# andrewjong/SwapNet

Hardware: NVIDIA H100
Metric: images/sec (G+D fwd+bwd) warp-stage 512x512 (higher is better)
Workload: dtype fp16/bf16-split x3 tensor-core products, fp32 accumulate (fp32-faithful)

## Files before the change

### include/swapnet_b200.h

```cpp
#ifndef SWAPNET_B200_H
#define SWAPNET_B200_H

#include <stdint.h>

#ifdef __cplusplus
extern "C" {
#endif

#define SN_MAX_TAPS 32
#define SN_MAX_SRC 3

enum { SN_ACT_NONE = 0, SN_ACT_TANH = 1, SN_ACT_LRELU = 2, SN_ACT_RELU = 3 };
enum { SN_LAYOUT_NCHW = 0, SN_LAYOUT_NHWC = 1, SN_LAYOUT_LABEL_U8 = 2, SN_LAYOUT_MASK_I32 = 3 };
#define SN_FMT_BF16 0
#define SN_FMT_F16 1

const char* sn_version(void);
const char* sn_last_error(void);
long long sn_launch_count(void);
void sn_count_replayed(long long n);

typedef struct sn_tap {
  int c_off;
  int kb_off;
  int dw, dh;
  int hp;
} sn_tap;

typedef struct sn_tap_gemm_desc {
  const void* a_hi; const void* a_lo;
  int a_n, a_h, a_w, a_c, a_pitch;
  int a_parity;
  int a_fmt;
  int a_chunk;
  const void* b_hi; const void* b_lo;
  int b_rows; long long b_k;
  int b_fmt;
  const float* b_scale;
  int m_n, m_h, m_w;
  int ntaps; int k_per_tap;
  sn_tap taps[SN_MAX_TAPS];
  float* out;
  long long out_sn, out_sh, out_sw;
  int out_mul_h, out_off_h, out_mul_w, out_off_w;
  int n_valid;
  int block_n;
  const float* bias;
  int act;
  int nsplit;
  int nphase;
  int stack_slot, stack_c;
  double* stats;
} sn_tap_gemm_desc;

typedef struct sn_wgrad_desc {
  const void* x_hi; const void* x_lo; int x_n, x_h, x_w, x_c, x_pitch, x_parity, x_fmt;
  const void* y_hi; const void* y_lo; int y_n, y_h, y_w, y_c, y_pitch, y_parity, y_fmt;
  int m_n, m_h, m_w;
  int ntaps;
  sn_tap xtaps[SN_MAX_TAPS];
  sn_tap ytaps[SN_MAX_TAPS];
  long long tap_off[SN_MAX_TAPS];
  float* out; long long s_row, s_col;
  int rows_valid, cols_valid;
  int block_n;
  int y_chunk;
  int ngroups; int group_start[SN_MAX_TAPS]; int group_size[SN_MAX_TAPS];
  int ksplit;
  int nsplit;
  int deterministic;
} sn_wgrad_desc;

typedef struct sn_plan sn_plan;

int sn_tap_gemm_plan_create(const sn_tap_gemm_desc* desc, sn_plan** out);
int sn_wgrad_plan_create(const sn_wgrad_desc* desc, sn_plan** out);
int sn_plan_run(const sn_plan* plan, void* stream);
void sn_plan_destroy(sn_plan* plan);
int sn_plan_has_stats(const sn_plan* plan);
int sn_plan_geometry(const sn_plan* plan, int* out);
long long sn_plan_workspace_bytes(const sn_plan* plan);
int sn_wgrad_ksplit(const sn_wgrad_desc* desc, int sm_count);

int sn_pack_planes(const float* src, int src_layout, int src_pitch, int n, int c, int h, int w,
                   void* dst_hi, void* dst_lo, int dst_pitch, int dst_coff, int fmt, void* stream);

int sn_pack_concat(int lead, const float* src0, int layout0, int pitch0, int c0, const float* src1, int layout1,
                   int pitch1, int c1, int n, int h, int w, int c_fill, void* dst_hi, void* dst_lo, void* dst2_hi,
                   void* dst2_lo, int dst_pitch, int dst_coff, int fmt, int fmt2, void* stream);

typedef struct sn_scale_item { const float* w; long long count; float* scale2; } sn_scale_item;
typedef struct sn_pack_item {
  const float* src; long long s_row, s_k;
  int rows, taps, taps_pitch, k_real, k_pad, fmt;
  void* hi; void* lo; const float* scale2;
  int slot[16];
  int block_begin;
} sn_pack_item;
int sn_weight_scale_multi(const sn_scale_item* items_dev, int nitems, unsigned int* scratch_dev, void* stream);
int sn_pack_weights_multi(const sn_pack_item* items_dev, int nitems, int total_blocks, int max_taps, void* stream);
int sn_pack_rows_per_block(void);
int sn_pack_k_per_block(void);

int sn_pack_head_weights(const float* src, int cout, int cin, int rows_pad, int k_pad, int dgrad, int taps_pitch,
                         void* dst_hi, void* dst_lo, int fmt, const float* scale2, void* stream);
int sn_pack_head_stacked(const float* src, int cout, int cin, int slot, int k_pad, void* dst_hi, void* dst_lo, int fmt,
                         const float* scale2, void* stream);
int sn_fold_head_wgrad(const float* geff, int cout, int cin, float* dw, void* stream);

int sn_plane_stats(const float* y, int pitch, int n, int hw, int c, float eps, double* stats,
                   void* stream);
int sn_stats_finalize(double* stats, int count, int hw, float eps, void* stream);
int sn_plane_sums(const float* y, int pitch, int n, int hw, int c, double* stats, void* stream);

long long sn_det_slots(int n, int c);
int sn_plane_sums_det(const float* y, int pitch, int n, int hw, int c, double* stats, double* slots,
                      long long slots_cap, void* stream);
int sn_plane_stats_det(const float* y, int pitch, int n, int hw, int c, float eps, double* stats, double* slots,
                       long long slots_cap, void* stream);

int sn_bn_finalize(double* stats, int n, int c, int groups, int hw, float eps, float momentum, float* running_mean,
                   float* running_var, long long* num_batches_tracked, void* stream);
int sn_bn_eval_stats(double* stats, int n, int c, const float* running_mean, const float* running_var, float eps,
                     void* stream);
int sn_bn_group_sums(const double* stats, int n, int c, int groups, int hw, double* part, void* stream);
int sn_bn_finalize_gathered(double* stats, int n, int c, int groups, const double* gathered, int world, float eps,
                            float momentum, float* running_mean, float* running_var, long long* num_batches_tracked,
                            void* stream);

typedef struct sn_norm_act_desc {
  const float* y; int y_pitch;
  int n, h, w, c;
  const double* stats;
  int act; float slope;
  float drop_p; unsigned long long drop_seed;
  unsigned long long drop_offset;
  const float* drop_step_seed_dev; unsigned int drop_stage_id;
  const float* residual; int res_pitch;
  void* out_hi; void* out_lo; int out_pitch, out_coff;
  int out_fmt;
  void* out2_hi; void* out2_lo; int out2_fmt;
  int out_reflect_pad;
  float* out_f32; int f32_pitch;
  const float* gamma; const float* beta;
} sn_norm_act_desc;
int sn_norm_act_fwd(const sn_norm_act_desc* d, void* stream);

typedef struct sn_grad_src {
  const float* ptr; int pitch; int c_off;
  int reflect_padded;
  int up;
  int act;
} sn_grad_src;

typedef struct sn_norm_act_bwd_desc {
  sn_grad_src src[SN_MAX_SRC]; int nsrc;
  const float* y; int y_pitch;
  int n, h, w, c;
  const double* stats;
  int act; float slope;
  float drop_p; unsigned long long drop_seed;
  unsigned long long drop_offset; const float* drop_step_seed_dev; unsigned int drop_stage_id;
  double* gstats;
  void* dy_hi; void* dy_lo; int dy_pitch, dy_coff;
  int dy_fmt;
  float* bias_grad;
  const float* gamma; const float* beta;
  int bn_groups;
  int bn_train;
  float* gamma_grad; float* beta_grad;
  double* det_slots; long long det_slots_cap;
  int bn_phase;
  const double* bn_gathered; int bn_world; int bn_rank;
} sn_norm_act_bwd_desc;
int sn_norm_act_bwd(const sn_norm_act_bwd_desc* d, void* stream);

int sn_bias_grad(const void* dy_hi, const void* dy_lo, int pitch, int coff, int fmt, long long npix, int c,
                 double* scratch, float* db, void* stream);
int sn_bias_grad_det(const void* dy_hi, const void* dy_lo, int pitch, int coff, int fmt, long long npix, int c,
                     double* scratch, float* db, double* slots, long long slots_cap, void* stream);

int sn_sum_grads(const sn_grad_src* src, int nsrc, int n, int h, int w, int c, float* dst,
                 int dst_pitch, void* stream);

int sn_tanh_bwd(const sn_grad_src* src, int nsrc, const float* out, int out_pitch, int n, int h,
                int w, int c, void* dy_hi, void* dy_lo, int dy_pitch, int dy_coff, int dy_fmt, void* stream);

int sn_upsample_planes(const void* src_hi, const void* src_lo, int src_pitch, int src_coff, int n, int h, int w,
                       int c, int factor, void* dst_hi, void* dst_lo, int dst_pitch, int dst_coff, void* stream);

int sn_adamw_step(float* p, const float* g, float* m, float* v, long long n, double lr, double beta1, double beta2,
                  double eps, double weight_decay, int step, void* stream);
int sn_adamw_step_dev(float* p, const float* g, float* m, float* v, long long n, const float* hyper_dev, void* stream);
void sn_adamw_hyper(double lr, double beta1, double beta2, double eps, double weight_decay, int step, double gscale,
                    float hyper_out[8]);

int sn_adabound_step(float* p, const float* g, float* m, float* v, long long n, double lr, double base_lr, double beta1,
                     double beta2, double eps, double weight_decay, double final_lr, double gamma, int step,
                     void* stream);
int sn_adabound_step_dev(float* p, const float* g, float* m, float* v, long long n, const float* hyper_dev,
                         void* stream);
void sn_adabound_hyper(double lr, double base_lr, double beta1, double beta2, double eps, double weight_decay,
                       double final_lr, double gamma, int step, double gscale, float hyper_out[8]);

int sn_set_step_params(float* dst, const float* vals, int n, void* stream);

int sn_dropout_mask(unsigned long long seed, float p, long long count, uint8_t* out, void* stream);

int sn_ce_loss_fwd_bwd(const float* logits, int pitch, const void* target, int target_layout, int n, int h, int w,
                       int c, float weight, double* loss_acc, float* grad, int grad_pitch, void* stream);
int sn_ce_tanh_bwd(const float* logits, int pitch, const void* target, int target_layout, const sn_grad_src* src,
                   int nsrc, int n, int h, int w, int c, float weight, double* loss_acc, void* dy_hi, void* dy_lo,
                   int dy_pitch, int dy_coff, int dy_fmt, void* stream);
int sn_ce_tanh_bwd_det(const float* logits, int pitch, const void* target, int target_layout, const sn_grad_src* src,
                       int nsrc, int n, int h, int w, int c, float weight, double* loss_acc, void* dy_hi, void* dy_lo,
                       int dy_pitch, int dy_coff, int dy_fmt, double* slots, long long slots_cap, void* stream);
int sn_bce_logits_fwd_bwd(const float* pred, long long count_per_half, int halves, float t0, float t1,
                          float gscale, double* loss_acc, float* dpred, void* stream);
int sn_bce_logits_fwd_bwd_dev(const float* pred, long long count_per_half, int halves, const float* t_dev,
                              float gscale, double* loss_acc, float* dpred, void* stream);
enum { SN_GAN_BCE = 0, SN_GAN_MSE = 1, SN_GAN_WGAN = 2 };
int sn_gan_loss_fwd_bwd_dev(int objective, const float* pred, long long count_per_half, int halves, float t0, float t1,
                            const float* t_dev, float gscale, double* loss_acc, float* dpred, void* stream);
int sn_gan_loss_fwd_bwd_det(int objective, const float* pred, long long count_per_half, int halves, float t0, float t1,
                            const float* t_dev, float gscale, double* loss_acc, float* dpred, double* slots,
                            long long slots_cap, void* stream);
int sn_l1_loss_fwd_bwd(const float* a, int pitch, const float* b_nchw, int n, int h, int w, int c,
                       float weight, double* loss_acc, float* grad, int grad_pitch, void* stream);
int sn_l1_loss_fwd_bwd_det(const float* a, int pitch, const float* b_nchw, int n, int h, int w, int c, float weight,
                           double* loss_acc, float* grad, int grad_pitch, double* slots, long long slots_cap,
                           void* stream);

int sn_tap_sum_fwd(const float* p, int p_pitch, int n, int h, int w, int k, int pad, const float* bias, float* y,
                   int y_pitch, void* stream);

int sn_to_one_fwd(const void* x_hi, const void* x_lo, int x_pitch, int x_fmt, long long npix, int c, const float* weight,
                  int k, float* p, int p_pitch, void* stream);
int sn_to_one_wgrad(const void* x_hi, const void* x_lo, int x_pitch, int x_fmt, int n, int h, int w, int c,
                    const void* dy_hi, const void* dy_lo, int dy_pitch, int dy_fmt, int k, int pad, float* dw,
                    void* stream);
int sn_to_one_wgrad_det(const void* x_hi, const void* x_lo, int x_pitch, int x_fmt, int n, int h, int w, int c,
                        const void* dy_hi, const void* dy_lo, int dy_pitch, int dy_fmt, int k, int pad, float* dw,
                        float* slots, long long slots_cap, void* stream);
long long sn_to_one_wgrad_det_slots(int c);
int sn_to_one_dgrad(const void* dy_hi, const void* dy_lo, int dy_pitch, int dy_fmt, int n, int h, int w, int c,
                    const float* weight, int k, int pad, float* dx, int dx_pitch, void* stream);

int sn_affine_pack(const float* src, int src_layout, int src_pitch, int n, int c, int h, int w, float mul, float add,
                   void* dst_hi, void* dst_lo, int dst_pitch, int dst_coff, int fmt, void* stream);
int sn_relu_pool_fwd(const float* y, int y_pitch, int n, int h, int w, int c, void* out_hi, void* out_lo,
                     int out_pitch, int out_coff, int fmt, void* stream);
int sn_relu_pool_bwd(const float* y, int y_pitch, const float* g_pool, int gp_pitch, const float* g_direct,
                     int gd_pitch, int n, int h, int w, int c, void* dy_hi, void* dy_lo, int dy_pitch, int dy_coff,
                     int dy_fmt, void* stream);
int sn_feat_loss_fwd_bwd(const float* y_out, int po, const float* y_tgt, int pt, long long npix, int c, double weight,
                         double gscale, double* loss_acc, float* dx, int pdx, void* stream);
int sn_feat_loss_fwd_bwd_det(const float* y_out, int po, const float* y_tgt, int pt, long long npix, int c,
                             double weight, double gscale, double* loss_acc, float* dx, int pdx, double* slots,
                             long long slots_cap, void* stream);

typedef struct sn_pixel_desc {
  const void* x_hi; const void* x_lo;
  const void* xb_hi; const void* xb_lo;
  int x_pitch, x_c;
  int n, hw, cin;
  const float* w1; const float* b1; const float* w2; const float* b2; const float* w3; const float* b3;
  const float* scale1; const float* scale2;
  int norm;
  int nsplit;
  float slope, eps;
  double* stats;
  double* gstats;
  float* pred;
  const float* dpred;
  float* dw1; float* db1; float* dw2; float* db2; float* dw3; float* db3;
  float* dx; int dx_pitch;
  float* debug;
  double* slots; long long slots_cap;
} sn_pixel_desc;
int sn_pixel_fwd_stats(const sn_pixel_desc* d, void* stream);
int sn_pixel_fwd(const sn_pixel_desc* d, void* stream);
int sn_pixel_bwd_reduce(const sn_pixel_desc* d, void* stream);
int sn_pixel_bwd_apply(const sn_pixel_desc* d, void* stream);
long long sn_pixel_det_slots(int n, int cin);
int sn_gram_rows(const float* a, long long a_n, long long a_c, long long a_p, int n_a, const float* b, long long b_n,
                 long long b_c, long long b_p, int n_b, int c, long long npix, double* out, void* stream);
int sn_gram_rows_det(const float* a, long long a_n, long long a_c, long long a_p, int n_a, const float* b,
                     long long b_n, long long b_c, long long b_p, int n_b, int c, long long npix, double* out,
                     double* slots, long long slots_cap, void* stream);
long long sn_gram_rows_det_slots(int rows_l, int rows);
int sn_gram_rows_mse(const double* gram_out, const double* gram_tgt, int rows_l, int rows, double weight,
                     double gscale, double* loss_acc, float* m, void* stream);
int sn_gram_rows_bwd(const float* m, int rows_l, const float* src, long long s_n, long long s_c, long long s_p, int n,
                     int c, long long npix, float* dx, int dx_pitch, int accumulate, void* stream);

int sn_roi_align_pack_fwd(const float* tex_nchw, int b, int ch, int h, int w, const float* rois,
                          int nroi, int pool, float* out_f32, int out_pitch, void* out_hi,
                          void* out_lo, int plane_pitch, int plane_coff, int plane_fmt, void* stream);

#define SN_AUG_NONE 0
#define SN_AUG_HFLIP 1
#define SN_AUG_VFLIP 2
#define SN_AUG_AFFINE_NEAREST 3
#define SN_AUG_PERSPECTIVE_BILINEAR 4
#define SN_AUG_MAX_OPS 8
typedef struct sn_aug_op {
  int kind;
  int nops;
  double p[8];
} sn_aug_op;
int sn_augment_channels(const void* labels_u8, const float* dense_nchw, int n, int c, int h, int w,
                        const sn_aug_op* ops_dev, int op_stride, int max_ops, float* out_nchw, float* tmp_nchw,
                        void* stream);

int sn_tap_gemm_simt(const sn_tap_gemm_desc* desc, void* stream);

#ifdef __cplusplus
}
#endif
#endif
```

### swapnet_b200/_lib.py

```python
from __future__ import annotations

import ctypes as C
import os

_HERE = os.path.dirname(os.path.abspath(__file__))
LIB_PATH = os.path.join(_HERE, "libswapnet_b200.so")

SN_MAX_TAPS = 32
SN_MAX_SRC = 3
ACT_NONE, ACT_TANH, ACT_LRELU, ACT_RELU = 0, 1, 2, 3
LAYOUT_NCHW, LAYOUT_NHWC, LAYOUT_LABEL_U8, LAYOUT_MASK_I32 = 0, 1, 2, 3
FMT_BF16, FMT_F16 = 0, 1
AUG_NONE, AUG_HFLIP, AUG_VFLIP, AUG_AFFINE_NEAREST, AUG_PERSPECTIVE_BILINEAR = 0, 1, 2, 3, 4
AUG_MAX_OPS = 8


class SnTap(C.Structure):
    _fields_ = [("c_off", C.c_int), ("kb_off", C.c_int), ("dw", C.c_int), ("dh", C.c_int), ("hp", C.c_int)]


class SnTapGemmDesc(C.Structure):
    _fields_ = [
        ("a_hi", C.c_void_p), ("a_lo", C.c_void_p),
        ("a_n", C.c_int), ("a_h", C.c_int), ("a_w", C.c_int), ("a_c", C.c_int), ("a_pitch", C.c_int),
        ("a_parity", C.c_int), ("a_fmt", C.c_int), ("a_chunk", C.c_int),
        ("b_hi", C.c_void_p), ("b_lo", C.c_void_p),
        ("b_rows", C.c_int), ("b_k", C.c_longlong), ("b_fmt", C.c_int), ("b_scale", C.c_void_p),
        ("m_n", C.c_int), ("m_h", C.c_int), ("m_w", C.c_int),
        ("ntaps", C.c_int), ("k_per_tap", C.c_int),
        ("taps", SnTap * SN_MAX_TAPS),
        ("out", C.c_void_p),
        ("out_sn", C.c_longlong), ("out_sh", C.c_longlong), ("out_sw", C.c_longlong),
        ("out_mul_h", C.c_int), ("out_off_h", C.c_int), ("out_mul_w", C.c_int), ("out_off_w", C.c_int),
        ("n_valid", C.c_int), ("block_n", C.c_int),
        ("bias", C.c_void_p), ("act", C.c_int), ("nsplit", C.c_int), ("nphase", C.c_int),
        ("stack_slot", C.c_int), ("stack_c", C.c_int), ("stats", C.c_void_p),
    ]


class SnWgradDesc(C.Structure):
    _fields_ = [
        ("x_hi", C.c_void_p), ("x_lo", C.c_void_p),
        ("x_n", C.c_int), ("x_h", C.c_int), ("x_w", C.c_int), ("x_c", C.c_int), ("x_pitch", C.c_int),
        ("x_parity", C.c_int), ("x_fmt", C.c_int),
        ("y_hi", C.c_void_p), ("y_lo", C.c_void_p),
        ("y_n", C.c_int), ("y_h", C.c_int), ("y_w", C.c_int), ("y_c", C.c_int), ("y_pitch", C.c_int),
        ("y_parity", C.c_int), ("y_fmt", C.c_int),
        ("m_n", C.c_int), ("m_h", C.c_int), ("m_w", C.c_int),
        ("ntaps", C.c_int),
        ("xtaps", SnTap * SN_MAX_TAPS), ("ytaps", SnTap * SN_MAX_TAPS),
        ("tap_off", C.c_longlong * SN_MAX_TAPS),
        ("out", C.c_void_p), ("s_row", C.c_longlong), ("s_col", C.c_longlong),
        ("rows_valid", C.c_int), ("cols_valid", C.c_int),
        ("block_n", C.c_int), ("y_chunk", C.c_int),
        ("ngroups", C.c_int), ("group_start", C.c_int * SN_MAX_TAPS), ("group_size", C.c_int * SN_MAX_TAPS),
        ("ksplit", C.c_int), ("nsplit", C.c_int), ("deterministic", C.c_int),
    ]


class SnScaleItem(C.Structure):
    _fields_ = [("w", C.c_void_p), ("count", C.c_longlong), ("scale2", C.c_void_p)]


class SnPackItem(C.Structure):
    _fields_ = [("src", C.c_void_p), ("s_row", C.c_longlong), ("s_k", C.c_longlong),
                ("rows", C.c_int), ("taps", C.c_int), ("taps_pitch", C.c_int), ("k_real", C.c_int), ("k_pad", C.c_int),
                ("fmt", C.c_int), ("hi", C.c_void_p), ("lo", C.c_void_p), ("scale2", C.c_void_p),
                ("slot", C.c_int * 16), ("block_begin", C.c_int)]


class SnNormActDesc(C.Structure):
    _fields_ = [
        ("y", C.c_void_p), ("y_pitch", C.c_int),
        ("n", C.c_int), ("h", C.c_int), ("w", C.c_int), ("c", C.c_int),
        ("stats", C.c_void_p),
        ("act", C.c_int), ("slope", C.c_float),
        ("drop_p", C.c_float), ("drop_seed", C.c_ulonglong),
        ("drop_offset", C.c_ulonglong), ("drop_step_seed_dev", C.c_void_p), ("drop_stage_id", C.c_uint),
        ("residual", C.c_void_p), ("res_pitch", C.c_int),
        ("out_hi", C.c_void_p), ("out_lo", C.c_void_p), ("out_pitch", C.c_int), ("out_coff", C.c_int),
        ("out_fmt", C.c_int), ("out2_hi", C.c_void_p), ("out2_lo", C.c_void_p), ("out2_fmt", C.c_int),
        ("out_reflect_pad", C.c_int),
        ("out_f32", C.c_void_p), ("f32_pitch", C.c_int),
        ("gamma", C.c_void_p), ("beta", C.c_void_p),
    ]


class SnGradSrc(C.Structure):
    _fields_ = [("ptr", C.c_void_p), ("pitch", C.c_int), ("c_off", C.c_int), ("reflect_padded", C.c_int),
                ("up", C.c_int), ("act", C.c_int)]


class SnNormActBwdDesc(C.Structure):
    _fields_ = [
        ("src", SnGradSrc * SN_MAX_SRC), ("nsrc", C.c_int),
        ("y", C.c_void_p), ("y_pitch", C.c_int),
        ("n", C.c_int), ("h", C.c_int), ("w", C.c_int), ("c", C.c_int),
        ("stats", C.c_void_p),
        ("act", C.c_int), ("slope", C.c_float),
        ("drop_p", C.c_float), ("drop_seed", C.c_ulonglong),
        ("drop_offset", C.c_ulonglong), ("drop_step_seed_dev", C.c_void_p), ("drop_stage_id", C.c_uint),
        ("gstats", C.c_void_p),
        ("dy_hi", C.c_void_p), ("dy_lo", C.c_void_p), ("dy_pitch", C.c_int), ("dy_coff", C.c_int),
        ("dy_fmt", C.c_int), ("bias_grad", C.c_void_p),
        ("gamma", C.c_void_p), ("beta", C.c_void_p), ("bn_groups", C.c_int), ("bn_train", C.c_int),
        ("gamma_grad", C.c_void_p), ("beta_grad", C.c_void_p),
        ("det_slots", C.c_void_p), ("det_slots_cap", C.c_longlong),
        ("bn_phase", C.c_int), ("bn_gathered", C.c_void_p), ("bn_world", C.c_int), ("bn_rank", C.c_int),
    ]


class SnPixelDesc(C.Structure):
    _fields_ = [
        ("x_hi", C.c_void_p), ("x_lo", C.c_void_p), ("xb_hi", C.c_void_p), ("xb_lo", C.c_void_p),
        ("x_pitch", C.c_int), ("x_c", C.c_int), ("n", C.c_int), ("hw", C.c_int), ("cin", C.c_int),
        ("w1", C.c_void_p), ("b1", C.c_void_p), ("w2", C.c_void_p), ("b2", C.c_void_p), ("w3", C.c_void_p),
        ("b3", C.c_void_p), ("scale1", C.c_void_p), ("scale2", C.c_void_p),
        ("norm", C.c_int), ("nsplit", C.c_int), ("slope", C.c_float), ("eps", C.c_float),
        ("stats", C.c_void_p), ("gstats", C.c_void_p), ("pred", C.c_void_p), ("dpred", C.c_void_p),
        ("dw1", C.c_void_p), ("db1", C.c_void_p), ("dw2", C.c_void_p), ("db2", C.c_void_p), ("dw3", C.c_void_p),
        ("db3", C.c_void_p), ("dx", C.c_void_p), ("dx_pitch", C.c_int), ("debug", C.c_void_p),
        ("slots", C.c_void_p), ("slots_cap", C.c_longlong),
    ]


_VP, _I, _LL, _F, _ULL = C.c_void_p, C.c_int, C.c_longlong, C.c_float, C.c_ulonglong
SIGNATURES = {
    "sn_version": (C.c_char_p, []),
    "sn_last_error": (C.c_char_p, []),
    "sn_launch_count": (_LL, []),
    "sn_count_replayed": (None, [_LL]),
    "sn_tap_gemm_plan_create": (_I, [C.POINTER(SnTapGemmDesc), C.POINTER(_VP)]),
    "sn_wgrad_plan_create": (_I, [C.POINTER(SnWgradDesc), C.POINTER(_VP)]),
    "sn_plan_run": (_I, [_VP, _VP]),
    "sn_plan_destroy": (None, [_VP]),
    "sn_plan_has_stats": (_I, [_VP]),
    "sn_plan_geometry": (_I, [_VP, C.POINTER(C.c_int)]),
    "sn_plan_workspace_bytes": (_LL, [_VP]),
    "sn_wgrad_ksplit": (_I, [C.POINTER(SnWgradDesc), _I]),
    "sn_det_slots": (_LL, [_I, _I]),
    "sn_plane_sums_det": (_I, [_VP, _I, _I, _I, _I, _VP, _VP, _LL, _VP]),
    "sn_plane_stats_det": (_I, [_VP, _I, _I, _I, _I, _F, _VP, _VP, _LL, _VP]),
    "sn_bias_grad_det": (_I, [_VP, _VP, _I, _I, _I, _LL, _I, _VP, _VP, _VP, _LL, _VP]),
    "sn_ce_tanh_bwd_det": (_I, [_VP, _I, _VP, _I, C.POINTER(SnGradSrc), _I, _I, _I, _I, _I, _F, _VP, _VP, _VP, _I, _I,
                                _I, _VP, _LL, _VP]),
    "sn_gan_loss_fwd_bwd_det": (_I, [_I, _VP, _LL, _I, _F, _F, _VP, _F, _VP, _VP, _VP, _LL, _VP]),
    "sn_l1_loss_fwd_bwd_det": (_I, [_VP, _I, _VP, _I, _I, _I, _I, _F, _VP, _VP, _I, _VP, _LL, _VP]),
    "sn_to_one_wgrad_det": (_I, [_VP, _VP, _I, _I, _I, _I, _I, _I, _VP, _VP, _I, _I, _I, _I, _VP, _VP, _LL, _VP]),
    "sn_to_one_wgrad_det_slots": (_LL, [_I]),
    "sn_stats_finalize": (_I, [_VP, _I, _I, _F, _VP]),
    "sn_plane_sums": (_I, [_VP, _I, _I, _I, _I, _VP, _VP]),
    "sn_bn_finalize": (_I, [_VP, _I, _I, _I, _I, _F, _F, _VP, _VP, _VP, _VP]),
    "sn_bn_eval_stats": (_I, [_VP, _I, _I, _VP, _VP, _F, _VP]),
    "sn_bn_group_sums": (_I, [_VP, _I, _I, _I, _I, _VP, _VP]),
    "sn_bn_finalize_gathered": (_I, [_VP, _I, _I, _I, _VP, _I, _F, _F, _VP, _VP, _VP, _VP]),
    "sn_pack_planes": (_I, [_VP, _I, _I, _I, _I, _I, _I, _VP, _VP, _I, _I, _I, _VP]),
    "sn_pack_concat": (_I, [_I, _VP, _I, _I, _I, _VP, _I, _I, _I, _I, _I, _I, _I, _VP, _VP, _VP, _VP, _I, _I, _I, _I, _VP]),
    "sn_pack_head_weights": (_I, [_VP, _I, _I, _I, _I, _I, _I, _VP, _VP, _I, _VP, _VP]),
    "sn_weight_scale_multi": (_I, [_VP, _I, _VP, _VP]),
    "sn_pack_weights_multi": (_I, [_VP, _I, _I, _I, _VP]),
    "sn_pack_rows_per_block": (_I, []),
    "sn_pack_k_per_block": (_I, []),
    "sn_pack_head_stacked": (_I, [_VP, _I, _I, _I, _I, _VP, _VP, _I, _VP, _VP]),
    "sn_fold_head_wgrad": (_I, [_VP, _I, _I, _VP, _VP]),
    "sn_plane_stats": (_I, [_VP, _I, _I, _I, _I, _F, _VP, _VP]),
    "sn_norm_act_fwd": (_I, [C.POINTER(SnNormActDesc), _VP]),
    "sn_norm_act_bwd": (_I, [C.POINTER(SnNormActBwdDesc), _VP]),
    "sn_bias_grad": (_I, [_VP, _VP, _I, _I, _I, _LL, _I, _VP, _VP, _VP]),
    "sn_sum_grads": (_I, [C.POINTER(SnGradSrc), _I, _I, _I, _I, _I, _VP, _I, _VP]),
    "sn_tanh_bwd": (_I, [C.POINTER(SnGradSrc), _I, _VP, _I, _I, _I, _I, _I, _VP, _VP, _I, _I, _I, _VP]),
    "sn_upsample_planes": (_I, [_VP, _VP, _I, _I, _I, _I, _I, _I, _I, _VP, _VP, _I, _I, _VP]),
    "sn_adamw_step": (_I, [_VP, _VP, _VP, _VP, _LL, C.c_double, C.c_double, C.c_double, C.c_double, C.c_double, _I, _VP]),
    "sn_adamw_step_dev": (_I, [_VP, _VP, _VP, _VP, _LL, _VP, _VP]),
    "sn_adamw_hyper": (None, [C.c_double, C.c_double, C.c_double, C.c_double, C.c_double, _I, C.c_double,
                              C.POINTER(C.c_float)]),
    "sn_adabound_step": (_I, [_VP, _VP, _VP, _VP, _LL] + [C.c_double] * 8 + [_I, _VP]),
    "sn_adabound_step_dev": (_I, [_VP, _VP, _VP, _VP, _LL, _VP, _VP]),
    "sn_adabound_hyper": (None, [C.c_double] * 8 + [_I, C.c_double, C.POINTER(C.c_float)]),
    "sn_set_step_params": (_I, [_VP, C.POINTER(C.c_float), _I, _VP]),
    "sn_bce_logits_fwd_bwd_dev": (_I, [_VP, _LL, _I, _VP, _F, _VP, _VP, _VP]),
    "sn_dropout_mask": (_I, [_ULL, _F, _LL, _VP, _VP]),
    "sn_ce_loss_fwd_bwd": (_I, [_VP, _I, _VP, _I, _I, _I, _I, _I, _F, _VP, _VP, _I, _VP]),
    "sn_ce_tanh_bwd": (_I, [_VP, _I, _VP, _I, C.POINTER(SnGradSrc), _I, _I, _I, _I, _I, _F, _VP, _VP, _VP, _I, _I, _I, _VP]),
    "sn_bce_logits_fwd_bwd": (_I, [_VP, _LL, _I, _F, _F, _F, _VP, _VP, _VP]),
    "sn_gan_loss_fwd_bwd_dev": (_I, [_I, _VP, _LL, _I, _F, _F, _VP, _F, _VP, _VP, _VP]),
    "sn_l1_loss_fwd_bwd": (_I, [_VP, _I, _VP, _I, _I, _I, _I, _F, _VP, _VP, _I, _VP]),
    "sn_tap_sum_fwd": (_I, [_VP, _I, _I, _I, _I, _I, _I, _VP, _VP, _I, _VP]),
    "sn_to_one_fwd": (_I, [_VP, _VP, _I, _I, _LL, _I, _VP, _I, _VP, _I, _VP]),
    "sn_to_one_wgrad": (_I, [_VP, _VP, _I, _I, _I, _I, _I, _I, _VP, _VP, _I, _I, _I, _I, _VP, _VP]),
    "sn_to_one_dgrad": (_I, [_VP, _VP, _I, _I, _I, _I, _I, _I, _VP, _I, _I, _VP, _I, _VP]),
    "sn_affine_pack": (_I, [_VP, _I, _I, _I, _I, _I, _I, _F, _F, _VP, _VP, _I, _I, _I, _VP]),
    "sn_relu_pool_fwd": (_I, [_VP, _I, _I, _I, _I, _I, _VP, _VP, _I, _I, _I, _VP]),
    "sn_relu_pool_bwd": (_I, [_VP, _I, _VP, _I, _VP, _I, _I, _I, _I, _I, _VP, _VP, _I, _I, _I, _VP]),
    "sn_feat_loss_fwd_bwd": (_I, [_VP, _I, _VP, _I, _LL, _I, C.c_double, C.c_double, _VP, _VP, _I, _VP]),
    "sn_feat_loss_fwd_bwd_det": (_I, [_VP, _I, _VP, _I, _LL, _I, C.c_double, C.c_double, _VP, _VP, _I, _VP, _LL, _VP]),
    "sn_gram_rows": (_I, [_VP, _LL, _LL, _LL, _I, _VP, _LL, _LL, _LL, _I, _I, _LL, _VP, _VP]),
    "sn_gram_rows_det": (_I, [_VP, _LL, _LL, _LL, _I, _VP, _LL, _LL, _LL, _I, _I, _LL, _VP, _VP, _LL, _VP]),
    "sn_gram_rows_det_slots": (_LL, [_I, _I]),
    "sn_gram_rows_mse": (_I, [_VP, _VP, _I, _I, C.c_double, C.c_double, _VP, _VP, _VP]),
    "sn_gram_rows_bwd": (_I, [_VP, _I, _VP, _LL, _LL, _LL, _I, _I, _LL, _VP, _I, _I, _VP]),
    "sn_roi_align_pack_fwd": (_I, [_VP, _I, _I, _I, _I, _VP, _I, _I, _VP, _I, _VP, _VP, _I, _I, _I, _VP]),
    "sn_tap_gemm_simt": (_I, [C.POINTER(SnTapGemmDesc), _VP]),
    "sn_pixel_fwd_stats": (_I, [C.POINTER(SnPixelDesc), _VP]),
    "sn_pixel_fwd": (_I, [C.POINTER(SnPixelDesc), _VP]),
    "sn_pixel_bwd_reduce": (_I, [C.POINTER(SnPixelDesc), _VP]),
    "sn_pixel_bwd_apply": (_I, [C.POINTER(SnPixelDesc), _VP]),
    "sn_pixel_det_slots": (_LL, [_I, _I]),
    "sn_augment_channels": (_I, [_VP, _VP, _I, _I, _I, _I, _VP, _I, _I, _VP, _VP, _VP]),
}

_lib = None


class SwapnetB200Error(RuntimeError):
    pass


def load(build_if_missing: bool = False) -> C.CDLL:
    global _lib
    if _lib is not None:
        return _lib
    if not os.path.exists(LIB_PATH):
        if build_if_missing:
            from . import build as _build

            _build.build(verbose=False)
        else:
            raise SwapnetB200Error(
                f"{LIB_PATH} is missing: build it with `python -m swapnet_b200.build` "
                "(there is no CPU / eager fallback for the hot path)"
            )
    lib = C.CDLL(LIB_PATH)
    for name, (res, args) in SIGNATURES.items():
        fn = getattr(lib, name)
        fn.restype = res
        fn.argtypes = args
    _lib = lib
    return lib


def check(rc: int) -> None:
    if rc != 0:
        msg = load().sn_last_error().decode("utf-8", "replace")
        raise SwapnetB200Error(f"libswapnet_b200 call failed ({rc}): {msg}")
```

### swapnet_b200/csrc/api.cu

```cuda
#include <stdarg.h>
#include <atomic>
#include "common.cuh"
#include "plan.h"

static thread_local char g_err[1024] = "";
std::atomic<long long> g_launches{0};

void sn_set_error(const char* fmt, ...) {
  va_list ap;
  va_start(ap, fmt);
  vsnprintf(g_err, sizeof(g_err), fmt, ap);
  va_end(ap);
}
void sn_count_launch(int n) { g_launches.fetch_add(n, std::memory_order_relaxed); }

struct sn_plan {
  int kind;
  TapGemmPlan tg;
  WgradPlan wg;
};

static int g_sm_count = 0;
static int sm_count() {
  if (!g_sm_count) {
    int dev = 0;
    cudaGetDevice(&dev);
    cudaDeviceGetAttribute(&g_sm_count, cudaDevAttrMultiProcessorCount, dev);
    if (g_sm_count <= 0) g_sm_count = SN_NUM_SMS;
  }
  return g_sm_count;
}

extern "C" {

const char* sn_version(void) { return "swapnet_b200 0.1.0 (sm_90a, wgmma split-bf16)"; }
const char* sn_last_error(void) { return g_err; }
long long sn_launch_count(void) { return g_launches.load(std::memory_order_relaxed); }
void sn_count_replayed(long long n) { g_launches.fetch_add(n, std::memory_order_relaxed); }

int sn_tap_gemm_plan_create(const sn_tap_gemm_desc* desc, sn_plan** out) {
  SN_REQUIRE(desc && out, "null argument");
  sn_plan* p = new sn_plan();
  p->kind = 0;
  int rc = sn_tap_gemm_plan_init(&p->tg, desc);
  if (rc) {
    delete p;
    return rc;
  }
  *out = p;
  return SN_OK;
}

int sn_wgrad_plan_create(const sn_wgrad_desc* desc, sn_plan** out) {
  SN_REQUIRE(desc && out, "null argument");
  sn_plan* p = new sn_plan();
  p->kind = 1;
  int rc = sn_wgrad_plan_init(&p->wg, desc, sm_count());
  if (rc) {
    delete p;
    return rc;
  }
  *out = p;
  return SN_OK;
}

int sn_plan_run(const sn_plan* plan, void* stream) {
  SN_REQUIRE(plan, "null plan");
  sn_count_launch(1);
  if (plan->kind == 0) return sn_tap_gemm_plan_launch(&plan->tg, (cudaStream_t)stream);
  return sn_wgrad_plan_launch(&plan->wg, (cudaStream_t)stream);
}

int sn_plan_has_stats(const sn_plan* plan) { return plan && plan->kind == 0 && plan->tg.p.stats != nullptr; }

int sn_plan_geometry(const sn_plan* plan, int* out) {
  SN_REQUIRE(plan && out, "null argument");
  const dim3 g = plan->kind == 0 ? plan->tg.grid : plan->wg.grid;
  out[0] = plan->kind;
  out[1] = (int)g.x;
  out[2] = (int)g.y;
  out[3] = (int)g.z;
  out[4] = plan->kind == 0 ? plan->tg.p.block_n : plan->wg.p.block_n;
  out[5] = plan->kind == 0 ? plan->tg.p.a_chunk : plan->wg.p.y_chunk;
  return SN_OK;
}

long long sn_plan_workspace_bytes(const sn_plan* plan) {
  return plan && plan->kind == 1 ? (long long)plan->wg.ws_bytes : 0;
}

int sn_wgrad_ksplit(const sn_wgrad_desc* desc, int sm_count) { return sn_wgrad_plan_ksplit(desc, sm_count); }

void sn_plan_destroy(sn_plan* plan) {
  if (plan && plan->kind == 0 && plan->tg.p.tile_counter) cudaFree(plan->tg.p.tile_counter);
  if (plan && plan->kind == 1 && plan->wg.p.det_ws) cudaFree(plan->wg.p.det_ws);
  delete plan;
}

}
```

### swapnet_b200/csrc/common.cuh

```cuda
#pragma once
#include <cuda_runtime.h>
#include <cuda.h>
#include <cuda_bf16.h>
#include <cuda_fp16.h>
#include <stdint.h>
#include <stdio.h>
#include <string.h>

void sn_set_error(const char* fmt, ...);
#define SN_OK 0
#define SN_ERR_INVALID (-1)
#define SN_ERR_CUDA (-2)
#define SN_ERR_UNSUPPORTED (-3)
#define SN_NUM_SMS 132
#ifndef SN_FMT_BF16
#define SN_FMT_BF16 0
#define SN_FMT_F16 1
#endif

#define SN_CHECK_CUDA(expr)                                                        \
  do {                                                                             \
    cudaError_t _e = (expr);                                                       \
    if (_e != cudaSuccess) {                                                       \
      sn_set_error("%s:%d CUDA error %s: %s", __FILE__, __LINE__, #expr,           \
                   cudaGetErrorString(_e));                                        \
      return SN_ERR_CUDA;                                                          \
    }                                                                              \
  } while (0)

#define SN_REQUIRE(cond, ...)                                                      \
  do {                                                                             \
    if (!(cond)) {                                                                 \
      sn_set_error(__VA_ARGS__);                                                   \
      return SN_ERR_INVALID;                                                       \
    }                                                                              \
  } while (0)

#ifdef __CUDACC__

__device__ __forceinline__ uint32_t smem_u32(const void* p) {
  return static_cast<uint32_t>(__cvta_generic_to_shared(p));
}

__device__ __forceinline__ bool elect_one_sync() {
  uint32_t pred = 0;
  asm volatile(
      "{\n\t"
      ".reg .pred P;\n\t"
      "elect.sync _|P, 0xffffffff;\n\t"
      "selp.b32 %0, 1, 0, P;\n\t"
      "}\n"
      : "=r"(pred));
  return pred != 0;
}

__device__ __forceinline__ void mbar_init(uint64_t* bar, uint32_t count) {
  asm volatile("mbarrier.init.shared::cta.b64 [%0], %1;" ::"r"(smem_u32(bar)), "r"(count));
}
__device__ __forceinline__ void mbar_fence_init() {
  asm volatile("fence.mbarrier_init.release.cluster;" ::: "memory");
}
__device__ __forceinline__ void mbar_expect_tx(uint64_t* bar, uint32_t bytes) {
  asm volatile("mbarrier.arrive.expect_tx.shared::cta.b64 _, [%0], %1;" ::"r"(smem_u32(bar)),
               "r"(bytes)
               : "memory");
}
__device__ __forceinline__ void mbar_arrive(uint64_t* bar) {
  asm volatile("mbarrier.arrive.shared::cta.b64 _, [%0];" ::"r"(smem_u32(bar)) : "memory");
}
__device__ __forceinline__ bool mbar_try_wait(uint64_t* bar, uint32_t parity) {
  uint32_t ok;
  asm volatile(
      "{\n\t"
      ".reg .pred P;\n\t"
      "mbarrier.try_wait.parity.shared::cta.b64 P, [%1], %2;\n\t"
      "selp.b32 %0, 1, 0, P;\n\t"
      "}\n"
      : "=r"(ok)
      : "r"(smem_u32(bar)), "r"(parity)
      : "memory");
  return ok != 0;
}
__device__ __forceinline__ void mbar_wait(uint64_t* bar, uint32_t parity) {
  uint32_t spins = 0;
  while (!mbar_try_wait(bar, parity)) {
    if (++spins > (1u << 28)) __trap();
  }
}

__device__ __forceinline__ void tma_prefetch_desc(const void* desc) {
  asm volatile("prefetch.tensormap [%0];" ::"l"(reinterpret_cast<uint64_t>(desc)) : "memory");
}
__device__ __forceinline__ void tma_load_2d(const void* desc, uint64_t* bar, void* dst, int c0,
                                            int c1) {
  asm volatile(
      "cp.async.bulk.tensor.2d.shared::cluster.global.mbarrier::complete_tx::bytes"
      " [%0], [%1, {%3, %4}], [%2];"
      :
      : "r"(smem_u32(dst)), "l"(reinterpret_cast<uint64_t>(desc)), "r"(smem_u32(bar)), "r"(c0),
        "r"(c1)
      : "memory");
}
__device__ __forceinline__ void tma_load_3d(const void* desc, uint64_t* bar, void* dst, int c0, int c1, int c2) {
  asm volatile(
      "cp.async.bulk.tensor.3d.shared::cluster.global.mbarrier::complete_tx::bytes"
      " [%0], [%1, {%3, %4, %5}], [%2];"
      :
      : "r"(smem_u32(dst)), "l"(reinterpret_cast<uint64_t>(desc)), "r"(smem_u32(bar)), "r"(c0), "r"(c1), "r"(c2)
      : "memory");
}
__device__ __forceinline__ void tma_load_5d(const void* desc, uint64_t* bar, void* dst, int c0,
                                            int c1, int c2, int c3, int c4) {
  asm volatile(
      "cp.async.bulk.tensor.5d.shared::cluster.global.mbarrier::complete_tx::bytes"
      " [%0], [%1, {%3, %4, %5, %6, %7}], [%2];"
      :
      : "r"(smem_u32(dst)), "l"(reinterpret_cast<uint64_t>(desc)), "r"(smem_u32(bar)), "r"(c0),
        "r"(c1), "r"(c2), "r"(c3), "r"(c4)
      : "memory");
}

__device__ __forceinline__ void wgmma_fence() { asm volatile("wgmma.fence.sync.aligned;" ::: "memory"); }
__device__ __forceinline__ void wgmma_commit() { asm volatile("wgmma.commit_group.sync.aligned;" ::: "memory"); }
template <int N>
__device__ __forceinline__ void wgmma_wait() {
  asm volatile("wgmma.wait_group.sync.aligned %0;" ::"n"(N) : "memory");
}
template <int R>
__device__ __forceinline__ void wgmma_fence_acc(float (&d)[R]) {
#pragma unroll
  for (int i = 0; i < R; ++i) asm volatile("" : "+f"(d[i])::"memory");
}

template <int N, bool F16>
struct Wgmma;
template <> struct Wgmma<16, false> {
  template <int TA, int TB>
  static __device__ __forceinline__ void mma(float (&d)[8], uint64_t a, uint64_t b, int scale_d) {
    asm volatile(
        "{\n.reg .pred p;\nsetp.ne.b32 p, %10, 0;\n"
        "wgmma.mma_async.sync.aligned.m64n16k16.f32.bf16.bf16 "
        "{%0, %1, %2, %3, %4, %5, %6, %7}, %8, %9, p, 1, 1, %11, %12;\n}\n"
        : "+f"(d[0]), "+f"(d[1]), "+f"(d[2]), "+f"(d[3]), "+f"(d[4]), "+f"(d[5]), "+f"(d[6]), "+f"(d[7])
        : "l"(a), "l"(b), "r"(scale_d), "n"(TA), "n"(TB));
  }
};
template <> struct Wgmma<16, true> {
  template <int TA, int TB>
  static __device__ __forceinline__ void mma(float (&d)[8], uint64_t a, uint64_t b, int scale_d) {
    asm volatile(
        "{\n.reg .pred p;\nsetp.ne.b32 p, %10, 0;\n"
        "wgmma.mma_async.sync.aligned.m64n16k16.f32.f16.f16 "
        "{%0, %1, %2, %3, %4, %5, %6, %7}, %8, %9, p, 1, 1, %11, %12;\n}\n"
        : "+f"(d[0]), "+f"(d[1]), "+f"(d[2]), "+f"(d[3]), "+f"(d[4]), "+f"(d[5]), "+f"(d[6]), "+f"(d[7])
        : "l"(a), "l"(b), "r"(scale_d), "n"(TA), "n"(TB));
  }
};
template <> struct Wgmma<32, false> {
  template <int TA, int TB>
  static __device__ __forceinline__ void mma(float (&d)[16], uint64_t a, uint64_t b, int scale_d) {
    asm volatile(
        "{\n.reg .pred p;\nsetp.ne.b32 p, %18, 0;\n"
        "wgmma.mma_async.sync.aligned.m64n32k16.f32.bf16.bf16 "
        "{%0, %1, %2, %3, %4, %5, %6, %7, %8, %9, %10, %11, %12, %13, %14, %15}, %16, %17, p, 1, 1, %19, %20;\n}\n"
        : "+f"(d[0]), "+f"(d[1]), "+f"(d[2]), "+f"(d[3]), "+f"(d[4]), "+f"(d[5]), "+f"(d[6]), "+f"(d[7]), "+f"(d[8]), "+f"(d[9]), "+f"(d[10]), "+f"(d[11]), "+f"(d[12]), "+f"(d[13]), "+f"(d[14]), "+f"(d[15])
        : "l"(a), "l"(b), "r"(scale_d), "n"(TA), "n"(TB));
  }
};
template <> struct Wgmma<32, true> {
  template <int TA, int TB>
  static __device__ __forceinline__ void mma(float (&d)[16], uint64_t a, uint64_t b, int scale_d) {
    asm volatile(
        "{\n.reg .pred p;\nsetp.ne.b32 p, %18, 0;\n"
        "wgmma.mma_async.sync.aligned.m64n32k16.f32.f16.f16 "
        "{%0, %1, %2, %3, %4, %5, %6, %7, %8, %9, %10, %11, %12, %13, %14, %15}, %16, %17, p, 1, 1, %19, %20;\n}\n"
        : "+f"(d[0]), "+f"(d[1]), "+f"(d[2]), "+f"(d[3]), "+f"(d[4]), "+f"(d[5]), "+f"(d[6]), "+f"(d[7]), "+f"(d[8]), "+f"(d[9]), "+f"(d[10]), "+f"(d[11]), "+f"(d[12]), "+f"(d[13]), "+f"(d[14]), "+f"(d[15])
        : "l"(a), "l"(b), "r"(scale_d), "n"(TA), "n"(TB));
  }
};
template <> struct Wgmma<64, false> {
  template <int TA, int TB>
  static __device__ __forceinline__ void mma(float (&d)[32], uint64_t a, uint64_t b, int scale_d) {
    asm volatile(
        "{\n.reg .pred p;\nsetp.ne.b32 p, %34, 0;\n"
        "wgmma.mma_async.sync.aligned.m64n64k16.f32.bf16.bf16 "
        "{%0, %1, %2, %3, %4, %5, %6, %7, %8, %9, %10, %11, %12, %13, %14, %15, %16, %17, %18, %19, %20, %21, %22, %23, %24, %25, %26, %27, %28, %29, %30, %31}, %32, %33, p, 1, 1, %35, %36;\n}\n"
        : "+f"(d[0]), "+f"(d[1]), "+f"(d[2]), "+f"(d[3]), "+f"(d[4]), "+f"(d[5]), "+f"(d[6]), "+f"(d[7]), "+f"(d[8]), "+f"(d[9]), "+f"(d[10]), "+f"(d[11]), "+f"(d[12]), "+f"(d[13]), "+f"(d[14]), "+f"(d[15]), "+f"(d[16]), "+f"(d[17]), "+f"(d[18]), "+f"(d[19]), "+f"(d[20]), "+f"(d[21]), "+f"(d[22]), "+f"(d[23]), "+f"(d[24]), "+f"(d[25]), "+f"(d[26]), "+f"(d[27]), "+f"(d[28]), "+f"(d[29]), "+f"(d[30]), "+f"(d[31])
        : "l"(a), "l"(b), "r"(scale_d), "n"(TA), "n"(TB));
  }
};
template <> struct Wgmma<64, true> {
  template <int TA, int TB>
  static __device__ __forceinline__ void mma(float (&d)[32], uint64_t a, uint64_t b, int scale_d) {
    asm volatile(
        "{\n.reg .pred p;\nsetp.ne.b32 p, %34, 0;\n"
        "wgmma.mma_async.sync.aligned.m64n64k16.f32.f16.f16 "
        "{%0, %1, %2, %3, %4, %5, %6, %7, %8, %9, %10, %11, %12, %13, %14, %15, %16, %17, %18, %19, %20, %21, %22, %23, %24, %25, %26, %27, %28, %29, %30, %31}, %32, %33, p, 1, 1, %35, %36;\n}\n"
        : "+f"(d[0]), "+f"(d[1]), "+f"(d[2]), "+f"(d[3]), "+f"(d[4]), "+f"(d[5]), "+f"(d[6]), "+f"(d[7]), "+f"(d[8]), "+f"(d[9]), "+f"(d[10]), "+f"(d[11]), "+f"(d[12]), "+f"(d[13]), "+f"(d[14]), "+f"(d[15]), "+f"(d[16]), "+f"(d[17]), "+f"(d[18]), "+f"(d[19]), "+f"(d[20]), "+f"(d[21]), "+f"(d[22]), "+f"(d[23]), "+f"(d[24]), "+f"(d[25]), "+f"(d[26]), "+f"(d[27]), "+f"(d[28]), "+f"(d[29]), "+f"(d[30]), "+f"(d[31])
        : "l"(a), "l"(b), "r"(scale_d), "n"(TA), "n"(TB));
  }
};
template <> struct Wgmma<96, false> {
  template <int TA, int TB>
  static __device__ __forceinline__ void mma(float (&d)[48], uint64_t a, uint64_t b, int scale_d) {
    asm volatile(
        "{\n.reg .pred p;\nsetp.ne.b32 p, %50, 0;\n"
        "wgmma.mma_async.sync.aligned.m64n96k16.f32.bf16.bf16 "
        "{%0, %1, %2, %3, %4, %5, %6, %7, %8, %9, %10, %11, %12, %13, %14, %15, %16, %17, %18, %19, %20, %21, %22, %23, %24, %25, %26, %27, %28, %29, %30, %31, %32, %33, %34, %35, %36, %37, %38, %39, %40, %41, %42, %43, %44, %45, %46, %47}, %48, %49, p, 1, 1, %51, %52;\n}\n"
        : "+f"(d[0]), "+f"(d[1]), "+f"(d[2]), "+f"(d[3]), "+f"(d[4]), "+f"(d[5]), "+f"(d[6]), "+f"(d[7]), "+f"(d[8]), "+f"(d[9]), "+f"(d[10]), "+f"(d[11]), "+f"(d[12]), "+f"(d[13]), "+f"(d[14]), "+f"(d[15]), "+f"(d[16]), "+f"(d[17]), "+f"(d[18]), "+f"(d[19]), "+f"(d[20]), "+f"(d[21]), "+f"(d[22]), "+f"(d[23]), "+f"(d[24]), "+f"(d[25]), "+f"(d[26]), "+f"(d[27]), "+f"(d[28]), "+f"(d[29]), "+f"(d[30]), "+f"(d[31]), "+f"(d[32]), "+f"(d[33]), "+f"(d[34]), "+f"(d[35]), "+f"(d[36]), "+f"(d[37]), "+f"(d[38]), "+f"(d[39]), "+f"(d[40]), "+f"(d[41]), "+f"(d[42]), "+f"(d[43]), "+f"(d[44]), "+f"(d[45]), "+f"(d[46]), "+f"(d[47])
        : "l"(a), "l"(b), "r"(scale_d), "n"(TA), "n"(TB));
  }
};
template <> struct Wgmma<96, true> {
  template <int TA, int TB>
  static __device__ __forceinline__ void mma(float (&d)[48], uint64_t a, uint64_t b, int scale_d) {
    asm volatile(
        "{\n.reg .pred p;\nsetp.ne.b32 p, %50, 0;\n"
        "wgmma.mma_async.sync.aligned.m64n96k16.f32.f16.f16 "
        "{%0, %1, %2, %3, %4, %5, %6, %7, %8, %9, %10, %11, %12, %13, %14, %15, %16, %17, %18, %19, %20, %21, %22, %23, %24, %25, %26, %27, %28, %29, %30, %31, %32, %33, %34, %35, %36, %37, %38, %39, %40, %41, %42, %43, %44, %45, %46, %47}, %48, %49, p, 1, 1, %51, %52;\n}\n"
        : "+f"(d[0]), "+f"(d[1]), "+f"(d[2]), "+f"(d[3]), "+f"(d[4]), "+f"(d[5]), "+f"(d[6]), "+f"(d[7]), "+f"(d[8]), "+f"(d[9]), "+f"(d[10]), "+f"(d[11]), "+f"(d[12]), "+f"(d[13]), "+f"(d[14]), "+f"(d[15]), "+f"(d[16]), "+f"(d[17]), "+f"(d[18]), "+f"(d[19]), "+f"(d[20]), "+f"(d[21]), "+f"(d[22]), "+f"(d[23]), "+f"(d[24]), "+f"(d[25]), "+f"(d[26]), "+f"(d[27]), "+f"(d[28]), "+f"(d[29]), "+f"(d[30]), "+f"(d[31]), "+f"(d[32]), "+f"(d[33]), "+f"(d[34]), "+f"(d[35]), "+f"(d[36]), "+f"(d[37]), "+f"(d[38]), "+f"(d[39]), "+f"(d[40]), "+f"(d[41]), "+f"(d[42]), "+f"(d[43]), "+f"(d[44]), "+f"(d[45]), "+f"(d[46]), "+f"(d[47])
        : "l"(a), "l"(b), "r"(scale_d), "n"(TA), "n"(TB));
  }
};
template <> struct Wgmma<128, false> {
  template <int TA, int TB>
  static __device__ __forceinline__ void mma(float (&d)[64], uint64_t a, uint64_t b, int scale_d) {
    asm volatile(
        "{\n.reg .pred p;\nsetp.ne.b32 p, %66, 0;\n"
        "wgmma.mma_async.sync.aligned.m64n128k16.f32.bf16.bf16 "
        "{%0, %1, %2, %3, %4, %5, %6, %7, %8, %9, %10, %11, %12, %13, %14, %15, %16, %17, %18, %19, %20, %21, %22, %23, %24, %25, %26, %27, %28, %29, %30, %31, %32, %33, %34, %35, %36, %37, %38, %39, %40, %41, %42, %43, %44, %45, %46, %47, %48, %49, %50, %51, %52, %53, %54, %55, %56, %57, %58, %59, %60, %61, %62, %63}, %64, %65, p, 1, 1, %67, %68;\n}\n"
        : "+f"(d[0]), "+f"(d[1]), "+f"(d[2]), "+f"(d[3]), "+f"(d[4]), "+f"(d[5]), "+f"(d[6]), "+f"(d[7]), "+f"(d[8]), "+f"(d[9]), "+f"(d[10]), "+f"(d[11]), "+f"(d[12]), "+f"(d[13]), "+f"(d[14]), "+f"(d[15]), "+f"(d[16]), "+f"(d[17]), "+f"(d[18]), "+f"(d[19]), "+f"(d[20]), "+f"(d[21]), "+f"(d[22]), "+f"(d[23]), "+f"(d[24]), "+f"(d[25]), "+f"(d[26]), "+f"(d[27]), "+f"(d[28]), "+f"(d[29]), "+f"(d[30]), "+f"(d[31]), "+f"(d[32]), "+f"(d[33]), "+f"(d[34]), "+f"(d[35]), "+f"(d[36]), "+f"(d[37]), "+f"(d[38]), "+f"(d[39]), "+f"(d[40]), "+f"(d[41]), "+f"(d[42]), "+f"(d[43]), "+f"(d[44]), "+f"(d[45]), "+f"(d[46]), "+f"(d[47]), "+f"(d[48]), "+f"(d[49]), "+f"(d[50]), "+f"(d[51]), "+f"(d[52]), "+f"(d[53]), "+f"(d[54]), "+f"(d[55]), "+f"(d[56]), "+f"(d[57]), "+f"(d[58]), "+f"(d[59]), "+f"(d[60]), "+f"(d[61]), "+f"(d[62]), "+f"(d[63])
        : "l"(a), "l"(b), "r"(scale_d), "n"(TA), "n"(TB));
  }
};
template <> struct Wgmma<128, true> {
  template <int TA, int TB>
  static __device__ __forceinline__ void mma(float (&d)[64], uint64_t a, uint64_t b, int scale_d) {
    asm volatile(
        "{\n.reg .pred p;\nsetp.ne.b32 p, %66, 0;\n"
        "wgmma.mma_async.sync.aligned.m64n128k16.f32.f16.f16 "
        "{%0, %1, %2, %3, %4, %5, %6, %7, %8, %9, %10, %11, %12, %13, %14, %15, %16, %17, %18, %19, %20, %21, %22, %23, %24, %25, %26, %27, %28, %29, %30, %31, %32, %33, %34, %35, %36, %37, %38, %39, %40, %41, %42, %43, %44, %45, %46, %47, %48, %49, %50, %51, %52, %53, %54, %55, %56, %57, %58, %59, %60, %61, %62, %63}, %64, %65, p, 1, 1, %67, %68;\n}\n"
        : "+f"(d[0]), "+f"(d[1]), "+f"(d[2]), "+f"(d[3]), "+f"(d[4]), "+f"(d[5]), "+f"(d[6]), "+f"(d[7]), "+f"(d[8]), "+f"(d[9]), "+f"(d[10]), "+f"(d[11]), "+f"(d[12]), "+f"(d[13]), "+f"(d[14]), "+f"(d[15]), "+f"(d[16]), "+f"(d[17]), "+f"(d[18]), "+f"(d[19]), "+f"(d[20]), "+f"(d[21]), "+f"(d[22]), "+f"(d[23]), "+f"(d[24]), "+f"(d[25]), "+f"(d[26]), "+f"(d[27]), "+f"(d[28]), "+f"(d[29]), "+f"(d[30]), "+f"(d[31]), "+f"(d[32]), "+f"(d[33]), "+f"(d[34]), "+f"(d[35]), "+f"(d[36]), "+f"(d[37]), "+f"(d[38]), "+f"(d[39]), "+f"(d[40]), "+f"(d[41]), "+f"(d[42]), "+f"(d[43]), "+f"(d[44]), "+f"(d[45]), "+f"(d[46]), "+f"(d[47]), "+f"(d[48]), "+f"(d[49]), "+f"(d[50]), "+f"(d[51]), "+f"(d[52]), "+f"(d[53]), "+f"(d[54]), "+f"(d[55]), "+f"(d[56]), "+f"(d[57]), "+f"(d[58]), "+f"(d[59]), "+f"(d[60]), "+f"(d[61]), "+f"(d[62]), "+f"(d[63])
        : "l"(a), "l"(b), "r"(scale_d), "n"(TA), "n"(TB));
  }
};


__device__ __forceinline__ uint64_t gmma_smem_desc(uint32_t smem_addr, uint32_t lbo_bytes, uint32_t sbo_bytes,
                                                   uint32_t layout = 1) {
  uint64_t d = 0;
  d |= (uint64_t)((smem_addr >> 4) & 0x3FFF);
  d |= (uint64_t)((lbo_bytes >> 4) & 0x3FFF) << 16;
  d |= (uint64_t)((sbo_bytes >> 4) & 0x3FFF) << 32;
  d |= (uint64_t)(layout & 3u) << 62;
  return d;
}
__host__ __device__ __forceinline__ uint32_t gmma_layout_of_chunk(int chunk) {
  return chunk >= 64 ? 1u : (chunk == 32 ? 2u : 3u);
}

__device__ __forceinline__ void split16(float v, int fmt, uint16_t& hi, uint16_t& lo) {
  if (fmt == SN_FMT_F16) {
    if (fabsf(v) <= 3.402823466e38f) v = fminf(fmaxf(v, -65504.f), 65504.f);
    const __half h = __float2half_rn(v);
    const __half l = __float2half_rn(v - __half2float(h));
    hi = __half_as_ushort(h);
    lo = __half_as_ushort(l);
  } else {
    const __nv_bfloat16 h = __float2bfloat16_rn(v);
    const __nv_bfloat16 l = __float2bfloat16_rn(v - __bfloat162float(h));
    hi = __bfloat16_as_ushort(h);
    lo = __bfloat16_as_ushort(l);
  }
}
__device__ __forceinline__ float decode16(uint16_t x, int fmt) {
  return fmt == SN_FMT_F16 ? __half2float(__ushort_as_half(x)) : __bfloat162float(__ushort_as_bfloat16(x));
}

__device__ __forceinline__ float warp_sum(float v) {
#pragma unroll
  for (int o = 16; o > 0; o >>= 1) v += __shfl_xor_sync(0xffffffffu, v, o);
  return v;
}

template <typename T>
__global__ void det_sum_slots_kernel(const T* __restrict__ slots, int nslots, long long count, T* __restrict__ dst) {
  for (long long i = blockIdx.x * (long long)blockDim.x + threadIdx.x; i < count;
       i += (long long)gridDim.x * blockDim.x) {
    T s = slots[i];
    for (int k = 1; k < nslots; ++k) s += slots[(long long)k * count + i];
    dst[i] += s;
  }
}
template <typename T>
inline cudaError_t det_sum_slots(const T* slots, int nslots, long long count, T* dst, cudaStream_t st) {
  long long g = (count + 255) / 256;
  if (g > SN_NUM_SMS * 8) g = SN_NUM_SMS * 8;
  det_sum_slots_kernel<T><<<(int)(g < 1 ? 1 : g), 256, 0, st>>>(slots, nslots, count, dst);
  return cudaGetLastError();
}

#endif
```

### swapnet_b200/csrc/gemm_tc.cu

```cuda
#include "common.cuh"
#include "plan.h"

namespace {

constexpr int kBlockM = 128;
constexpr int kTileRing = 4;
constexpr int kTileBytes = 16384;
constexpr int kConsumerWarps = 8;
constexpr int kProducerWarp = kConsumerWarps;
constexpr int kThreads = (kConsumerWarps + 1) * 32;

template <int NSPLIT>
struct Cfg {
  static constexpr int kPlanes = NSPLIT == 3 ? 2 : 1;
  static constexpr int kStages = NSPLIT == 3 ? 3 : 6;
  static constexpr int kStageBytes = kPlanes * 2 * kTileBytes;
  static constexpr int kSmemBytes = kStages * kStageBytes + 1024;
};

__device__ __forceinline__ float apply_act(float v, int act) {
  if (act == SN_ACT_TANH) return tanhf(v);
  return v;
}

__device__ __forceinline__ float quad_col_sum(float v) {
  v += __shfl_xor_sync(0xffffffffu, v, 4);
  v += __shfl_xor_sync(0xffffffffu, v, 8);
  v += __shfl_xor_sync(0xffffffffu, v, 16);
  return v;
}

template <int NSPLIT, int CW, int BN, bool F16>
__global__ void __launch_bounds__(kThreads, 1)
tap_gemm_kernel(const __grid_constant__ TapGemmParams p, const int m_tiles, const int n_tiles, const int total_tiles) {
  const auto tile_coords = [&](int tile, int& mt, int& nt, int& z) {
    nt = tile % n_tiles;
    const int rest = tile / n_tiles;
    mt = rest % m_tiles;
    z = rest / m_tiles;
  };
  using C = Cfg<NSPLIT>;
  extern __shared__ uint8_t smem_raw[];
  __shared__ __align__(8) uint64_t full_bar[C::kStages];
  __shared__ __align__(8) uint64_t empty_bar[C::kStages];
  __shared__ __align__(8) uint64_t tr_full[kTileRing];
  __shared__ __align__(8) uint64_t tr_empty[kTileRing];
  __shared__ int tile_ring[kTileRing];

  const uint32_t smem_base = (smem_u32(smem_raw) + 1023u) & ~1023u;
  uint8_t* smem = smem_raw + (smem_base - smem_u32(smem_raw));
  const int warp = threadIdx.x >> 5;
  const int lane = threadIdx.x & 31;

  constexpr int cw = CW;
  constexpr int tps = 64 / cw;
  const int tpp = p.ntaps / p.nphase;
  const int k_iters = cw == 64 ? tpp * p.chunks : tpp / tps;

  if (threadIdx.x == 0) {
    for (int s = 0; s < C::kStages; ++s) {
      mbar_init(&full_bar[s], 1);
      mbar_init(&empty_bar[s], 2);
    }
    for (int r = 0; r < kTileRing; ++r) {
      mbar_init(&tr_full[r], 1);
      mbar_init(&tr_empty[r], kConsumerWarps);
    }
    mbar_fence_init();
  }
  if (warp == kProducerWarp && lane == 0) {
    for (int pl = 0; pl < C::kPlanes; ++pl) {
      tma_prefetch_desc(&p.tmA[pl]);
      tma_prefetch_desc(&p.tmB[pl]);
    }
  }
  __syncthreads();

  if (warp == kProducerWarp) {
    if (lane == 0) {
      const uint32_t stage_tx = C::kPlanes * (p.a_rows * 128 + p.block_n * 128);
      uint32_t it = 0, tcount = 0;
      for (int tile = blockIdx.x;; ++tcount) {
        const int next = tile < total_tiles ? (int)gridDim.x + atomicAdd(p.tile_counter, 1) : total_tiles;
        const uint32_t slot = tcount % kTileRing, rph = (tcount / kTileRing) & 1;
        mbar_wait(&tr_empty[slot], rph ^ 1);
        tile_ring[slot] = tile < total_tiles ? tile : -1;
        mbar_arrive(&tr_full[slot]);
        if (tile >= total_tiles) break;
        int mt, nt, z;
        tile_coords(tile, mt, nt, z);
        const int ncol0 = nt * p.block_n;
        const int tap0 = z * tpp;
        const int w0 = (mt % p.tiles_w) * p.tw;
        const int h0 = ((mt / p.tiles_w) % p.tiles_h) * p.th;
        const int n0 = (mt / (p.tiles_w * p.tiles_h)) * p.nb;
        for (int k = 0; k < k_iters; ++k, ++it) {
          const uint32_t s = it % C::kStages;
          const uint32_t ph = (it / C::kStages) & 1;
          mbar_wait(&empty_bar[s], ph ^ 1);
          mbar_expect_tx(&full_bar[s], stage_tx);
          uint8_t* st = smem + s * C::kStageBytes;
          if (cw == 64) {
            const int t = k / p.chunks;
            const int ch = k - t * p.chunks;
            const TapDesc tap = p.taps[tap0 + t];
            if (p.a_merged) {
              tma_load_5d(&p.tmA[0], &full_bar[s], st, tap.c_off + ch * 64, w0 + tap.dw, h0 + tap.dh, n0, 0);
            } else {
#pragma unroll
              for (int pl = 0; pl < C::kPlanes; ++pl)
                tma_load_5d(&p.tmA[pl], &full_bar[s], st + pl * kTileBytes, tap.c_off + ch * 64,
                            w0 + tap.dw, tap.hp, h0 + tap.dh, n0);
            }
            if (p.b_merged) {
              tma_load_3d(&p.tmB[0], &full_bar[s], st + C::kPlanes * kTileBytes, tap.kb_off + ch * 64, ncol0, 0);
            } else {
#pragma unroll
              for (int pl = 0; pl < C::kPlanes; ++pl)
                tma_load_2d(&p.tmB[pl], &full_bar[s], st + (C::kPlanes + pl) * kTileBytes,
                            tap.kb_off + ch * 64, ncol0);
            }
          } else {
            constexpr int sub = 128 * cw * 2;
#pragma unroll
            for (int j = 0; j < tps; ++j) {
              const TapDesc tap = p.taps[tap0 + k * tps + j];
#pragma unroll
              for (int pl = 0; pl < C::kPlanes; ++pl)
                tma_load_5d(&p.tmA[pl], &full_bar[s], st + pl * kTileBytes + j * sub, tap.c_off,
                            w0 + tap.dw, tap.hp, h0 + tap.dh, n0);
            }
            const int kb = p.taps[tap0 + k * tps].kb_off;
            if (p.b_merged) {
              tma_load_3d(&p.tmB[0], &full_bar[s], st + C::kPlanes * kTileBytes, kb, ncol0, 0);
            } else {
#pragma unroll
              for (int pl = 0; pl < C::kPlanes; ++pl)
                tma_load_2d(&p.tmB[pl], &full_bar[s], st + (C::kPlanes + pl) * kTileBytes, kb, ncol0);
            }
          }
        }
        tile = next;
      }
    }
  } else {
    const int wg = warp >> 2;
    const int quad = lane & 3;
    const int row0 = wg * 64 + (warp & 3) * 16 + (lane >> 2);
    int w_i[2], h_i[2], n_i[2];
#pragma unroll
    for (int h = 0; h < 2; ++h) {
      const int row = row0 + 8 * h;
      w_i[h] = row % p.tw;
      h_i[h] = (row / p.tw) % p.th;
      n_i[h] = row / (p.tw * p.th);
    }
    const float oscale = p.b_scale ? p.b_scale[1] : 1.f;
    float acc[BN / 2];
    uint32_t it = 0;
    for (uint32_t tcount = 0;; ++tcount) {
      const uint32_t slot = tcount % kTileRing, rph = (tcount / kTileRing) & 1;
      mbar_wait(&tr_full[slot], rph);
      const int tile = tile_ring[slot];
      __syncwarp();
      if (lane == 0) mbar_arrive(&tr_empty[slot]);
      if (tile < 0) break;
      for (int k = 0; k < k_iters; ++k, ++it) {
        const uint32_t s = it % C::kStages;
        const uint32_t ph = (it / C::kStages) & 1;
        mbar_wait(&full_bar[s], ph);
        const uint32_t st = smem_base + s * C::kStageBytes;
        constexpr uint32_t a_layout = cw >= 64 ? 1u : (cw == 32 ? 2u : 3u);
        constexpr uint32_t a_sbo = 8u * cw * 2u;
        const uint32_t a_row0 = (uint32_t)wg * 64u * cw * 2u;
        const uint64_t a_hi = gmma_smem_desc(st + a_row0, 16, a_sbo, a_layout);
        const uint64_t b_hi = gmma_smem_desc(st + C::kPlanes * kTileBytes, 16, 1024);
        const uint64_t a_lo = gmma_smem_desc(st + p.a_lo_off + a_row0, 16, a_sbo, a_layout);
        const uint64_t b_lo = gmma_smem_desc(st + C::kPlanes * kTileBytes + p.b_lo_off, 16, 1024);
        constexpr uint32_t sub16 = (uint32_t)(128 * cw * 2) >> 4;
        wgmma_fence();
#pragma unroll
        for (int kk = 0; kk < 4; ++kk) {
          const uint64_t badv = (uint64_t)(kk * 2);
          const uint64_t aadv = (uint64_t)(((kk * 16) / cw) * sub16 + (((kk * 16) % cw) >> 3));
          Wgmma<BN, F16>::template mma<0, 0>(acc, a_hi + aadv, b_hi + badv, (k | kk) != 0);
          if (NSPLIT == 3) {
            Wgmma<BN, F16>::template mma<0, 0>(acc, a_lo + aadv, b_hi + badv, 1);
            Wgmma<BN, F16>::template mma<0, 0>(acc, a_hi + aadv, b_lo + badv, 1);
          }
        }
        wgmma_commit();
        wgmma_wait<0>();
        wgmma_fence_acc(acc);
        if ((threadIdx.x & 127) == 0) mbar_arrive(&empty_bar[s]);
      }

      int mt, nt, z;
      tile_coords(tile, mt, nt, z);
      const int ncol0 = nt * p.block_n;
      const int ph_h = p.nphase == 4 ? (z >> 1) : 0, ph_w = p.nphase == 4 ? (z & 1) : 0;
      int gw[2], gh[2], gn[2];
      bool valid[2];
      float* optr[2];
#pragma unroll
      for (int h = 0; h < 2; ++h) {
        gw[h] = (mt % p.tiles_w) * p.tw + w_i[h];
        gh[h] = ((mt / p.tiles_w) % p.tiles_h) * p.th + h_i[h];
        gn[h] = (mt / (p.tiles_w * p.tiles_h)) * p.nb + n_i[h];
        valid[h] = (row0 + 8 * h < p.a_rows) && (gw[h] < p.m_w) && (gh[h] < p.m_h) && (gn[h] < p.m_n);
        optr[h] = p.out + (long long)gn[h] * p.out_sn + (long long)(gh[h] * p.omh + p.ooh + ph_h) * p.out_sh +
                  (long long)(gw[h] * p.omw + p.oow + ph_w) * p.out_sw + ncol0;
      }
#pragma unroll
      for (int i = 0; i < BN / 8; ++i) {
        const int c = 8 * i + 2 * quad;
        if (BN > 16 && 8 * i >= p.block_n) break;
        if (p.stack_slot) {
#pragma unroll
          for (int h = 0; h < 2; ++h) {
            if (!valid[h]) continue;
#pragma unroll
            for (int e = 0; e < 2; ++e) {
              const int col = ncol0 + c + e;
              const int ph = col / p.stack_slot, ch = col - ph * p.stack_slot;
              if (ph < 4 && ch < p.stack_c) {
                float v = acc[4 * i + 2 * h + e] * oscale;
                if (p.bias) v += p.bias[ch];
                float* o = p.out + (long long)gn[h] * p.out_sn + (long long)(gh[h] * p.omh + (ph >> 1)) * p.out_sh +
                           (long long)(gw[h] * p.omw + (ph & 1)) * p.out_sw + ch;
                *o = apply_act(v, p.act);
              }
            }
          }
        } else if (p.stats) {
          if (ncol0 + 8 * i >= p.n_valid) continue;
          float v[2][2];
#pragma unroll
          for (int h = 0; h < 2; ++h) {
#pragma unroll
            for (int e = 0; e < 2; ++e) {
              float t = acc[4 * i + 2 * h + e] * oscale;
              if (p.bias) t += p.bias[ncol0 + c + e];
              v[h][e] = valid[h] ? t : 0.f;
            }
            if (valid[h]) *reinterpret_cast<float2*>(optr[h] + c) = make_float2(v[h][0], v[h][1]);
          }
          const float s0 = quad_col_sum(v[0][0] + v[1][0]);
          const float s1 = quad_col_sum(v[0][1] + v[1][1]);
          const float q0 = quad_col_sum(v[0][0] * v[0][0] + v[1][0] * v[1][0]);
          const float q1 = quad_col_sum(v[0][1] * v[0][1] + v[1][1] * v[1][1]);
          if (lane < 4) {
            const int tn = (mt / (p.tiles_w * p.tiles_h)) * p.nb;
            double* sp = p.stats + ((long long)tn * p.n_valid + ncol0 + c) * 2;
            atomicAdd(sp, (double)s0);
            atomicAdd(sp + 1, (double)q0);
            atomicAdd(sp + 2, (double)s1);
            atomicAdd(sp + 3, (double)q1);
          }
        } else {
#pragma unroll
          for (int h = 0; h < 2; ++h) {
            if (!valid[h]) continue;
            float v0 = acc[4 * i + 2 * h] * oscale, v1 = acc[4 * i + 2 * h + 1] * oscale;
            const int col = ncol0 + c;
            if (p.vec4 && col + 1 < p.n_valid) {
              if (p.bias) {
                const float2 bb = *reinterpret_cast<const float2*>(p.bias + col);
                v0 += bb.x; v1 += bb.y;
              }
              *reinterpret_cast<float2*>(optr[h] + c) = make_float2(apply_act(v0, p.act), apply_act(v1, p.act));
            } else {
              if (col < p.n_valid) optr[h][c] = apply_act(p.bias ? v0 + p.bias[col] : v0, p.act);
              if (col + 1 < p.n_valid) optr[h][c + 1] = apply_act(p.bias ? v1 + p.bias[col + 1] : v1, p.act);
            }
          }
        }
      }
    }
  }

  __syncthreads();
  if (threadIdx.x == 0) {
    __threadfence();
    if (atomicAdd(p.tile_counter + 1, 1) == (int)gridDim.x - 1) {
      p.tile_counter[0] = 0;
      p.tile_counter[1] = 0;
      __threadfence();
    }
  }
}

template <int NSPLIT, int BN, bool F16, bool DET>
__global__ void __launch_bounds__(kThreads, 1)
wgrad_gemm_kernel(const __grid_constant__ WgradParams p) {
  using C = Cfg<NSPLIT>;
  extern __shared__ uint8_t smem_raw[];
  __shared__ __align__(8) uint64_t full_bar[C::kStages];
  __shared__ __align__(8) uint64_t empty_bar[C::kStages];

  const uint32_t smem_base = (smem_u32(smem_raw) + 1023u) & ~1023u;
  uint8_t* smem = smem_raw + (smem_base - smem_u32(smem_raw));
  const int warp = threadIdx.x >> 5;
  const int lane = threadIdx.x & 31;

  const int m_tile = blockIdx.x / p.n_tiles;
  const int n_tile = blockIdx.x - m_tile * p.n_tiles;
  const bool grouped = p.ngroups > 0;
  const int tap_i = grouped ? p.gstart[blockIdx.y] : blockIdx.y;
  const int gsize = grouped ? p.gsize[blockIdx.y] : 1;
  const int m0 = m_tile * kBlockM;
  const int ncol0 = n_tile * p.block_n;
  const int total = p.tiles_w * p.tiles_h * p.tiles_n;
  const int kt0 = (int)(((long long)total * blockIdx.z) / gridDim.z);
  const int kt1 = (int)(((long long)total * (blockIdx.z + 1)) / gridDim.z);
  const int k_iters = kt1 - kt0;
  const int ycw = p.y_chunk;
  const int y_blocks = ycw == 64 ? p.block_n / 64 : gsize;
  const int y_block_bytes = 64 * ycw * 2;

  if (threadIdx.x == 0) {
    for (int s = 0; s < C::kStages; ++s) {
      mbar_init(&full_bar[s], 1);
      mbar_init(&empty_bar[s], 2);
    }
    mbar_fence_init();
  }
  if (warp == kProducerWarp && lane == 0) {
    for (int pl = 0; pl < C::kPlanes; ++pl) {
      tma_prefetch_desc(&p.tmX[pl]);
      tma_prefetch_desc(&p.tmY[pl]);
    }
  }
  __syncthreads();

  if (k_iters > 0) {
    if (warp == kProducerWarp) {
      if (lane == 0) {
        const TapDesc xt = p.xtaps[tap_i];
        const uint32_t stage_tx = C::kPlanes * (2 * 8192 + y_blocks * y_block_bytes);
        for (int it = 0; it < k_iters; ++it) {
          const int s = it % C::kStages;
          const uint32_t ph = (it / C::kStages) & 1;
          mbar_wait(&empty_bar[s], ph ^ 1);
          mbar_expect_tx(&full_bar[s], stage_tx);
          const int kt = kt0 + it;
          const int tw_i = kt % p.tiles_w;
          const int th_i = (kt / p.tiles_w) % p.tiles_h;
          const int tn_i = kt / (p.tiles_w * p.tiles_h);
          const int w0 = tw_i * p.tw, h0 = th_i * p.th, n0 = tn_i * p.nb;
          uint8_t* st = smem + s * C::kStageBytes;
          if (p.x_merged) {
            for (int b = 0; b < 2; ++b)
              tma_load_5d(&p.tmX[0], &full_bar[s], st + b * 16384, xt.c_off + m0 + b * 64, w0 + xt.dw, h0 + xt.dh,
                          n0, 0);
          } else {
#pragma unroll
            for (int pl = 0; pl < C::kPlanes; ++pl)
              for (int b = 0; b < 2; ++b)
                tma_load_5d(&p.tmX[pl], &full_bar[s], st + pl * kTileBytes + b * 8192,
                            xt.c_off + m0 + b * 64, w0 + xt.dw, xt.hp, h0 + xt.dh, n0);
          }
          if (p.y_merged) {
            const TapDesc yt = p.ytaps[tap_i];
            for (int b = 0; b < y_blocks; ++b)
              tma_load_5d(&p.tmY[0], &full_bar[s], st + C::kPlanes * kTileBytes + b * 16384,
                          yt.c_off + ncol0 + b * 64, w0 + yt.dw, h0 + yt.dh, n0, 0);
          } else {
#pragma unroll
            for (int pl = 0; pl < C::kPlanes; ++pl)
              for (int b = 0; b < y_blocks; ++b) {
                const TapDesc yt = p.ytaps[grouped ? tap_i + b : tap_i];
                tma_load_5d(&p.tmY[pl], &full_bar[s],
                            st + (C::kPlanes + pl) * kTileBytes + b * y_block_bytes,
                            yt.c_off + (grouped ? 0 : ncol0 + b * 64), w0 + yt.dw, yt.hp, h0 + yt.dh, n0);
              }
          }
        }
      }
    } else if (warp < kProducerWarp) {
      const int wg = warp >> 2;
      float acc[BN / 2], part[BN / 2];
#pragma unroll
      for (int i = 0; i < BN / 2; ++i) acc[i] = 0.f;
      const uint32_t y_layout = gmma_layout_of_chunk(ycw);
      const uint32_t y_sbo = 8u * ycw * 2u;
      const uint32_t x_lbo = p.x_merged ? 16384u : 8192u;
      const uint32_t x_lo_off = p.x_merged ? 8192u : (uint32_t)kTileBytes;
      const uint32_t y_lbo = p.y_merged ? 16384u : (uint32_t)y_block_bytes;
      const uint32_t y_lo_off = p.y_merged ? 8192u : (uint32_t)kTileBytes;
      for (int it = 0; it < k_iters; ++it) {
        const int s = it % C::kStages;
        const uint32_t ph = (it / C::kStages) & 1;
        mbar_wait(&full_bar[s], ph);
        const uint32_t st = smem_base + s * C::kStageBytes;
        const uint64_t x_hi = gmma_smem_desc(st + wg * x_lbo, x_lbo, 1024);
        const uint64_t y_hi = gmma_smem_desc(st + C::kPlanes * kTileBytes, y_lbo, y_sbo, y_layout);
        const uint64_t x_lo = gmma_smem_desc(st + x_lo_off + wg * x_lbo, x_lbo, 1024);
        const uint64_t y_lo = gmma_smem_desc(st + C::kPlanes * kTileBytes + y_lo_off, y_lbo, y_sbo, y_layout);
        wgmma_fence();
#pragma unroll
        for (int k = 0; k < 4; ++k) {
          const uint64_t xadv = (uint64_t)(k * 128);
          const uint64_t yadv = (uint64_t)((k * 16 * ycw * 2) >> 4);
          Wgmma<BN, F16>::template mma<1, 1>(part, x_hi + xadv, y_hi + yadv, k != 0);
          if (NSPLIT == 3) {
            Wgmma<BN, F16>::template mma<1, 1>(part, x_lo + xadv, y_hi + yadv, 1);
            Wgmma<BN, F16>::template mma<1, 1>(part, x_hi + xadv, y_lo + yadv, 1);
          }
        }
        wgmma_commit();
        wgmma_wait<0>();
        wgmma_fence_acc(part);
        if ((threadIdx.x & 127) == 0) mbar_arrive(&empty_bar[s]);
#pragma unroll
        for (int i = 0; i < BN / 2; ++i) acc[i] += part[i];
      }
      const int quad = lane & 3;
      const int row0 = m0 + wg * 64 + (warp & 3) * 16 + (lane >> 2);
#pragma unroll
      for (int h = 0; h < 2; ++h) {
        const int row = row0 + 8 * h;
        if (row >= p.rows_valid) continue;
        float* orow = p.out + (long long)row * p.s_row;
        float* wrow = DET ? p.det_ws + (long long)blockIdx.z * p.det_count + (long long)row * p.cols_valid : nullptr;
#pragma unroll
        for (int i = 0; i < BN / 8; ++i) {
#pragma unroll
          for (int e = 0; e < 2; ++e) {
            const int c = 8 * i + 2 * quad + e;
            const float v = acc[4 * i + 2 * h + e];
            if (!grouped) {
              const int col = ncol0 + c;
              if (c < p.block_n && col < p.cols_valid) {
                if constexpr (DET) wrow[(long long)tap_i * p.rows_valid * p.cols_valid + col] = v;
                else atomicAdd(orow + p.tap_off[tap_i] + (long long)col * p.s_col, v);
              }
            } else {
              const int b = c / ycw;
              const int cbase = c - b * ycw;
              if (b < gsize && cbase < p.cols_valid) {
                if constexpr (DET) wrow[(long long)(tap_i + b) * p.rows_valid * p.cols_valid + cbase] = v;
                else atomicAdd(orow + p.tap_off[tap_i + b] + (long long)cbase * p.s_col, v);
              }
            }
          }
        }
      }
    }
  }
}

__global__ void __launch_bounds__(256) wgrad_det_sum_kernel(const __grid_constant__ WgradParams p, int ksplit) {
  const long long rc = (long long)p.rows_valid * p.cols_valid;
  for (long long e = blockIdx.x * (long long)blockDim.x + threadIdx.x; e < p.det_count;
       e += (long long)gridDim.x * blockDim.x) {
    float s = p.det_ws[e];
    for (int z = 1; z < ksplit; ++z) s += p.det_ws[(long long)z * p.det_count + e];
    const int tap = (int)(e / rc);
    const long long r = e - tap * rc;
    const int row = (int)(r / p.cols_valid), col = (int)(r - (long long)row * p.cols_valid);
    p.out[(long long)row * p.s_row + p.tap_off[tap] + (long long)col * p.s_col] += s;
  }
}

}

void sn_count_launch(int n);
typedef CUresult (*PFN_encodeTiled)(CUtensorMap*, CUtensorMapDataType, cuuint32_t, void*,
                                    const cuuint64_t*, const cuuint64_t*, const cuuint32_t*,
                                    const cuuint32_t*, CUtensorMapInterleave, CUtensorMapSwizzle,
                                    CUtensorMapL2promotion, CUtensorMapFloatOOBfill);

static PFN_encodeTiled get_encode_fn() {
  static PFN_encodeTiled fn = nullptr;
  if (!fn) {
    void* ptr = nullptr;
    cudaDriverEntryPointQueryResult qres;
    cudaError_t e = cudaGetDriverEntryPoint("cuTensorMapEncodeTiled", &ptr, cudaEnableDefault, &qres);
    if (e != cudaSuccess || qres != cudaDriverEntryPointSuccess || !ptr) return nullptr;
    fn = reinterpret_cast<PFN_encodeTiled>(ptr);
  }
  return fn;
}

int sn_make_act_map(CUtensorMap* tm, const void* base, int N, int H, int W, int C, int pitch,
                    int parity, int box_w, int box_h, int box_n, int chunk = 64, long long plane_stride = 0) {
  PFN_encodeTiled enc = get_encode_fn();
  SN_REQUIRE(enc != nullptr, "cuTensorMapEncodeTiled driver entry point unavailable");
  SN_REQUIRE(pitch % 8 == 0 && ((uintptr_t)base % 16) == 0,
             "activation plane needs 16-B aligned base and pitch %% 8 == 0 (pitch=%d)", pitch);
  SN_REQUIRE(box_w >= 1 && box_h >= 1 && box_n >= 1 && box_w <= 256 && box_h <= 256 && box_n <= 256,
             "bad TMA box %d x %d x %d", box_w, box_h, box_n);
  cuuint64_t dims[5];
  cuuint64_t strides[4];
  const cuuint64_t e = 2;
  cuuint32_t box[5] = {(cuuint32_t)chunk, (cuuint32_t)box_w, 1, (cuuint32_t)box_h, (cuuint32_t)box_n};
  if (plane_stride > 0) {
    SN_REQUIRE(plane_stride % 16 == 0, "merged planes: 16-B aligned plane stride");
    if (!parity) {
      dims[0] = C; dims[1] = W; dims[2] = H; dims[3] = N; dims[4] = 2;
      strides[0] = (cuuint64_t)pitch * e;
      strides[1] = (cuuint64_t)W * pitch * e;
    } else {
      SN_REQUIRE(H % 2 == 0 && W % 2 == 0, "parity view needs even H, W (got %d x %d)", H, W);
      dims[0] = (cuuint64_t)(W + 1) * pitch + C; dims[1] = W / 2; dims[2] = H / 2; dims[3] = N; dims[4] = 2;
      strides[0] = (cuuint64_t)2 * pitch * e;
      strides[1] = (cuuint64_t)2 * W * pitch * e;
    }
    strides[2] = (cuuint64_t)H * W * pitch * e;
    strides[3] = (cuuint64_t)plane_stride;
    box[2] = (cuuint32_t)box_h; box[3] = (cuuint32_t)box_n; box[4] = 2;
  } else if (!parity) {
    dims[0] = C; dims[1] = W; dims[2] = 1; dims[3] = H; dims[4] = N;
    strides[0] = (cuuint64_t)pitch * e;
    strides[1] = (cuuint64_t)W * pitch * e;
    strides[2] = (cuuint64_t)W * pitch * e;
    strides[3] = (cuuint64_t)H * W * pitch * e;
  } else {
    SN_REQUIRE(H % 2 == 0 && W % 2 == 0, "parity view needs even H, W (got %d x %d)", H, W);
    dims[0] = (cuuint64_t)pitch + C; dims[1] = W / 2; dims[2] = 2; dims[3] = H / 2; dims[4] = N;
    strides[0] = (cuuint64_t)2 * pitch * e;
    strides[1] = (cuuint64_t)W * pitch * e;
    strides[2] = (cuuint64_t)2 * W * pitch * e;
    strides[3] = (cuuint64_t)H * W * pitch * e;
  }
  SN_REQUIRE(chunk == 64 || chunk == 32 || chunk == 16, "row chunk must be 64, 32 or 16 channels (got %d)", chunk);
  cuuint32_t estr[5] = {1, 1, 1, 1, 1};
  const CUtensorMapSwizzle swz = chunk == 64 ? CU_TENSOR_MAP_SWIZZLE_128B
                                 : chunk == 32 ? CU_TENSOR_MAP_SWIZZLE_64B : CU_TENSOR_MAP_SWIZZLE_32B;
  CUresult r = enc(tm, CU_TENSOR_MAP_DATA_TYPE_BFLOAT16, 5, const_cast<void*>(base), dims, strides,
                   box, estr, CU_TENSOR_MAP_INTERLEAVE_NONE, swz,
                   CU_TENSOR_MAP_L2_PROMOTION_L2_256B, CU_TENSOR_MAP_FLOAT_OOB_FILL_NONE);
  SN_REQUIRE(r == CUDA_SUCCESS,
             "cuTensorMapEncodeTiled(act) failed: %d (N=%d H=%d W=%d C=%d pitch=%d parity=%d box=%dx%dx%d)",
             (int)r, N, H, W, C, pitch, parity, box_w, box_h, box_n);
  return SN_OK;
}

int sn_make_weight_map(CUtensorMap* tm, const void* base, int rows, long long k_total, int box_rows,
                       long long plane_stride = 0) {
  PFN_encodeTiled enc = get_encode_fn();
  SN_REQUIRE(enc != nullptr, "cuTensorMapEncodeTiled driver entry point unavailable");
  SN_REQUIRE(k_total % 64 == 0 && ((uintptr_t)base % 16) == 0, "packed weights need K %% 64 == 0");
  cuuint64_t dims[3] = {(cuuint64_t)k_total, (cuuint64_t)rows, 2};
  cuuint64_t strides[2] = {(cuuint64_t)k_total * 2, (cuuint64_t)plane_stride};
  cuuint32_t box[3] = {64, (cuuint32_t)box_rows, 2};
  cuuint32_t estr[3] = {1, 1, 1};
  CUresult r = enc(tm, CU_TENSOR_MAP_DATA_TYPE_BFLOAT16, plane_stride > 0 ? 3 : 2, const_cast<void*>(base), dims, strides,
                   box, estr, CU_TENSOR_MAP_INTERLEAVE_NONE, CU_TENSOR_MAP_SWIZZLE_128B,
                   CU_TENSOR_MAP_L2_PROMOTION_L2_256B, CU_TENSOR_MAP_FLOAT_OOB_FILL_NONE);
  SN_REQUIRE(r == CUDA_SUCCESS, "cuTensorMapEncodeTiled(weights) failed: %d (rows=%d K=%lld box_rows=%d)",
             (int)r, rows, k_total, box_rows);
  return SN_OK;
}

static void pick_patch(int m_h, int m_w, int rows, int* th, int* tw, int* nb) {
  int w = 16;
  while (w > 1 && w / 2 >= m_w) w /= 2;
  if (w > rows) w = rows;
  int h = rows / w;
  while (h > 1 && h / 2 >= m_h) h /= 2;
  *tw = w;
  *th = h;
  *nb = rows / (w * h);
}

static void pick_patch_conv(int m_n, int m_h, int m_w, int* th, int* tw, int* nb) {
  double best_eff = -1.0;
  int best_perim = 1 << 30, best_rows = 0, best_area = 0;
  const long long useful = (long long)m_n * m_h * m_w;
  for (int w = 1; w <= m_w && w <= 128; ++w) {
    for (int h = 1; h <= m_h && h * w <= 128; ++h) {
      int n = 1;
      if (m_h * m_w < 128) {
        if (w != m_w || h != m_h) continue;
        n = 128 / (w * h);
        if (n > m_n) n = m_n;
        if (n > 256) n = 256;
      }
      const long long tiles = (long long)((m_w + w - 1) / w) * ((m_h + h - 1) / h) * ((m_n + n - 1) / n);
      const double eff = (double)useful / (double)(tiles * 128);
      const int rows = w * h * n, perim = w + h, area = w * h;
      const bool better =
          eff > best_eff + 1e-9 ||
          (eff > best_eff - 1e-9 &&
           (rows > best_rows ||
            (rows == best_rows && (area > best_area || (area == best_area && (perim < best_perim || (perim == best_perim && w > *tw)))))));
      if (better) {
        best_eff = eff; best_rows = rows; best_perim = perim; best_area = area;
        *tw = w; *th = h; *nb = n;
      }
    }
  }
}

int sn_tap_gemm_plan_init(TapGemmPlan* plan, const sn_tap_gemm_desc* d) {
  memset(plan, 0, sizeof(*plan));
  TapGemmParams& p = plan->p;
  SN_REQUIRE(d->nsplit == 1 || d->nsplit == 3, "nsplit must be 1 or 3");
  SN_REQUIRE(d->ntaps >= 1 && d->ntaps <= SN_MAX_TAPS, "ntaps out of range: %d", d->ntaps);
  const int a_chunk = d->a_chunk ? d->a_chunk : 64;
  SN_REQUIRE(a_chunk == 64 || a_chunk == 32 || a_chunk == 16, "a_chunk must be 64, 32 or 16");
  if (a_chunk == 64) {
    SN_REQUIRE(d->k_per_tap > 0 && d->k_per_tap % 64 == 0, "k_per_tap must be a multiple of 64");
  } else {
    SN_REQUIRE(d->k_per_tap == a_chunk && d->ntaps % (64 / a_chunk) == 0,
               "narrow operand: k_per_tap must equal a_chunk (%d) and ntaps (%d) be a multiple of %d", a_chunk,
               d->ntaps, 64 / a_chunk);
  }
  p.a_chunk = a_chunk;
  SN_REQUIRE(d->block_n >= 16 && d->block_n <= 128 && d->block_n % 16 == 0,
             "block_n must be a multiple of 16 in [16,128]");
  SN_REQUIRE(d->a_hi && d->b_hi && d->out, "null operand");
  SN_REQUIRE(d->nsplit == 1 || (d->a_lo && d->b_lo), "nsplit=3 needs lo planes");
  SN_REQUIRE(d->a_fmt == d->b_fmt, "A and B of one wgmma must share a 16-bit format (a=%d b=%d)",
             d->a_fmt, d->b_fmt);
  int th, tw, nb;
  pick_patch_conv(d->m_n, d->m_h, d->m_w, &th, &tw, &nb);
  p.a_rows = th * tw * nb;
  p.tw = tw; p.th = th; p.nb = nb;
  p.tiles_w = (d->m_w + tw - 1) / tw;
  p.tiles_h = (d->m_h + th - 1) / th;
  p.tiles_n = (d->m_n + nb - 1) / nb;
  p.m_w = d->m_w; p.m_h = d->m_h; p.m_n = d->m_n;
  p.ntaps = d->ntaps;
  p.chunks = a_chunk == 64 ? d->k_per_tap / 64 : 1;
  for (int t = 0; t < d->ntaps; ++t) {
    p.taps[t].c_off = d->taps[t].c_off;
    p.taps[t].kb_off = d->taps[t].kb_off;
    p.taps[t].dw = (short)d->taps[t].dw;
    p.taps[t].dh = (short)d->taps[t].dh;
    p.taps[t].hp = (short)d->taps[t].hp;
  }
  p.block_n = d->block_n;
  p.n_valid = d->n_valid;
  p.out = d->out;
  p.out_sn = d->out_sn; p.out_sh = d->out_sh; p.out_sw = d->out_sw;
  p.omh = d->out_mul_h; p.ooh = d->out_off_h; p.omw = d->out_mul_w; p.oow = d->out_off_w;
  p.nphase = d->nphase == 4 ? 4 : 1;
  SN_REQUIRE(d->nphase == 0 || d->nphase == 1 || d->nphase == 4, "nphase must be 1 or 4");
  if (p.nphase == 4) {
    SN_REQUIRE(d->ntaps % 4 == 0, "4-phase launch: ntaps must split into 4 equal groups");
    const int tpp = d->ntaps / 4;
    SN_REQUIRE(a_chunk == 64 || tpp % (64 / a_chunk) == 0, "4-phase launch: taps per phase must fill whole stages");
  }
  p.bias = d->bias;
  p.stack_slot = d->stack_slot; p.stack_c = d->stack_c;
  p.stats = nullptr;
  if (d->stack_slot > 0)
    SN_REQUIRE(d->nphase <= 1 && d->n_valid == 4 * d->stack_slot && d->stack_c >= 1 && d->stack_c <= d->stack_slot &&
                   d->out_mul_h == 2 && d->out_mul_w == 2,
               "phase-stacked output: n_valid = 4*stack_slot, nphase 1, out_mul 2 (slot=%d c=%d n_valid=%d)",
               d->stack_slot, d->stack_c, d->n_valid);
  p.b_scale = d->b_scale;
  p.a_fmt = d->a_fmt;
  p.b_fmt = d->b_fmt;
  p.act = d->act;
  p.vec4 = ((uintptr_t)d->out % 16 == 0) && (d->out_sn % 4 == 0) && (d->out_sh % 4 == 0) &&
           (d->out_sw % 4 == 0) && (!d->bias || (uintptr_t)d->bias % 16 == 0);
  if (d->stats && nb == 1 && p.vec4 && d->n_valid % 16 == 0 && d->act == 0 && d->stack_slot == 0 && d->m_n * 1 >= 1)
    p.stats = d->stats;
  plan->stats_bytes = p.stats ? sizeof(double) * 2 * (size_t)d->m_n * d->n_valid : 0;
  p.tile_counter = nullptr;
  SN_CHECK_CUDA(cudaMalloc(&p.tile_counter, 2 * sizeof(int)));
  SN_CHECK_CUDA(cudaMemset(p.tile_counter, 0, 2 * sizeof(int)));
  int rc;
  const void* a_pl[2] = {d->a_hi, d->a_lo};
  const void* b_pl[2] = {d->b_hi, d->b_lo};
  const long long a_ps = d->nsplit == 3 ? (const char*)d->a_lo - (const char*)d->a_hi : 0;
  const long long b_ps = d->nsplit == 3 ? (const char*)d->b_lo - (const char*)d->b_hi : 0;
  p.a_merged = a_chunk == 64 && a_ps > 0 && a_ps % 16 == 0 && p.a_rows % 8 == 0;
  if (p.a_merged && d->a_parity)
    for (int t = 0; t < d->ntaps; ++t) p.taps[t].c_off += p.taps[t].hp * d->a_w * d->a_pitch;
  p.b_merged = b_ps > 0 && b_ps % 16 == 0 && d->block_n % 8 == 0;
  p.a_lo_off = p.a_merged ? p.a_rows * 128 : kTileBytes;
  p.b_lo_off = p.b_merged ? d->block_n * 128 : kTileBytes;
  for (int pl = 0; pl < (d->nsplit == 3 ? 2 : 1); ++pl) {
    if (!(p.a_merged && pl == 1)) {
      rc = sn_make_act_map(&p.tmA[pl], a_pl[pl], d->a_n, d->a_h, d->a_w, d->a_c, d->a_pitch,
                           d->a_parity, tw, th, nb, a_chunk, p.a_merged ? a_ps : 0);
      if (rc) return rc;
    }
    if (!(p.b_merged && pl == 1)) {
      rc = sn_make_weight_map(&p.tmB[pl], b_pl[pl], d->b_rows, d->b_k, d->block_n, p.b_merged ? b_ps : 0);
      if (rc) return rc;
    }
  }
  if (p.a_merged) p.tmA[1] = p.tmA[0];
  if (p.b_merged) p.tmB[1] = p.tmB[0];
  plan->nsplit = d->nsplit;
  plan->grid = dim3(p.tiles_w * p.tiles_h * p.tiles_n, (d->n_valid + d->block_n - 1) / d->block_n, p.nphase);
  return SN_OK;
}

static int mma_n(int block_n) {
  return block_n <= 16 ? 16 : block_n <= 32 ? 32 : block_n <= 64 ? 64 : block_n <= 96 ? 96 : 128;
}

template <int NSPLIT, int CW, int BN, bool F16>
static int launch_tap(const TapGemmPlan* plan, cudaStream_t stream) {
  static bool attr_done = false;
  if (!attr_done) {
    SN_CHECK_CUDA(cudaFuncSetAttribute(tap_gemm_kernel<NSPLIT, CW, BN, F16>, cudaFuncAttributeMaxDynamicSharedMemorySize,
                                       Cfg<NSPLIT>::kSmemBytes));
    attr_done = true;
  }
  static int sms = 0;
  if (sms == 0) {
    int dev = 0;
    SN_CHECK_CUDA(cudaGetDevice(&dev));
    SN_CHECK_CUDA(cudaDeviceGetAttribute(&sms, cudaDevAttrMultiProcessorCount, dev));
  }
  const int m_tiles = (int)plan->grid.x, n_tiles = (int)plan->grid.y;
  const int total = m_tiles * n_tiles * (int)plan->grid.z;
  if (plan->p.stats) SN_CHECK_CUDA(cudaMemsetAsync(plan->p.stats, 0, plan->stats_bytes, stream));
  const int ctas = total < sms ? total : sms;
  tap_gemm_kernel<NSPLIT, CW, BN, F16>
      <<<ctas, kThreads, Cfg<NSPLIT>::kSmemBytes, stream>>>(plan->p, m_tiles, n_tiles, total);
  SN_CHECK_CUDA(cudaGetLastError());
  return SN_OK;
}

template <int NSPLIT, int CW, bool F16>
static int launch_tap_n(const TapGemmPlan* plan, cudaStream_t stream) {
  switch (mma_n(plan->p.block_n)) {
    case 16: return launch_tap<NSPLIT, CW, 16, F16>(plan, stream);
    case 32: return launch_tap<NSPLIT, CW, 32, F16>(plan, stream);
    case 64: return launch_tap<NSPLIT, CW, 64, F16>(plan, stream);
    case 96: return launch_tap<NSPLIT, CW, 96, F16>(plan, stream);
    default: return launch_tap<NSPLIT, CW, 128, F16>(plan, stream);
  }
}

template <int NSPLIT, bool F16>
static int launch_tap_cw(const TapGemmPlan* plan, cudaStream_t stream) {
  const int cw = plan->p.a_chunk;
  if (cw == 64) return launch_tap_n<NSPLIT, 64, F16>(plan, stream);
  if (cw == 32) return launch_tap_n<NSPLIT, 32, F16>(plan, stream);
  return launch_tap_n<NSPLIT, 16, F16>(plan, stream);
}

int sn_tap_gemm_plan_launch(const TapGemmPlan* plan, cudaStream_t stream) {
  const bool f16 = plan->p.a_fmt == SN_FMT_F16;
  if (plan->nsplit == 3) return f16 ? launch_tap_cw<3, true>(plan, stream) : launch_tap_cw<3, false>(plan, stream);
  return f16 ? launch_tap_cw<1, true>(plan, stream) : launch_tap_cw<1, false>(plan, stream);
}

static int wgrad_ksplit(const sn_wgrad_desc* d, int base_ctas, int total, int sm_count) {
  if (d->deterministic) sm_count = SN_NUM_SMS;
  int ks = d->ksplit;
  if (ks <= 0) {
    ks = (3 * sm_count + base_ctas - 1) / base_ctas;
    int max_ks = total / 8;
    if (max_ks < 1) max_ks = 1;
    if (ks > max_ks) ks = max_ks;
    if (ks < 1) ks = 1;
  }
  if (ks > total) ks = total;
  return ks;
}

int sn_wgrad_plan_init(WgradPlan* plan, const sn_wgrad_desc* d, int sm_count) {
  memset(plan, 0, sizeof(*plan));
  WgradParams& p = plan->p;
  SN_REQUIRE(d->nsplit == 1 || d->nsplit == 3, "nsplit must be 1 or 3");
  SN_REQUIRE(d->ntaps >= 1 && d->ntaps <= SN_MAX_TAPS, "ntaps out of range: %d", d->ntaps);
  const int y_chunk = d->y_chunk ? d->y_chunk : 64;
  SN_REQUIRE(y_chunk == 64 || y_chunk == 32 || y_chunk == 16, "y_chunk must be 64, 32 or 16");
  p.y_chunk = y_chunk;
  p.ngroups = 0;
  int grid_y = d->ntaps;
  if (y_chunk == 64) {
    SN_REQUIRE(d->block_n == 64 || d->block_n == 128, "wgrad block_n must be 64 or 128 for 64-channel Y rows");
  } else {
    SN_REQUIRE(d->cols_valid <= y_chunk, "narrow Y: cols_valid must fit one %d-channel block", y_chunk);
    if (d->ngroups > 0) {
      int maxg = 0, covered = 0;
      for (int g = 0; g < d->ngroups; ++g) {
        SN_REQUIRE(d->group_size[g] >= 1 && d->group_start[g] >= 0 &&
                       d->group_start[g] + d->group_size[g] <= d->ntaps, "bad tap group %d", g);
        if (d->group_size[g] > maxg) maxg = d->group_size[g];
        covered += d->group_size[g];
        p.gstart[g] = (short)d->group_start[g];
        p.gsize[g] = (short)d->group_size[g];
      }
      SN_REQUIRE(covered == d->ntaps && maxg * y_chunk <= 128 && d->block_n == maxg * y_chunk,
                 "tap groups must cover all taps and block_n == max group * y_chunk <= 128");
      p.ngroups = d->ngroups;
      grid_y = d->ngroups;
    } else {
      SN_REQUIRE(d->block_n == y_chunk, "narrow Y without groups: block_n must equal y_chunk");
    }
  }
  SN_REQUIRE(d->x_hi && d->y_hi && d->out, "null operand");
  SN_REQUIRE(d->nsplit == 1 || (d->x_lo && d->y_lo), "nsplit=3 needs lo planes");
  SN_REQUIRE(d->x_fmt == d->y_fmt, "X and Y of one wgmma must share a 16-bit format (x=%d y=%d)",
             d->x_fmt, d->y_fmt);
  int th, tw, nb;
  pick_patch(d->m_h, d->m_w, 64, &th, &tw, &nb);
  p.tw = tw; p.th = th; p.nb = nb;
  p.tiles_w = (d->m_w + tw - 1) / tw;
  p.tiles_h = (d->m_h + th - 1) / th;
  p.tiles_n = (d->m_n + nb - 1) / nb;
  p.ntaps = d->ntaps;
  for (int t = 0; t < d->ntaps; ++t) {
    p.xtaps[t].c_off = d->xtaps[t].c_off; p.xtaps[t].dw = (short)d->xtaps[t].dw;
    p.xtaps[t].dh = (short)d->xtaps[t].dh; p.xtaps[t].hp = (short)d->xtaps[t].hp;
    p.ytaps[t].c_off = d->ytaps[t].c_off; p.ytaps[t].dw = (short)d->ytaps[t].dw;
    p.ytaps[t].dh = (short)d->ytaps[t].dh; p.ytaps[t].hp = (short)d->ytaps[t].hp;
    p.tap_off[t] = d->tap_off[t];
  }
  p.block_n = d->block_n;
  p.m_tiles = (d->rows_valid + kBlockM - 1) / kBlockM;
  p.n_tiles = y_chunk == 64 ? (d->cols_valid + d->block_n - 1) / d->block_n : 1;
  p.rows_valid = d->rows_valid;
  p.cols_valid = d->cols_valid;
  p.out = d->out;
  p.s_row = d->s_row;
  p.s_col = d->s_col;
  p.x_fmt = d->x_fmt;
  p.y_fmt = d->y_fmt;
  int rc;
  const void* x_pl[2] = {d->x_hi, d->x_lo};
  const void* y_pl[2] = {d->y_hi, d->y_lo};
  {
    const long long x_ps = d->nsplit == 3 ? (const char*)d->x_lo - (const char*)d->x_hi : 0;
    const long long y_ps = d->nsplit == 3 ? (const char*)d->y_lo - (const char*)d->y_hi : 0;
    p.x_merged = x_ps > 0 && x_ps % 16 == 0 && tw * th * nb == 64;
    p.y_merged = y_ps > 0 && y_ps % 16 == 0 && tw * th * nb == 64 && y_chunk == 64 && d->ngroups == 0;
    for (int t = 0; t < d->ntaps; ++t) {
      if (p.x_merged && d->x_parity) p.xtaps[t].c_off += p.xtaps[t].hp * d->x_w * d->x_pitch;
      if (p.y_merged && d->y_parity) p.ytaps[t].c_off += p.ytaps[t].hp * d->y_w * d->y_pitch;
    }
    for (int pl = 0; pl < (d->nsplit == 3 ? 2 : 1); ++pl) {
      if (!(p.x_merged && pl == 1)) {
        rc = sn_make_act_map(&p.tmX[pl], x_pl[pl], d->x_n, d->x_h, d->x_w, d->x_c, d->x_pitch,
                             d->x_parity, tw, th, nb, 64, p.x_merged ? x_ps : 0);
        if (rc) return rc;
      }
      if (!(p.y_merged && pl == 1)) {
        rc = sn_make_act_map(&p.tmY[pl], y_pl[pl], d->y_n, d->y_h, d->y_w, d->y_c, d->y_pitch,
                             d->y_parity, tw, th, nb, y_chunk, p.y_merged ? y_ps : 0);
        if (rc) return rc;
      }
    }
    if (p.x_merged) p.tmX[1] = p.tmX[0];
    if (p.y_merged) p.tmY[1] = p.tmY[0];
  }
  plan->nsplit = d->nsplit;
  const int base_ctas = p.m_tiles * p.n_tiles * grid_y;
  const int total = p.tiles_w * p.tiles_h * p.tiles_n;
  const int ks = wgrad_ksplit(d, base_ctas, total, sm_count);
  plan->grid = dim3(p.m_tiles * p.n_tiles, grid_y, ks);
  p.det_ws = nullptr;
  p.det_count = 0;
  plan->ws_bytes = 0;
  if (d->deterministic) {
    for (int t = 0; t < d->ntaps; ++t)
      for (int u = 0; u < t; ++u)
        SN_REQUIRE(d->tap_off[t] != d->tap_off[u], "deterministic wgrad: taps %d and %d share tap_off", u, t);
    p.det_count = (long long)d->ntaps * d->rows_valid * d->cols_valid;
    plan->ws_bytes = sizeof(float) * (size_t)ks * p.det_count;
    SN_CHECK_CUDA(cudaMalloc(&p.det_ws, plan->ws_bytes));
  }
  return SN_OK;
}

int sn_wgrad_plan_ksplit(const sn_wgrad_desc* d, int sm_count) {
  SN_REQUIRE(d && d->ntaps >= 1 && d->ntaps <= SN_MAX_TAPS, "wgrad_ksplit: bad descriptor");
  int th, tw, nb;
  pick_patch(d->m_h, d->m_w, 64, &th, &tw, &nb);
  const int total = ((d->m_w + tw - 1) / tw) * ((d->m_h + th - 1) / th) * ((d->m_n + nb - 1) / nb);
  const int y_chunk = d->y_chunk ? d->y_chunk : 64;
  const int grid_y = (y_chunk != 64 && d->ngroups > 0) ? d->ngroups : d->ntaps;
  const int m_tiles = (d->rows_valid + kBlockM - 1) / kBlockM;
  const int n_tiles = y_chunk == 64 ? (d->cols_valid + d->block_n - 1) / d->block_n : 1;
  return wgrad_ksplit(d, m_tiles * n_tiles * grid_y, total, sm_count);
}

template <int NSPLIT, int BN, bool F16, bool DET>
static int launch_wgrad_k(const WgradPlan* plan, cudaStream_t stream) {
  static bool attr_done = false;
  if (!attr_done) {
    SN_CHECK_CUDA(cudaFuncSetAttribute(wgrad_gemm_kernel<NSPLIT, BN, F16, DET>,
                                       cudaFuncAttributeMaxDynamicSharedMemorySize, Cfg<NSPLIT>::kSmemBytes));
    attr_done = true;
  }
  wgrad_gemm_kernel<NSPLIT, BN, F16, DET><<<plan->grid, kThreads, Cfg<NSPLIT>::kSmemBytes, stream>>>(plan->p);
  SN_CHECK_CUDA(cudaGetLastError());
  return SN_OK;
}

template <int NSPLIT, int BN, bool F16>
static int launch_wgrad(const WgradPlan* plan, cudaStream_t stream) {
  if (!plan->p.det_ws) return launch_wgrad_k<NSPLIT, BN, F16, false>(plan, stream);
  const int rc = launch_wgrad_k<NSPLIT, BN, F16, true>(plan, stream);
  if (rc) return rc;
  long long g = (plan->p.det_count + 255) / 256;
  if (g > SN_NUM_SMS * 8) g = SN_NUM_SMS * 8;
  wgrad_det_sum_kernel<<<(int)g, 256, 0, stream>>>(plan->p, (int)plan->grid.z);
  SN_CHECK_CUDA(cudaGetLastError());
  sn_count_launch(1);
  return SN_OK;
}

template <int NSPLIT, bool F16>
static int launch_wgrad_n(const WgradPlan* plan, cudaStream_t stream) {
  switch (mma_n(plan->p.block_n)) {
    case 16: return launch_wgrad<NSPLIT, 16, F16>(plan, stream);
    case 32: return launch_wgrad<NSPLIT, 32, F16>(plan, stream);
    case 64: return launch_wgrad<NSPLIT, 64, F16>(plan, stream);
    case 96: return launch_wgrad<NSPLIT, 96, F16>(plan, stream);
    default: return launch_wgrad<NSPLIT, 128, F16>(plan, stream);
  }
}

int sn_wgrad_plan_launch(const WgradPlan* plan, cudaStream_t stream) {
  const bool f16 = plan->p.x_fmt == SN_FMT_F16;
  if (plan->nsplit == 3) return f16 ? launch_wgrad_n<3, true>(plan, stream) : launch_wgrad_n<3, false>(plan, stream);
  return f16 ? launch_wgrad_n<1, true>(plan, stream) : launch_wgrad_n<1, false>(plan, stream);
}
```

### swapnet_b200/csrc/plan.h

```cpp
#pragma once
#include <cuda.h>
#include <cuda_runtime.h>
#include "../../include/swapnet_b200.h"

struct TapDesc {
  int c_off;
  int kb_off;
  short dw, dh, hp, _pad;
};

struct alignas(64) TapGemmParams {
  CUtensorMap tmA[2];
  CUtensorMap tmB[2];
  TapDesc taps[SN_MAX_TAPS];
  int ntaps, chunks;
  int tiles_w, tiles_h, tiles_n;
  int tw, th, nb;
  int a_rows;
  int m_w, m_h, m_n;
  int block_n, n_valid;
  float* out;
  long long out_sn, out_sh, out_sw;
  int omh, ooh, omw, oow;
  const float* bias;
  const float* b_scale;
  int act;
  int vec4;
  int a_fmt, b_fmt;
  int a_chunk;
  int nphase;
  int a_merged, b_merged;
  int a_lo_off, b_lo_off;
  int stack_slot, stack_c;
  double* stats;
  int* tile_counter;
};

struct alignas(64) WgradParams {
  CUtensorMap tmX[2];
  CUtensorMap tmY[2];
  TapDesc xtaps[SN_MAX_TAPS];
  TapDesc ytaps[SN_MAX_TAPS];
  long long tap_off[SN_MAX_TAPS];
  int ntaps;
  int tiles_w, tiles_h, tiles_n;
  int tw, th, nb;
  int m_tiles, n_tiles, block_n;
  int rows_valid, cols_valid;
  float* out;
  long long s_row, s_col;
  int x_fmt, y_fmt;
  int y_chunk;
  int ngroups;
  int x_merged, y_merged;
  short gstart[SN_MAX_TAPS], gsize[SN_MAX_TAPS];
  float* det_ws;
  long long det_count;
};

struct TapGemmPlan {
  TapGemmParams p;
  dim3 grid;
  int nsplit;
  size_t stats_bytes;
};
struct WgradPlan {
  WgradParams p;
  dim3 grid;
  int nsplit;
  size_t ws_bytes;
};

int sn_tap_gemm_plan_init(TapGemmPlan* plan, const sn_tap_gemm_desc* d);
int sn_tap_gemm_plan_launch(const TapGemmPlan* plan, cudaStream_t stream);
int sn_wgrad_plan_init(WgradPlan* plan, const sn_wgrad_desc* d, int sm_count);
int sn_wgrad_plan_launch(const WgradPlan* plan, cudaStream_t stream);
int sn_wgrad_plan_ksplit(const sn_wgrad_desc* d, int sm_count);
```

### swapnet_b200/lowering.py

```python
from __future__ import annotations

from dataclasses import dataclass, field
from typing import List, Tuple

KINDS = ("conv4s2", "convT4s2", "conv3r", "conv4s1", "head", "conv3z")

@dataclass
class Tap:
    pw: int
    kb: int
    dw: int
    dh: int
    hp: int = 0


@dataclass
class GemmSpec:
    parity: bool
    m_h: int
    m_w: int
    taps: List[Tap]
    out_mul: Tuple[int, int] = (1, 1)
    out_off: Tuple[int, int] = (0, 0)
    w_phase: int = 0
    a_hw: Tuple[int, int] = (0, 0)


@dataclass
class WgradSpec:
    m_h: int
    m_w: int
    x_parity: bool
    y_parity: bool
    xtaps: List[Tap]
    ytaps: List[Tap]
    x_is: str = "dy"
    tap_ids: List[int] = field(default_factory=list)


def _phase_taps():
    out = []
    for py in range(2):
        khs = [(1, 0), (3, -1)] if py == 0 else [(0, 1), (2, 0)]
        for px in range(2):
            kws = [(1, 0), (3, -1)] if px == 0 else [(0, 1), (2, 0)]
            out.append(((py, px), [(kh, dh, kw, dw) for kh, dh in khs for kw, dw in kws]))
    return out


def phase_major_slots() -> List[int]:
    slot = [0] * 16
    for p, (_, taps) in enumerate(_phase_taps()):
        for j, (kh, _, kw, _) in enumerate(taps):
            slot[kh * 4 + kw] = p * 4 + j
    return slot


def pack_slots(kind: str, dgrad: bool) -> List[int]:
    if (kind == "convT4s2" and not dgrad) or (kind == "conv4s2" and dgrad):
        return phase_major_slots()
    return list(range(ntaps(kind)))


def _s2_tap(k: int) -> Tuple[int, int]:
    return ((k - 1) >> 1, (k - 1) & 1)


def out_hw(kind: str, h: int, w: int) -> Tuple[int, int]:
    if kind == "conv4s2":
        return h // 2, w // 2
    if kind == "convT4s2":
        return 2 * h, 2 * w
    if kind in ("conv3r", "conv3z"):
        return h, w
    if kind == "conv4s1":
        return h - 1, w - 1
    if kind == "head":
        return 2 * h, 2 * w
    raise ValueError(kind)


def ntaps(kind: str) -> int:
    return {"conv4s2": 16, "convT4s2": 16, "conv3r": 9, "conv4s1": 16, "head": 25, "conv3z": 9}[kind]


HEAD_PHASE_OFF = (0, 4, 10, 16)


def head_neff(par: int) -> int:
    return 3 if par else 2


def forward_specs(kind: str, h: int, w: int) -> List[GemmSpec]:
    if kind == "conv4s2":
        taps = []
        for kh in range(4):
            dh, hp = _s2_tap(kh)
            for kw in range(4):
                dw, pw = _s2_tap(kw)
                taps.append(Tap(pw, kh * 4 + kw, dw, dh, hp))
        return [GemmSpec(True, h // 2, w // 2, taps, a_hw=(h, w))]
    if kind == "convT4s2":
        slot = phase_major_slots()
        return [GemmSpec(False, h, w, [Tap(0, slot[kh * 4 + kw], dw, dh) for kh, dh, kw, dw in taps], (2, 2),
                         (py, px), a_hw=(h, w)) for (py, px), taps in _phase_taps()]
    if kind == "conv3r":
        taps = [Tap(0, kh * 3 + kw, kw, kh) for kh in range(3) for kw in range(3)]
        return [GemmSpec(False, h, w, taps, a_hw=(h + 2, w + 2))]
    if kind == "conv4s1":
        taps = [Tap(0, kh * 4 + kw, kw - 1, kh - 1) for kh in range(4) for kw in range(4)]
        return [GemmSpec(False, h - 1, w - 1, taps, a_hw=(h, w))]
    if kind == "conv3z":
        taps = [Tap(0, kh * 3 + kw, kw - 1, kh - 1) for kh in range(3) for kw in range(3)]
        return [GemmSpec(False, h, w, taps, a_hw=(h, w))]
    if kind == "head":
        specs = []
        for py in range(2):
            for px in range(2):
                taps = []
                for ey in range(head_neff(py)):
                    for ex in range(head_neff(px)):
                        taps.append(Tap(0, ey * head_neff(px) + ex, ex - 1, ey - 1))
                specs.append(GemmSpec(False, h, w, taps, (2, 2), (py, px), w_phase=2 * py + px, a_hw=(h, w)))
        return specs
    raise ValueError(kind)


HEAD_SLOT = 24


def head_stacked_spec(h: int, w: int) -> GemmSpec:
    taps = [Tap(0, (sy + 1) * 3 + (sx + 1), sx, sy) for sy in (-1, 0, 1) for sx in (-1, 0, 1)]
    return GemmSpec(False, h, w, taps, (2, 2), (0, 0), a_hw=(h, w))


def dgrad_specs(kind: str, h: int, w: int) -> List[GemmSpec]:
    oh, ow = out_hw(kind, h, w)
    if kind == "conv4s2":
        slot = phase_major_slots()
        return [GemmSpec(False, oh, ow, [Tap(0, slot[kh * 4 + kw], dw, dh) for kh, dh, kw, dw in taps], (2, 2),
                         (py, px), a_hw=(oh, ow)) for (py, px), taps in _phase_taps()]
    if kind == "convT4s2":
        taps = []
        for kh in range(4):
            dh, hp = _s2_tap(kh)
            for kw in range(4):
                dw, pw = _s2_tap(kw)
                taps.append(Tap(pw, kh * 4 + kw, dw, dh, hp))
        return [GemmSpec(True, h, w, taps, a_hw=(oh, ow))]
    if kind == "conv3r":
        taps = [Tap(0, kh * 3 + kw, -kw, -kh) for kh in range(3) for kw in range(3)]
        return [GemmSpec(False, h + 2, w + 2, taps, a_hw=(oh, ow))]
    if kind == "conv4s1":
        taps = [Tap(0, kh * 4 + kw, 1 - kw, 1 - kh) for kh in range(4) for kw in range(4)]
        return [GemmSpec(False, h, w, taps, a_hw=(oh, ow))]
    if kind == "conv3z":
        taps = [Tap(0, kh * 3 + kw, 1 - kw, 1 - kh) for kh in range(3) for kw in range(3)]
        return [GemmSpec(False, h, w, taps, a_hw=(oh, ow))]
    if kind == "head":
        taps = []
        for py in range(2):
            for px in range(2):
                for ey in range(head_neff(py)):
                    for ex in range(head_neff(px)):
                        te = HEAD_PHASE_OFF[2 * py + px] + ey * head_neff(px) + ex
                        taps.append(Tap(px, te, -(ex - 1), -(ey - 1), py))
        return [GemmSpec(True, h, w, taps, a_hw=(oh, ow))]
    raise ValueError(kind)


def wgrad_specs(kind: str, h: int, w: int) -> List[WgradSpec]:
    oh, ow = out_hw(kind, h, w)
    zero = Tap(0, 0, 0, 0, 0)
    if kind == "conv4s2":
        yt = []
        for kh in range(4):
            dh, hp = _s2_tap(kh)
            for kw in range(4):
                dw, pw = _s2_tap(kw)
                yt.append(Tap(pw, 0, dw, dh, hp))
        return [WgradSpec(oh, ow, False, True, [zero] * 16, yt, "dy", list(range(16)))]
    if kind == "convT4s2":
        yt = []
        for kh in range(4):
            dh, hp = _s2_tap(kh)
            for kw in range(4):
                dw, pw = _s2_tap(kw)
                yt.append(Tap(pw, 0, dw, dh, hp))
        return [WgradSpec(h, w, False, True, [zero] * 16, yt, "in", list(range(16)))]
    if kind == "conv3r":
        yt = [Tap(0, 0, kw, kh) for kh in range(3) for kw in range(3)]
        return [WgradSpec(h, w, False, False, [zero] * 9, yt, "dy", list(range(9)))]
    if kind == "conv4s1":
        yt = [Tap(0, 0, kw - 1, kh - 1) for kh in range(4) for kw in range(4)]
        return [WgradSpec(oh, ow, False, False, [zero] * 16, yt, "dy", list(range(16)))]
    if kind == "conv3z":
        yt = [Tap(0, 0, kw - 1, kh - 1) for kh in range(3) for kw in range(3)]
        return [WgradSpec(oh, ow, False, False, [zero] * 9, yt, "dy", list(range(9)))]
    if kind == "head":
        xt, yt, ids = [], [], []
        for py in range(2):
            for px in range(2):
                for ey in range(head_neff(py)):
                    for ex in range(head_neff(px)):
                        xt.append(Tap(px, 0, 0, 0, py))
                        yt.append(Tap(0, 0, ex - 1, ey - 1))
                        ids.append(HEAD_PHASE_OFF[2 * py + px] + ey * head_neff(px) + ex)
        return [WgradSpec(h, w, True, False, xt, yt, "dy", ids)]
    raise ValueError(kind)


def pack_strides(kind: str, cin: int, cout: int, dgrad: bool) -> Tuple[int, int, int, int]:
    t = ntaps(kind)
    if kind == "convT4s2":
        if not dgrad:
            return t, cout * t, cout, cin
        return cout * t, t, cin, cout
    if not dgrad:
        return cin * t, t, cout, cin
    return t, cin * t, cin, cout


def wgrad_out_strides(kind: str, cin: int, cout: int, x_is_dy: bool) -> Tuple[int, int]:
    t = ntaps(kind)
    if kind == "head":
        co_s, ci_s = 25 * cin, 1
    elif kind == "convT4s2":
        ci_s, co_s = cout * t, t
    else:
        co_s, ci_s = cin * t, t
    return (co_s, ci_s) if x_is_dy else (ci_s, co_s)


def pad64(c: int) -> int:
    return (c + 63) // 64 * 64


def padc(c: int) -> int:
    if c <= 16:
        return 16
    if c <= 32:
        return 32
    return pad64(c)


def pick_block_n(n_valid: int) -> int:
    if n_valid >= 128:
        return 128
    for b in (16, 32, 64, 128):
        if n_valid <= b:
            return b
    return 128
```

### swapnet_b200/ops.py

```python
from __future__ import annotations

import ctypes as C
from dataclasses import dataclass
from typing import Optional, Sequence, Tuple

import torch

from . import _lib
from . import lowering as L

from ._lib import (ACT_LRELU, ACT_NONE, ACT_RELU, ACT_TANH, FMT_BF16, FMT_F16, LAYOUT_LABEL_U8, LAYOUT_MASK_I32,
                   LAYOUT_NCHW, LAYOUT_NHWC, SnGradSrc, SnNormActBwdDesc, SnNormActDesc, SnTap, SnTapGemmDesc,
                   SnWgradDesc, check)

IN_EPS = 1e-5


def _stream() -> int:
    return torch.cuda.current_stream().cuda_stream


def _ptr(t: Optional[torch.Tensor]) -> Optional[int]:
    return None if t is None else t.data_ptr()


class Planes:

    def __init__(self, n: int, h: int, w: int, pitch: int, device, c: Optional[int] = None, c_off: int = 0,
                 hi: Optional[torch.Tensor] = None, lo: Optional[torch.Tensor] = None, fmt: int = FMT_F16,
                 dual: bool = False, twin: Optional["Planes"] = None):
        assert pitch % 8 == 0
        self.fmt = fmt
        self.twin = twin
        if dual and twin is None:
            self.twin = Planes(n, h, w, pitch, device, c, c_off, fmt=FMT_BF16)
        self.n, self.h, self.w, self.pitch = n, h, w, pitch
        self.c = pitch if c is None else c
        self.c_off = c_off
        if hi is None:
            assert lo is None
            buf = torch.zeros(2, n, h, w, pitch, dtype=torch.bfloat16, device=device)
            hi, lo = buf[0], buf[1]
        self.hi, self.lo = hi, lo

    def slice(self, c_off: int, c: int) -> "Planes":
        assert c_off + c <= self.pitch
        return Planes(self.n, self.h, self.w, self.pitch, self.hi.device, c, self.c_off + c_off, self.hi, self.lo,
                      self.fmt, twin=None if self.twin is None else self.twin.slice(c_off, c))

    def batch_slice(self, n0: int, n: int) -> "Planes":
        return Planes(n, self.h, self.w, self.pitch, self.hi.device, self.c, self.c_off, self.hi[n0:n0 + n],
                      self.lo[n0:n0 + n], self.fmt, twin=None if self.twin is None else self.twin.batch_slice(n0, n))

    @property
    def hi_ptr(self) -> int:
        return self.hi.data_ptr() + 2 * self.c_off

    @property
    def lo_ptr(self) -> int:
        return self.lo.data_ptr() + 2 * self.c_off

    def dense(self) -> torch.Tensor:
        s = slice(self.c_off, self.c_off + self.c)
        if self.fmt == FMT_F16:
            return self.hi[..., s].view(torch.float16).float() + self.lo[..., s].view(torch.float16).float()
        return self.hi[..., s].float() + self.lo[..., s].float()


class PackedWeights:

    def __init__(self, rows: int, k_total: int, device, scale: Optional[torch.Tensor] = None, fmt: int = FMT_F16):
        self.rows, self.k_total = rows, k_total
        self.fmt = fmt
        self.scale = scale if (scale is not None and fmt == FMT_F16) else None
        buf = torch.zeros(2, rows, k_total, dtype=torch.bfloat16, device=device)
        self.hi, self.lo = buf[0], buf[1]


class DetWorkspace:

    def __init__(self, device):
        self.device = torch.device(device)
        self._buf: Optional[torch.Tensor] = None

    @property
    def nbytes(self) -> int:
        return 0 if self._buf is None else self._buf.numel() * self._buf.element_size()

    def get(self, elems: int, dtype=torch.float64) -> torch.Tensor:
        nb = elems * torch.tensor([], dtype=dtype).element_size()
        if nb > self.nbytes:
            if self.device.type == "cuda" and torch.cuda.is_current_stream_capturing():
                raise RuntimeError("DetWorkspace: a CUDA-graph capture cannot grow the workspace; run the step eagerly "
                                   "first")
            self._buf = torch.empty((nb + 7) // 8, dtype=torch.float64, device=self.device)
        return self._buf.view(dtype)

    def slots(self, n: int, c: int) -> torch.Tensor:
        return self.get(int(_lib.load().sn_det_slots(n, c)))


class Plan:

    def __init__(self, handle: int, keep: Sequence, tag=None):
        self.handle = handle
        self.tag = tag
        self._keep = list(keep)

    @property
    def workspace_bytes(self) -> int:
        return int(_lib.load().sn_plan_workspace_bytes(self.handle))

    @property
    def has_stats(self) -> bool:
        return bool(_lib.load().sn_plan_has_stats(self.handle))

    trace = None

    def run(self) -> None:
        if Plan.trace is None:
            check(_lib.load().sn_plan_run(self.handle, _stream()))
            return
        e0, e1 = torch.cuda.Event(enable_timing=True), torch.cuda.Event(enable_timing=True)
        e0.record()
        check(_lib.load().sn_plan_run(self.handle, _stream()))
        e1.record()
        Plan.trace.append((self, e0, e1))

    def __del__(self):
        try:
            if self.handle:
                _lib.load().sn_plan_destroy(self.handle)
        except Exception:
            pass


def _fill_tap(dst: SnTap, tap: L.Tap, pitch: int, k_pad: int, c_base: int = 0) -> None:
    dst.c_off = tap.pw * pitch + c_base
    dst.kb_off = tap.kb * k_pad
    dst.dw, dst.dh, dst.hp = tap.dw, tap.dh, tap.hp


def tap_gemm_desc(a: Planes, spec: L.GemmSpec, w: PackedWeights, k_per_tap: int, out: torch.Tensor,
                  n_valid: int, *, w_row_off: int = 0, w_rows: Optional[int] = None,
                  w_k: Optional[int] = None, w_elem_off: int = 0, bias: Optional[torch.Tensor] = None,
                  act: int = ACT_NONE, nsplit: int = 3, block_n: Optional[int] = None,
                  out_c_off: int = 0, nphase: int = 1, stack_slot: int = 0, stack_c: int = 0,
                  stats: Optional[torch.Tensor] = None) -> SnTapGemmDesc:
    assert (a.h, a.w) == tuple(spec.a_hw), f"operand is {a.h}x{a.w}, spec wants {spec.a_hw}"
    assert a.c_off % 8 == 0 and k_per_tap <= a.c
    narrow = k_per_tap < 64
    assert (k_per_tap in (16, 32)) if narrow else (k_per_tap % 64 == 0)
    taps = list(spec.taps)
    if narrow and nphase == 4:
        assert (len(taps) // 4) % (64 // k_per_tap) == 0, "4-phase narrow launch: taps per phase must fill whole stages"
    elif narrow:
        tps = 64 // k_per_tap
        kb_next = max(t.kb for t in taps) + 1
        while len(taps) % tps:
            taps.append(L.Tap(taps[0].pw, kb_next, taps[0].dw, taps[0].dh, taps[0].hp))
            kb_next += 1
    d = SnTapGemmDesc()
    d.a_chunk = k_per_tap if narrow else 64
    d.a_hi, d.a_lo = a.hi_ptr, a.lo_ptr
    d.a_n, d.a_h, d.a_w, d.a_c, d.a_pitch = a.n, a.h, a.w, a.c, a.pitch
    d.a_parity = 1 if spec.parity else 0
    d.a_fmt, d.b_fmt = a.fmt, w.fmt
    d.b_scale = None if w.scale is None else w.scale.data_ptr()
    d.b_hi = w.hi.data_ptr() + 2 * w_elem_off
    d.b_lo = w.lo.data_ptr() + 2 * w_elem_off
    d.b_rows = w.rows if w_rows is None else w_rows
    d.b_k = w.k_total if w_k is None else w_k
    d.m_n, d.m_h, d.m_w = a.n, spec.m_h, spec.m_w
    d.ntaps, d.k_per_tap = len(taps), k_per_tap
    for i, t in enumerate(taps):
        _fill_tap(d.taps[i], t, a.pitch, k_per_tap)
    assert out.dtype == torch.float32 and out.dim() == 4 and (out.shape[3] == 1 or out.stride(3) == 1)
    d.out = out.data_ptr() + 4 * out_c_off
    d.out_sn, d.out_sh, d.out_sw = out.stride(0), out.stride(1), out.stride(2)
    d.out_mul_h, d.out_mul_w = spec.out_mul
    d.out_off_h, d.out_off_w = spec.out_off
    d.n_valid = n_valid
    d.block_n = block_n or L.pick_block_n(n_valid)
    d.bias = _ptr(bias)
    d.act = act
    d.nsplit = nsplit
    d.nphase = nphase
    d.stack_slot, d.stack_c = stack_slot, stack_c
    if stats is not None:
        assert stats.dtype == torch.float64 and stats.numel() >= a.n * n_valid * 2 and out_c_off == 0
        d.stats = stats.data_ptr()
    return d


def merge_phase_specs(specs) -> Optional[L.GemmSpec]:
    if len(specs) != 4:
        return None
    s0 = specs[0]
    n = len(s0.taps)
    for z, s in enumerate(specs):
        if (s.parity, s.m_h, s.m_w, s.out_mul, s.a_hw, len(s.taps)) != (s0.parity, s0.m_h, s0.m_w, s0.out_mul, s0.a_hw, n):
            return None
        if s.out_off != (z >> 1, z & 1) or s.w_phase != 0:
            return None
    return L.GemmSpec(s0.parity, s0.m_h, s0.m_w, [t for s in specs for t in s.taps], s0.out_mul, (0, 0), 0, s0.a_hw)


def tap_gemm_plan(desc: SnTapGemmDesc, keep: Sequence = ()) -> Plan:
    h = C.c_void_p()
    check(_lib.load().sn_tap_gemm_plan_create(C.byref(desc), C.byref(h)))
    return Plan(h.value, keep)


def tap_gemm_simt(desc: SnTapGemmDesc) -> None:
    check(_lib.load().sn_tap_gemm_simt(C.byref(desc), _stream()))


def wgrad_desc(x: Planes, y: Planes, spec: L.WgradSpec, out: torch.Tensor, s_row: int, s_col: int,
               tap_off: Sequence[int], rows_valid: int, cols_valid: int, *, swap: bool = False,
               nsplit: int = 3, block_n: Optional[int] = None, ksplit: int = 0,
               deterministic: bool = False) -> SnWgradDesc:
    xt, yt = spec.xtaps, spec.ytaps
    xp, yp = spec.x_parity, spec.y_parity
    if swap:
        x, y, xt, yt, xp, yp = y, x, yt, xt, yp, xp
        s_row, s_col = s_col, s_row
        rows_valid, cols_valid = cols_valid, rows_valid
    assert x.c_off % 8 == 0 and y.c_off % 8 == 0
    order = list(range(len(xt)))
    groups = []
    if y.c < 64:
        gmax = 128 // y.c
        key = lambda i: (xt[i].pw, xt[i].dw, xt[i].dh, xt[i].hp)
        order = sorted(order, key=key)
        i = 0
        while i < len(order):
            j = i
            while j < len(order) and j - i < gmax and key(order[j]) == key(order[i]):
                j += 1
            groups.append((i, j - i))
            i = j
        xt = [xt[i] for i in order]
        yt = [yt[i] for i in order]
        tap_off = [tap_off[i] for i in order]
    d = SnWgradDesc()
    d.x_hi, d.x_lo = x.hi_ptr, x.lo_ptr
    d.x_n, d.x_h, d.x_w, d.x_c, d.x_pitch, d.x_parity = x.n, x.h, x.w, x.c, x.pitch, int(xp)
    d.x_fmt, d.y_fmt = x.fmt, y.fmt
    d.y_hi, d.y_lo = y.hi_ptr, y.lo_ptr
    d.y_n, d.y_h, d.y_w, d.y_c, d.y_pitch, d.y_parity = y.n, y.h, y.w, y.c, y.pitch, int(yp)
    d.m_n, d.m_h, d.m_w = x.n, spec.m_h, spec.m_w
    d.ntaps = len(xt)
    for i in range(len(xt)):
        _fill_tap(d.xtaps[i], xt[i], x.pitch, 0)
        _fill_tap(d.ytaps[i], yt[i], y.pitch, 0)
        d.tap_off[i] = tap_off[i]
    assert out.dtype == torch.float32
    d.out = out.data_ptr()
    d.s_row, d.s_col = s_row, s_col
    d.rows_valid, d.cols_valid = rows_valid, cols_valid
    assert x.c >= 64, "the 128-row operand of a wgrad GEMM must carry >= 64 channels (swap the roles)"
    if y.c < 64:
        assert y.c in (16, 32) and cols_valid <= y.c
        d.y_chunk = y.c
        d.ngroups = len(groups)
        for g, (st, sz) in enumerate(groups):
            d.group_start[g], d.group_size[g] = st, sz
        d.block_n = max(sz for _, sz in groups) * y.c
    else:
        d.y_chunk = 64
        d.block_n = block_n or (128 if cols_valid > 64 else 64)
    d.ksplit = ksplit
    d.nsplit = nsplit
    d.deterministic = int(deterministic)
    return d


def wgrad_ksplit(desc: SnWgradDesc, sm_count: int) -> int:
    k = _lib.load().sn_wgrad_ksplit(C.byref(desc), sm_count)
    if k <= 0:
        check(k)
    return int(k)


def wgrad_plan(desc: SnWgradDesc, keep: Sequence = ()) -> Plan:
    h = C.c_void_p()
    check(_lib.load().sn_wgrad_plan_create(C.byref(desc), C.byref(h)))
    return Plan(h.value, keep)


class SegMap:

    def __init__(self, data: torch.Tensor, channels: int):
        assert data.dim() == 3 and data.dtype in (torch.uint8, torch.int32), "uint8 label map or int32 bit mask [n,h,w]"
        assert channels <= (32 if data.dtype == torch.int32 else 256)
        self.data, self.channels = data.contiguous(), channels
        self.layout = LAYOUT_LABEL_U8 if data.dtype == torch.uint8 else LAYOUT_MASK_I32

    @property
    def shape(self):
        n, h, w = self.data.shape
        return (n, self.channels, h, w)

    @property
    def is_cuda(self):
        return self.data.is_cuda

    def dense(self) -> torch.Tensor:
        ch = torch.arange(self.channels, device=self.data.device).view(1, -1, 1, 1)
        d = self.data.unsqueeze(1)
        if self.layout == LAYOUT_LABEL_U8:
            return ((d.long() == ch) & (ch > 0)).float()
        return ((d.long() >> ch) & 1).float()

    @staticmethod
    def from_dense(t: torch.Tensor) -> "SegMap":
        assert t.dim() == 4 and t.shape[1] <= 32
        b = t != 0
        if not torch.equal(b.to(t.dtype), t):
            raise ValueError("SegMap.from_dense: tensor is not 0/1-valued")
        c = t.shape[1]
        if int(b.sum(1).max()) <= 1 and not bool(b[:, 0].any()):
            return SegMap(b.to(torch.uint8).mul(torch.arange(c, dtype=torch.uint8, device=t.device).view(1, -1, 1, 1))
                          .sum(1, dtype=torch.uint8), c)
        w = (1 << torch.arange(c, dtype=torch.int64, device=t.device)).view(1, -1, 1, 1)
        return SegMap((b.long() * w).sum(1).to(torch.int32), c)


def _src_args(t, nhwc: bool):
    if isinstance(t, SegMap):
        n, h, w = t.data.shape
        return t.data.data_ptr(), t.layout, 0, t.channels, (n, h, w)
    assert t.dtype == torch.float32
    if nhwc:
        n, h, w, c = t.shape
        return t.data_ptr(), LAYOUT_NHWC, _pitch(t), c, (n, h, w)
    assert t.is_contiguous()
    n, c, h, w = t.shape
    return t.data_ptr(), LAYOUT_NCHW, 0, c, (n, h, w)


def pack_planes(src, dst: Planes, *, nhwc: bool = False) -> None:
    if isinstance(src, SegMap):
        ptr, layout, _, c, (n, h, w) = _src_args(src, False)
        assert c <= dst.c and (n, h, w) == (dst.n, dst.h, dst.w)
        for d_ in ((dst,) if dst.twin is None else (dst, dst.twin)):
            check(_lib.load().sn_pack_planes(ptr, layout, 0, n, c, h, w, d_.hi_ptr, d_.lo_ptr, d_.pitch, 0, d_.fmt,
                                             _stream()))
        return
    assert src.dtype == torch.float32
    if nhwc:
        n, h, w, sp = src.shape
        assert src.stride(3) == 1 and src.stride(2) == sp
        c = dst.c
        for d_ in ((dst,) if dst.twin is None else (dst, dst.twin)):
            check(_lib.load().sn_pack_planes(src.data_ptr(), LAYOUT_NHWC, sp, n, c, h, w, d_.hi_ptr, d_.lo_ptr,
                                             d_.pitch, 0, d_.fmt, _stream()))
    else:
        assert src.is_contiguous()
        n, c, h, w = src.shape
        assert c <= dst.c
        for d_ in ((dst,) if dst.twin is None else (dst, dst.twin)):
            check(_lib.load().sn_pack_planes(src.data_ptr(), LAYOUT_NCHW, 0, n, c, h, w, d_.hi_ptr, d_.lo_ptr,
                                             d_.pitch, 0, d_.fmt, _stream()))
    assert (n, h, w) == (dst.n, dst.h, dst.w)


def pack_concat(srcs, dst: Planes, lead: int = 0) -> None:
    assert 1 <= len(srcs) <= 2 and dst.c % 8 == 0 and dst.c_off % 8 == 0 and lead >= 0
    args = [lead]
    for t, nhwc in srcs:
        ptr, layout, pitch, c, nhw = _src_args(t, nhwc)
        args += [ptr, layout, pitch, c]
        assert nhw == (dst.n, dst.h, dst.w)
    if len(srcs) == 1:
        args += [None, 0, 0, 0]
    tw = dst.twin
    check(_lib.load().sn_pack_concat(*args, dst.n, dst.h, dst.w, dst.c, dst.hi.data_ptr(), dst.lo.data_ptr(),
                                     None if tw is None else tw.hi.data_ptr(), None if tw is None else tw.lo.data_ptr(),
                                     dst.pitch, dst.c_off, dst.fmt, FMT_BF16 if tw is None else tw.fmt, _stream()))


class PackTable:

    def __init__(self, device):
        self.device = device
        self._scales, self._packs, self._keep = [], [], []
        self._dev = None

    def add_scale(self, weight: torch.Tensor, scale: torch.Tensor) -> None:
        assert weight.is_contiguous() and weight.dtype == torch.float32 and self._dev is None
        assert weight.data_ptr() % 16 == 0, "weight_scale_multi reads float4: the weight must be 16-byte aligned"
        it = _lib.SnScaleItem()
        it.w, it.count, it.scale2 = weight.data_ptr(), weight.numel(), scale.data_ptr()
        self._scales.append(it)
        self._keep += [weight, scale]

    def add_pack(self, weight: torch.Tensor, kind: str, dgrad: bool, k_pad: int, dst: PackedWeights) -> None:
        assert weight.is_contiguous() and weight.dtype == torch.float32 and self._dev is None
        if kind == "convT4s2":
            cin, cout = weight.shape[0], weight.shape[1]
        else:
            cout, cin = weight.shape[0], weight.shape[1]
        s_row, s_k, rows, k_real = L.pack_strides(kind, cin, cout, dgrad)
        t = L.ntaps(kind)
        assert dst.rows >= rows and dst.k_total >= t * k_pad and k_pad >= k_real and dst.k_total % k_pad == 0 and t <= 16
        it = _lib.SnPackItem()
        it.src, it.s_row, it.s_k = weight.data_ptr(), s_row, s_k
        it.rows, it.taps, it.taps_pitch, it.k_real, it.k_pad, it.fmt = rows, t, dst.k_total // k_pad, k_real, k_pad, dst.fmt
        it.hi, it.lo = dst.hi.data_ptr(), dst.lo.data_ptr()
        it.scale2 = None if dst.scale is None else dst.scale.data_ptr()
        for i, sl in enumerate(L.pack_slots(kind, dgrad)):
            it.slot[i] = sl
        self._packs.append(it)
        self._keep += [weight, dst]

    def _upload(self, items, ctype):
        arr = (ctype * len(items))(*items)
        return torch.frombuffer(bytearray(bytes(arr)), dtype=torch.uint8).to(self.device)

    def finalize(self) -> None:
        lib = _lib.load()
        rpb, kpb = lib.sn_pack_rows_per_block(), lib.sn_pack_k_per_block()
        begin = 0
        for it in self._packs:
            it.block_begin = begin
            begin += ((it.rows + rpb - 1) // rpb) * ((it.k_pad + kpb - 1) // kpb)
        self._blocks = begin
        self._max_taps = max([it.taps for it in self._packs], default=1)
        self._dev = (self._upload(self._scales, _lib.SnScaleItem) if self._scales else None,
                     self._upload(self._packs, _lib.SnPackItem) if self._packs else None,
                     torch.zeros(2 * max(1, len(self._scales)), dtype=torch.int32, device=self.device))

    def run(self) -> None:
        if self._dev is None:
            self.finalize()
        sc, pk, scratch = self._dev
        lib = _lib.load()
        if sc is not None:
            check(lib.sn_weight_scale_multi(sc.data_ptr(), len(self._scales), scratch.data_ptr(), _stream()))
        if pk is not None:
            check(lib.sn_pack_weights_multi(pk.data_ptr(), len(self._packs), self._blocks, self._max_taps, _stream()))


def pack_head_weights(weight: torch.Tensor, rows_pad: int, k_pad: int, dgrad: bool, dst: PackedWeights) -> None:
    cout, cin = weight.shape[:2]
    assert dst.hi.numel() >= (cin * 25 * k_pad if dgrad else rows_pad * 25 * k_pad)
    taps_pitch = dst.k_total // k_pad if dgrad else 25
    check(_lib.load().sn_pack_head_weights(weight.data_ptr(), cout, cin, rows_pad, k_pad, int(dgrad), taps_pitch,
                                           dst.hi.data_ptr(), dst.lo.data_ptr(), dst.fmt,
                                           None if dst.scale is None else dst.scale.data_ptr(), _stream()))


def pack_head_stacked(weight: torch.Tensor, slot: int, k_pad: int, dst: PackedWeights) -> None:
    cout, cin = weight.shape[:2]
    assert dst.rows == 4 * slot and dst.k_total == 9 * k_pad and slot >= cout and k_pad >= cin
    check(_lib.load().sn_pack_head_stacked(weight.data_ptr(), cout, cin, slot, k_pad, dst.hi.data_ptr(),
                                           dst.lo.data_ptr(), dst.fmt,
                                           None if dst.scale is None else dst.scale.data_ptr(), _stream()))


def fold_head_wgrad(geff: torch.Tensor, cout: int, cin: int, dw: torch.Tensor) -> None:
    check(_lib.load().sn_fold_head_wgrad(geff.data_ptr(), cout, cin, dw.data_ptr(), _stream()))


def _pitch(t: torch.Tensor) -> int:
    assert t.dim() == 4 and (t.shape[3] == 1 or t.stride(3) == 1)
    n, h, w, c = t.shape
    if w > 1:
        p = t.stride(2)
    elif h > 1:
        p = t.stride(1)
    elif n > 1:
        p = t.stride(0)
    else:
        p = c
    assert t.stride(1) == w * p or h == 1, "not an NHWC-contiguous pixel grid"
    assert t.stride(0) == h * w * p or n == 1, "not an NHWC-contiguous pixel grid"
    return p


def plane_stats(y: torch.Tensor, c: int, stats: torch.Tensor, eps: float = IN_EPS,
                ws: Optional[DetWorkspace] = None) -> None:
    n, h, w, _ = y.shape
    pitch = _pitch(y)
    assert stats.dtype == torch.float64 and stats.numel() >= n * c * 2
    if ws is not None:
        sl = ws.slots(n, c)
        check(_lib.load().sn_plane_stats_det(y.data_ptr(), pitch, n, h * w, c, eps, stats.data_ptr(), sl.data_ptr(),
                                             sl.numel(), _stream()))
        return
    check(_lib.load().sn_plane_stats(y.data_ptr(), pitch, n, h * w, c, eps, stats.data_ptr(), _stream()))


def stats_finalize(stats: torch.Tensor, count: int, hw: int, eps: float = IN_EPS) -> None:
    check(_lib.load().sn_stats_finalize(stats.data_ptr(), count, hw, eps, _stream()))


def plane_sums(y: torch.Tensor, c: int, stats: torch.Tensor, ws: Optional[DetWorkspace] = None) -> None:
    n, h, w, _ = y.shape
    assert stats.dtype == torch.float64 and stats.numel() >= n * c * 2
    if ws is not None:
        sl = ws.slots(n, c)
        check(_lib.load().sn_plane_sums_det(y.data_ptr(), _pitch(y), n, h * w, c, stats.data_ptr(), sl.data_ptr(),
                                            sl.numel(), _stream()))
        return
    check(_lib.load().sn_plane_sums(y.data_ptr(), _pitch(y), n, h * w, c, stats.data_ptr(), _stream()))


def bn_finalize(stats: torch.Tensor, n: int, c: int, groups: int, hw: int, bn: "torch.nn.BatchNorm2d") -> None:
    assert stats.dtype == torch.float64 and n % groups == 0
    assert bn.momentum is not None, "BatchNorm2d(momentum=None) (cumulative average) is not provided"
    track = bn.track_running_stats
    check(_lib.load().sn_bn_finalize(stats.data_ptr(), n, c, groups, hw, float(bn.eps), float(bn.momentum),
                                     _ptr(bn.running_mean if track else None), _ptr(bn.running_var if track else None),
                                     _ptr(bn.num_batches_tracked if track else None), _stream()))


def bn_group_sums(stats: torch.Tensor, n: int, c: int, groups: int, hw: int, part: torch.Tensor) -> None:
    assert stats.dtype == part.dtype == torch.float64 and n % groups == 0 and part.numel() >= groups * c * 3
    check(_lib.load().sn_bn_group_sums(stats.data_ptr(), n, c, groups, hw, part.data_ptr(), _stream()))


def bn_finalize_gathered(stats: torch.Tensor, n: int, c: int, groups: int, gathered: torch.Tensor,
                         bn: "torch.nn.BatchNorm2d") -> None:
    assert stats.dtype == gathered.dtype == torch.float64 and n % groups == 0
    assert gathered.dim() == 4 and tuple(gathered.shape[1:]) == (groups, c, 3) and gathered.is_contiguous()
    assert bn.momentum is not None, "BatchNorm2d(momentum=None) (cumulative average) is not provided"
    track = bn.track_running_stats
    check(_lib.load().sn_bn_finalize_gathered(stats.data_ptr(), n, c, groups, gathered.data_ptr(), gathered.shape[0],
                                              float(bn.eps), float(bn.momentum),
                                              _ptr(bn.running_mean if track else None),
                                              _ptr(bn.running_var if track else None),
                                              _ptr(bn.num_batches_tracked if track else None), _stream()))


def bn_eval_stats(stats: torch.Tensor, n: int, c: int, bn: "torch.nn.BatchNorm2d") -> None:
    assert stats.dtype == torch.float64
    check(_lib.load().sn_bn_eval_stats(stats.data_ptr(), n, c, bn.running_mean.data_ptr(), bn.running_var.data_ptr(),
                                       float(bn.eps), _stream()))


def norm_act_fwd(y: torch.Tensor, c: int, stats: Optional[torch.Tensor], act: int, slope: float = 0.2,
                 drop_p: float = 0.0, drop_seed: int = 0, residual: Optional[torch.Tensor] = None,
                 out: Optional[Planes] = None, reflect_pad: bool = False,
                 out_f32: Optional[torch.Tensor] = None, drop_offset: int = 0,
                 seed_dev: Optional[torch.Tensor] = None, stage_id: int = 0,
                 gamma: Optional[torch.Tensor] = None, beta: Optional[torch.Tensor] = None) -> None:
    n, h, w, _ = y.shape
    pitch = _pitch(y)
    d = SnNormActDesc()
    d.y, d.y_pitch = y.data_ptr(), pitch
    d.n, d.h, d.w, d.c = n, h, w, c
    d.stats = _ptr(stats)
    d.act, d.slope = act, slope
    d.drop_p, d.drop_seed = drop_p, drop_seed
    d.drop_offset, d.drop_step_seed_dev, d.drop_stage_id = drop_offset, _ptr(seed_dev), stage_id
    if residual is not None:
        d.residual, d.res_pitch = residual.data_ptr(), _pitch(residual)
    if out is not None:
        if reflect_pad:
            assert (out.h, out.w) == (h + 2, w + 2)
        else:
            assert (out.h, out.w) == (h, w)
        assert out.c >= c and out.n == n
        d.out_hi, d.out_lo, d.out_pitch, d.out_coff = out.hi.data_ptr(), out.lo.data_ptr(), out.pitch, out.c_off
        d.out_reflect_pad = int(reflect_pad)
        d.out_fmt = out.fmt
        if out.twin is not None:
            d.out2_hi, d.out2_lo, d.out2_fmt = out.twin.hi.data_ptr(), out.twin.lo.data_ptr(), out.twin.fmt
    if out_f32 is not None:
        d.out_f32, d.f32_pitch = out_f32.data_ptr(), _pitch(out_f32)
    d.gamma, d.beta = _ptr(gamma), _ptr(beta)
    check(_lib.load().sn_norm_act_fwd(C.byref(d), _stream()))


@dataclass
class GradSrc:
    t: torch.Tensor
    c_off: int = 0
    reflect_padded: bool = False
    up: int = 1
    act: int = -1


def _fill_srcs(arr, srcs: Sequence[GradSrc]) -> None:
    assert 1 <= len(srcs) <= _lib.SN_MAX_SRC
    for i, s in enumerate(srcs):
        assert s.t.dtype == torch.float32 and (s.t.shape[3] == 1 or s.t.stride(3) == 1)
        arr[i].ptr = s.t.data_ptr()
        arr[i].pitch = _pitch(s.t)
        arr[i].c_off = s.c_off
        arr[i].reflect_padded = int(s.reflect_padded)
        arr[i].up = s.up
        arr[i].act = s.act


def norm_act_bwd(srcs: Sequence[GradSrc], y: torch.Tensor, c: int, stats: Optional[torch.Tensor], act: int,
                 dy: Planes, gstats: Optional[torch.Tensor] = None, slope: float = 0.2, drop_p: float = 0.0,
                 drop_seed: int = 0, drop_offset: int = 0, seed_dev: Optional[torch.Tensor] = None,
                 stage_id: int = 0, bias_grad: Optional[torch.Tensor] = None,
                 bn: Optional[Tuple[torch.Tensor, torch.Tensor]] = None, bn_groups: int = 1, bn_train: bool = True,
                 bn_grads: Optional[Tuple[torch.Tensor, torch.Tensor]] = None,
                 ws: Optional[DetWorkspace] = None, bn_phase: int = 0, bn_gathered: Optional[torch.Tensor] = None,
                 bn_rank: int = 0) -> None:
    n, h, w, _ = y.shape
    pitch = _pitch(y)
    d = SnNormActBwdDesc()
    _fill_srcs(d.src, srcs)
    d.nsrc = len(srcs)
    d.y, d.y_pitch = y.data_ptr(), pitch
    d.n, d.h, d.w, d.c = n, h, w, c
    d.stats = _ptr(stats)
    d.act, d.slope = act, slope
    d.drop_p, d.drop_seed = drop_p, drop_seed
    d.drop_offset, d.drop_step_seed_dev, d.drop_stage_id = drop_offset, _ptr(seed_dev), stage_id
    d.gstats = _ptr(gstats)
    assert (dy.n, dy.h, dy.w) == (n, h, w) and dy.c >= c
    d.dy_hi, d.dy_lo, d.dy_pitch, d.dy_coff = dy.hi.data_ptr(), dy.lo.data_ptr(), dy.pitch, dy.c_off
    d.dy_fmt = dy.fmt
    d.bias_grad = _ptr(bias_grad)
    if bn is not None:
        d.gamma, d.beta = bn[0].data_ptr(), bn[1].data_ptr()
        d.bn_groups, d.bn_train = bn_groups, int(bn_train)
        if bn_grads is not None:
            d.gamma_grad, d.beta_grad = bn_grads[0].data_ptr(), bn_grads[1].data_ptr()
    if ws is not None and stats is not None:
        sl = ws.slots(n, c)
        d.det_slots, d.det_slots_cap = sl.data_ptr(), sl.numel()
    d.bn_phase = bn_phase
    if bn_gathered is not None:
        assert bn_gathered.dtype == torch.float64 and bn_gathered.is_contiguous()
        assert bn_gathered.dim() == 4 and tuple(bn_gathered.shape[1:]) == (bn_groups, c, 3)
        d.bn_gathered, d.bn_world, d.bn_rank = bn_gathered.data_ptr(), bn_gathered.shape[0], bn_rank
    check(_lib.load().sn_norm_act_bwd(C.byref(d), _stream()))


def fused_bias_grad_ok(c: int) -> bool:
    return c in (256, 512, 1024)


def bias_grad(dy: Planes, c: int, scratch: torch.Tensor, db: torch.Tensor, ws: Optional[DetWorkspace] = None) -> None:
    assert scratch.dtype == torch.float64 and scratch.numel() >= c and db.dtype == torch.float32
    if ws is not None:
        sl = ws.slots(1, c)
        check(_lib.load().sn_bias_grad_det(dy.hi.data_ptr(), dy.lo.data_ptr(), dy.pitch, dy.c_off, dy.fmt,
                                           dy.n * dy.h * dy.w, c, scratch.data_ptr(), db.data_ptr(), sl.data_ptr(),
                                           sl.numel(), _stream()))
        return
    check(_lib.load().sn_bias_grad(dy.hi.data_ptr(), dy.lo.data_ptr(), dy.pitch, dy.c_off, dy.fmt, dy.n * dy.h * dy.w, c,
                                   scratch.data_ptr(), db.data_ptr(), _stream()))


def sum_grads(srcs: Sequence[GradSrc], n: int, h: int, w: int, c: int, dst: torch.Tensor) -> None:
    arr = (SnGradSrc * _lib.SN_MAX_SRC)()
    _fill_srcs(arr, srcs)
    check(_lib.load().sn_sum_grads(arr, len(srcs), n, h, w, c, dst.data_ptr(), _pitch(dst), _stream()))


def tanh_bwd(srcs: Sequence[GradSrc], out: torch.Tensor, c: int, dy: Planes) -> None:
    n, h, w, _ = out.shape
    pitch = _pitch(out)
    arr = (SnGradSrc * _lib.SN_MAX_SRC)()
    _fill_srcs(arr, srcs)
    check(_lib.load().sn_tanh_bwd(arr, len(srcs), out.data_ptr(), pitch, n, h, w, c, dy.hi.data_ptr(),
                                  dy.lo.data_ptr(), dy.pitch, dy.c_off, dy.fmt, _stream()))


def upsample_planes(src: Planes, dst: Planes, factor: int) -> None:
    assert (dst.h, dst.w) == (src.h * factor, src.w * factor) and dst.c >= src.c and src.fmt == dst.fmt
    pairs = [(src, dst)]
    if src.twin is not None and dst.twin is not None:
        pairs.append((src.twin, dst.twin))
    for s_, d_ in pairs:
        check(_lib.load().sn_upsample_planes(s_.hi.data_ptr(), s_.lo.data_ptr(), s_.pitch, s_.c_off, dst.n, dst.h,
                                             dst.w, src.c, factor, d_.hi.data_ptr(), d_.lo.data_ptr(), d_.pitch,
                                             d_.c_off, _stream()))


def adamw_step(p: torch.Tensor, g: torch.Tensor, m: torch.Tensor, v: torch.Tensor, lr: float, b1: float, b2: float,
               eps: float, wd: float, step: int) -> None:
    assert p.is_contiguous() and g.is_contiguous() and p.numel() == g.numel() == m.numel() == v.numel()
    check(_lib.load().sn_adamw_step(p.data_ptr(), g.data_ptr(), m.data_ptr(), v.data_ptr(), p.numel(), lr, b1, b2, eps,
                                    wd, step, _stream()))


def adamw_hyper(lr: float, b1: float, b2: float, eps: float, wd: float, step: int, gscale: float = 1.0):
    out = (C.c_float * 8)()
    _lib.load().sn_adamw_hyper(lr, b1, b2, eps, wd, step, gscale, out)
    return list(out)


def adamw_step_dev(p: torch.Tensor, g: torch.Tensor, m: torch.Tensor, v: torch.Tensor, hyper_dev: torch.Tensor) -> None:
    assert p.is_contiguous() and g.is_contiguous() and p.numel() == g.numel() == m.numel() == v.numel()
    assert hyper_dev.dtype == torch.float32 and hyper_dev.numel() >= 8
    check(_lib.load().sn_adamw_step_dev(p.data_ptr(), g.data_ptr(), m.data_ptr(), v.data_ptr(), p.numel(),
                                        hyper_dev.data_ptr(), _stream()))


def adabound_step(p: torch.Tensor, g: torch.Tensor, m: torch.Tensor, v: torch.Tensor, lr: float, base_lr: float,
                  b1: float, b2: float, eps: float, wd: float, final_lr: float, gamma: float, step: int) -> None:
    assert p.is_contiguous() and g.is_contiguous() and p.numel() == g.numel() == m.numel() == v.numel()
    check(_lib.load().sn_adabound_step(p.data_ptr(), g.data_ptr(), m.data_ptr(), v.data_ptr(), p.numel(), lr, base_lr,
                                       b1, b2, eps, wd, final_lr, gamma, step, _stream()))


def adabound_hyper(lr: float, base_lr: float, b1: float, b2: float, eps: float, wd: float, final_lr: float,
                   gamma: float, step: int, gscale: float = 1.0):
    out = (C.c_float * 8)()
    _lib.load().sn_adabound_hyper(lr, base_lr, b1, b2, eps, wd, final_lr, gamma, step, gscale, out)
    return list(out)


def adabound_step_dev(p: torch.Tensor, g: torch.Tensor, m: torch.Tensor, v: torch.Tensor,
                      hyper_dev: torch.Tensor) -> None:
    assert p.is_contiguous() and g.is_contiguous() and p.numel() == g.numel() == m.numel() == v.numel()
    assert hyper_dev.dtype == torch.float32 and hyper_dev.numel() >= 8
    check(_lib.load().sn_adabound_step_dev(p.data_ptr(), g.data_ptr(), m.data_ptr(), v.data_ptr(), p.numel(),
                                           hyper_dev.data_ptr(), _stream()))


def set_step_params(dst: torch.Tensor, values) -> None:
    n = len(values)
    assert dst.dtype == torch.float32 and dst.numel() >= n and n <= 64
    arr = (C.c_float * n)(*values)
    check(_lib.load().sn_set_step_params(dst.data_ptr(), arr, n, _stream()))


def dropout_mask(seed: int, p: float, count: int, device) -> torch.Tensor:
    out = torch.empty(count, dtype=torch.uint8, device=device)
    check(_lib.load().sn_dropout_mask(seed, p, count, out.data_ptr(), _stream()))
    return out


def ce_loss_fwd_bwd(logits: torch.Tensor, c: int, target, weight: float,
                    loss_acc: torch.Tensor, grad: torch.Tensor) -> None:
    n, h, w, pitch = logits.shape
    if isinstance(target, SegMap):
        assert target.layout == LAYOUT_LABEL_U8 and target.shape == (n, c, h, w), "CE target: a uint8 label map"
        tptr, layout = target.data.data_ptr(), LAYOUT_LABEL_U8
    else:
        assert target.is_contiguous() and target.shape == (n, c, h, w)
        tptr, layout = target.data_ptr(), LAYOUT_NCHW
    check(_lib.load().sn_ce_loss_fwd_bwd(logits.data_ptr(), pitch, tptr, layout, n, h, w, c, weight,
                                         loss_acc.data_ptr(), grad.data_ptr(), grad.shape[3], _stream()))


def ce_tanh_bwd(out: torch.Tensor, c: int, target, weight: float, loss_acc: torch.Tensor,
                extra: Sequence[GradSrc], dy: Planes, ws: Optional[DetWorkspace] = None) -> None:
    n, h, w, pitch = out.shape
    if isinstance(target, SegMap):
        assert target.layout == LAYOUT_LABEL_U8 and target.shape == (n, c, h, w), "CE target: a uint8 label map"
        tptr, layout = target.data.data_ptr(), LAYOUT_LABEL_U8
    else:
        assert target.is_contiguous() and target.shape == (n, c, h, w)
        tptr, layout = target.data_ptr(), LAYOUT_NCHW
    arr = (SnGradSrc * _lib.SN_MAX_SRC)()
    if extra:
        _fill_srcs(arr, extra)
    assert (dy.n, dy.h, dy.w) == (n, h, w)
    args = (out.data_ptr(), pitch, tptr, layout, arr, len(extra), n, h, w, c, weight, loss_acc.data_ptr(),
            dy.hi.data_ptr(), dy.lo.data_ptr(), dy.pitch, dy.c_off, dy.fmt)
    if ws is not None:
        sl = ws.slots(1, 1)
        check(_lib.load().sn_ce_tanh_bwd_det(*args, sl.data_ptr(), sl.numel(), _stream()))
        return
    check(_lib.load().sn_ce_tanh_bwd(*args, _stream()))


def bce_logits_fwd_bwd(pred: torch.Tensor, halves: int, t0, t1: float, gscale: float,
                       loss_acc: torch.Tensor, dpred: Optional[torch.Tensor]) -> None:
    count = pred.numel() // halves
    if torch.is_tensor(t0):
        assert t0.dtype == torch.float32 and t0.numel() >= halves and t0.is_cuda
        check(_lib.load().sn_bce_logits_fwd_bwd_dev(pred.data_ptr(), count, halves, t0.data_ptr(), gscale,
                                                    loss_acc.data_ptr(), _ptr(dpred), _stream()))
        return
    check(_lib.load().sn_bce_logits_fwd_bwd(pred.data_ptr(), count, halves, t0, t1, gscale, loss_acc.data_ptr(),
                                            _ptr(dpred), _stream()))


GAN_BCE, GAN_MSE, GAN_WGAN = 0, 1, 2
GAN_OBJECTIVES = {"vanilla": GAN_BCE, "lsgan": GAN_MSE, "wgan": GAN_WGAN}


def gan_loss_fwd_bwd(objective: int, pred: torch.Tensor, halves: int, t, gscale: float, loss_acc: torch.Tensor,
                     dpred: Optional[torch.Tensor], ws: Optional[DetWorkspace] = None) -> None:
    count = pred.numel() // halves
    if torch.is_tensor(t):
        assert objective != GAN_WGAN, "the WGAN signs are constants of the call, passed by value"
        assert t.dtype == torch.float32 and t.numel() >= halves and t.is_cuda
        t0 = t1 = 0.0
        tptr = t.data_ptr()
    else:
        assert len(t) == halves
        t0, t1, tptr = float(t[0]), float(t[-1]), None
    args = (objective, pred.data_ptr(), count, halves, t0, t1, tptr, gscale, loss_acc.data_ptr(), _ptr(dpred))
    if ws is not None:
        sl = ws.slots(1, halves)
        check(_lib.load().sn_gan_loss_fwd_bwd_det(*args, sl.data_ptr(), sl.numel(), _stream()))
        return
    check(_lib.load().sn_gan_loss_fwd_bwd_dev(*args, _stream()))


def l1_loss_fwd_bwd(a: torch.Tensor, c: int, b_nchw: torch.Tensor, weight: float, loss_acc: torch.Tensor,
                    grad: torch.Tensor, ws: Optional[DetWorkspace] = None) -> None:
    n, h, w, pitch = a.shape
    if ws is not None:
        sl = ws.slots(1, 1)
        check(_lib.load().sn_l1_loss_fwd_bwd_det(a.data_ptr(), pitch, b_nchw.data_ptr(), n, h, w, c, weight,
                                                 loss_acc.data_ptr(), grad.data_ptr(), grad.shape[3], sl.data_ptr(),
                                                 sl.numel(), _stream()))
        return
    check(_lib.load().sn_l1_loss_fwd_bwd(a.data_ptr(), pitch, b_nchw.data_ptr(), n, h, w, c, weight,
                                         loss_acc.data_ptr(), grad.data_ptr(), grad.shape[3], _stream()))


def roi_align_pack(tex_nchw: torch.Tensor, rois: torch.Tensor, pool: int, out_f32: Optional[torch.Tensor],
                   out_planes: Optional[Planes]) -> None:
    b, ch, h, w = tex_nchw.shape
    nroi = rois.shape[1]
    assert rois.shape == (b, nroi, 4) and rois.is_contiguous() and tex_nchw.is_contiguous()
    check(_lib.load().sn_roi_align_pack_fwd(
        tex_nchw.data_ptr(), b, ch, h, w, rois.data_ptr(), nroi, pool, _ptr(out_f32),
        0 if out_f32 is None else out_f32.shape[3],
        None if out_planes is None else out_planes.hi.data_ptr(),
        None if out_planes is None else out_planes.lo.data_ptr(),
        0 if out_planes is None else out_planes.pitch, 0 if out_planes is None else out_planes.c_off,
        FMT_F16 if out_planes is None else out_planes.fmt, _stream()))


def augment_channels(src, channels: int, ops_dev: torch.Tensor, op_stride: int, max_ops: int, out: torch.Tensor,
                     tmp: Optional[torch.Tensor]) -> None:
    labels = src.dtype == torch.uint8
    assert src.is_cuda and src.is_contiguous() and out.is_contiguous() and out.dtype == torch.float32
    n, h, w = (src.shape[0], src.shape[-2], src.shape[-1])
    assert (src.dim() == 3) if labels else (src.dtype == torch.float32 and tuple(src.shape) == (n, channels, h, w))
    assert tuple(out.shape) == (n, channels, h, w) and (tmp is None or (tmp.shape == out.shape and tmp.dtype == out.dtype))
    assert ops_dev.is_cuda and ops_dev.dtype == torch.uint8 and ops_dev.numel() == n * channels * op_stride * 72
    check(_lib.load().sn_augment_channels(src.data_ptr() if labels else None, None if labels else src.data_ptr(),
                                          n, channels, h, w, ops_dev.data_ptr(), op_stride, max_ops, out.data_ptr(),
                                          _ptr(tmp), _stream()))


def launch_count() -> int:
    return int(_lib.load().sn_launch_count())


def count_replayed(n: int) -> None:
    _lib.load().sn_count_replayed(int(n))


def affine_pack(src: torch.Tensor, nhwc: bool, mul: float, add: float, dst: Planes) -> None:
    assert src.dtype == torch.float32 and dst.c == 16
    if nhwc:
        n, h, w, c = src.shape
        pitch = _pitch(src)
    else:
        assert src.is_contiguous()
        n, c, h, w = src.shape
        pitch = 0
    assert (n, h, w) == (dst.n, dst.h, dst.w)
    check(_lib.load().sn_affine_pack(src.data_ptr(), LAYOUT_NHWC if nhwc else LAYOUT_NCHW, pitch, n, c, h, w, mul, add,
                                     dst.hi.data_ptr(), dst.lo.data_ptr(), dst.pitch, dst.c_off, dst.fmt, _stream()))


def relu_pool_fwd(y: torch.Tensor, c: int, out: Planes) -> None:
    n, h, w, _ = y.shape
    assert (out.n, out.h, out.w) == (n, h // 2, w // 2) and out.c >= c
    check(_lib.load().sn_relu_pool_fwd(y.data_ptr(), _pitch(y), n, h, w, c, out.hi.data_ptr(), out.lo.data_ptr(),
                                       out.pitch, out.c_off, out.fmt, _stream()))


def relu_pool_bwd(y: torch.Tensor, c: int, g_pool: Optional[torch.Tensor], g_direct: Optional[torch.Tensor],
                  dy: Planes) -> None:
    n, h, w, _ = y.shape
    assert (dy.n, dy.h, dy.w) == (n, h, w) and dy.c >= c
    assert g_pool is None or g_pool.shape[:3] == (n, h // 2, w // 2)
    assert g_direct is None or g_direct.shape[:3] == (n, h, w)
    check(_lib.load().sn_relu_pool_bwd(y.data_ptr(), _pitch(y), _ptr(g_pool), 0 if g_pool is None else _pitch(g_pool),
                                       _ptr(g_direct), 0 if g_direct is None else _pitch(g_direct), n, h, w, c,
                                       dy.hi.data_ptr(), dy.lo.data_ptr(), dy.pitch, dy.c_off, dy.fmt, _stream()))


def feat_loss_fwd_bwd(y_out: torch.Tensor, y_tgt: torch.Tensor, c: int, weight: float, gscale: float,
                      loss_acc: torch.Tensor, dx: torch.Tensor, ws: Optional[DetWorkspace] = None) -> None:
    n, h, w, _ = y_out.shape
    assert y_tgt.shape[:3] == (n, h, w) and dx.shape[:3] == (n, h, w) and loss_acc.dtype == torch.float64
    args = (y_out.data_ptr(), _pitch(y_out), y_tgt.data_ptr(), _pitch(y_tgt), n * h * w, c, weight, gscale,
            loss_acc.data_ptr(), dx.data_ptr(), _pitch(dx))
    if ws is not None:
        sl = ws.slots(1, 1)
        check(_lib.load().sn_feat_loss_fwd_bwd_det(*args, sl.data_ptr(), sl.numel(), _stream()))
        return
    check(_lib.load().sn_feat_loss_fwd_bwd(*args, _stream()))


def _gram_strides(x: torch.Tensor, nhwc: bool):
    if nhwc:
        n, h, w, c = x.shape
        assert x.is_contiguous()
        return n, c, h * w, h * w * c, 1, c
    n, c, h, w = x.shape
    assert x.is_contiguous()
    return n, c, h * w, c * h * w, h * w, 1


def gram_rows(a: torch.Tensor, b: torch.Tensor, nhwc: bool, out: torch.Tensor,
              ws: Optional[DetWorkspace] = None) -> None:
    na, c, npix, an, ac, ap = _gram_strides(a, nhwc)
    nb, cb, npix_b, bn, bc, bp = _gram_strides(b, nhwc)
    assert (cb, npix_b) == (c, npix) and out.dtype == torch.float64 and out.shape == (na * c, nb * c)
    assert out.is_contiguous()
    args = (a.data_ptr(), an, ac, ap, na, b.data_ptr(), bn, bc, bp, nb, c, npix, out.data_ptr())
    if ws is not None:
        sl = ws.get(int(_lib.load().sn_gram_rows_det_slots(na * c, nb * c)))
        check(_lib.load().sn_gram_rows_det(*args, sl.data_ptr(), sl.numel(), _stream()))
        return
    check(_lib.load().sn_gram_rows(*args, _stream()))


def gram_rows_mse(g_out: torch.Tensor, g_tgt: torch.Tensor, weight: float, loss_acc: torch.Tensor, m: torch.Tensor,
                  gscale: float = 1.0) -> None:
    rows_l, rows = g_out.shape
    assert g_tgt.shape == g_out.shape and m.dtype == torch.float32 and m.shape == g_out.shape
    assert g_out.is_contiguous() and g_tgt.is_contiguous() and m.is_contiguous() and loss_acc.dtype == torch.float64
    check(_lib.load().sn_gram_rows_mse(g_out.data_ptr(), g_tgt.data_ptr(), rows_l, rows, weight, gscale,
                                       loss_acc.data_ptr(), m.data_ptr(), _stream()))


def gram_rows_bwd(m: torch.Tensor, x: torch.Tensor, nhwc: bool, dx: torch.Tensor, accumulate: bool) -> None:
    n, c, npix, sn, sc, sp = _gram_strides(x, nhwc)
    rows_l = m.shape[0]
    assert m.dtype == torch.float32 and m.is_contiguous() and m.shape[1] == n * c
    assert dx.shape[0] * c == rows_l and dx.shape[1] * dx.shape[2] == npix
    check(_lib.load().sn_gram_rows_bwd(m.data_ptr(), rows_l, x.data_ptr(), sn, sc, sp, n, c, npix, dx.data_ptr(),
                                       _pitch(dx), 1 if accumulate else 0, _stream()))


def tap_sum_fwd(p: torch.Tensor, k: int, pad: int, bias: Optional[torch.Tensor], y: torch.Tensor) -> None:
    n, h, w, _ = p.shape
    assert y.shape[:3] == (n, h + 2 * pad - k + 1, w + 2 * pad - k + 1)
    check(_lib.load().sn_tap_sum_fwd(p.data_ptr(), _pitch(p), n, h, w, k, pad, _ptr(bias), y.data_ptr(), _pitch(y),
                                     _stream()))


def to_one_fwd(x: Planes, weight: torch.Tensor, p: torch.Tensor) -> None:
    assert weight.is_contiguous() and weight.shape[0] == 1 and tuple(weight.shape[2:]) == (4, 4)
    assert p.dtype == torch.float32 and p.shape[:3] == (x.n, x.h, x.w) and x.c_off % 8 == 0
    check(_lib.load().sn_to_one_fwd(x.hi_ptr, x.lo_ptr, x.pitch, x.fmt, x.n * x.h * x.w, weight.shape[1],
                                    weight.data_ptr(), 4, p.data_ptr(), _pitch(p), _stream()))


def to_one_wgrad(x: Planes, dy: Planes, pad: int, dw: torch.Tensor, ws: Optional[DetWorkspace] = None) -> None:
    assert dw.is_contiguous() and dw.dtype == torch.float32 and (dy.h, dy.w) == (x.h + 2 * pad - 3, x.w + 2 * pad - 3)
    if ws is not None:
        sl = ws.get(int(_lib.load().sn_to_one_wgrad_det_slots(dw.shape[1])), torch.float32)
        check(_lib.load().sn_to_one_wgrad_det(x.hi_ptr, x.lo_ptr, x.pitch, x.fmt, x.n, x.h, x.w, dw.shape[1], dy.hi_ptr,
                                              dy.lo_ptr, dy.pitch, dy.fmt, 4, pad, dw.data_ptr(), sl.data_ptr(),
                                              sl.numel(), _stream()))
        return
    check(_lib.load().sn_to_one_wgrad(x.hi_ptr, x.lo_ptr, x.pitch, x.fmt, x.n, x.h, x.w, dw.shape[1], dy.hi_ptr,
                                      dy.lo_ptr, dy.pitch, dy.fmt, 4, pad, dw.data_ptr(), _stream()))


def to_one_dgrad(dy: Planes, weight: torch.Tensor, pad: int, dx: torch.Tensor) -> None:
    n, h, w, _ = dx.shape
    assert (dy.h, dy.w) == (h + 2 * pad - 3, w + 2 * pad - 3)
    check(_lib.load().sn_to_one_dgrad(dy.hi_ptr, dy.lo_ptr, dy.pitch, dy.fmt, n, h, w, weight.shape[1],
                                      weight.data_ptr(), 4, pad, dx.data_ptr(), _pitch(dx), _stream()))


def pixel_desc(x: Planes, net, scales: torch.Tensor, nsplit: int, **kw) -> "_lib.SnPixelDesc":
    d = _lib.SnPixelDesc()
    d.x_hi, d.x_lo = x.hi_ptr, x.lo_ptr
    if x.twin is not None:
        d.xb_hi, d.xb_lo = x.twin.hi_ptr, x.twin.lo_ptr
    d.x_pitch, d.x_c, d.n, d.hw, d.cin = x.pitch, x.c, x.n, x.h * x.w, net.input_nc
    c0, c2, c5 = net.net[0], net.net[2], net.net[5]
    d.w1, d.b1, d.w2, d.b2 = c0.weight.data_ptr(), c0.bias.data_ptr(), c2.weight.data_ptr(), _ptr(c2.bias)
    d.w3, d.b3 = c5.weight.data_ptr(), _ptr(c5.bias)
    d.scale1, d.scale2 = scales[0].data_ptr(), scales[1].data_ptr()
    d.norm, d.nsplit, d.slope, d.eps = int(net.norm == "instance"), nsplit, 0.2, IN_EPS
    for k, v in kw.items():
        setattr(d, k, v.data_ptr() if torch.is_tensor(v) else v)
    return d


def pixel_pass(name: str, d: "_lib.SnPixelDesc", ws: Optional[DetWorkspace] = None) -> None:
    lib = _lib.load()
    if ws is not None:
        sl = ws.get(int(lib.sn_pixel_det_slots(d.n, d.cin)))
        d.slots, d.slots_cap = sl.data_ptr(), sl.numel()
    else:
        d.slots, d.slots_cap = None, 0
    check(getattr(lib, "sn_pixel_" + name)(C.byref(d), _stream()))
```

Baseline: 137.5.

## Specialize wgrad kernel per tile shape with half-row and narrow-N variants

The weight-gradient GEMM kernel is templated on the per-warpgroup N width and a half-row mode. When 64 or fewer output rows remain, the two warpgroups split the columns instead of the rows, and narrow wgmma shapes (n8, n48) are added. The launcher issues one launch per shape present, each with its own k-split, and CTAs exit early if their shape does not match. This cuts padded MMA work on ragged tiles, and pick_block_n now prefers 96 when it pads less. The cost is extra launches, idle early-exit CTAs, and more kernel instantiations. A MAC-count query API is also added.

```diff
diff --git a/include/swapnet_b200.h b/include/swapnet_b200.h
--- a/include/swapnet_b200.h
+++ b/include/swapnet_b200.h
@@ -81,6 +81,8 @@
 int sn_plan_geometry(const sn_plan* plan, int* out);
 long long sn_plan_workspace_bytes(const sn_plan* plan);
 int sn_wgrad_ksplit(const sn_wgrad_desc* desc, int sm_count);
+long long sn_tap_gemm_mma_macs(const sn_tap_gemm_desc* desc);
+long long sn_wgrad_mma_macs(const sn_wgrad_desc* desc);
 
 int sn_pack_planes(const float* src, int src_layout, int src_pitch, int n, int c, int h, int w,
                    void* dst_hi, void* dst_lo, int dst_pitch, int dst_coff, int fmt, void* stream);
diff --git a/swapnet_b200/_lib.py b/swapnet_b200/_lib.py
--- a/swapnet_b200/_lib.py
+++ b/swapnet_b200/_lib.py
@@ -138,6 +138,8 @@
     "sn_plan_geometry": (_I, [_VP, C.POINTER(C.c_int)]),
     "sn_plan_workspace_bytes": (_LL, [_VP]),
     "sn_wgrad_ksplit": (_I, [C.POINTER(SnWgradDesc), _I]),
+    "sn_tap_gemm_mma_macs": (_LL, [C.POINTER(SnTapGemmDesc)]),
+    "sn_wgrad_mma_macs": (_LL, [C.POINTER(SnWgradDesc)]),
     "sn_det_slots": (_LL, [_I, _I]),
     "sn_plane_sums_det": (_I, [_VP, _I, _I, _I, _I, _VP, _VP, _LL, _VP]),
     "sn_plane_stats_det": (_I, [_VP, _I, _I, _I, _I, _F, _VP, _VP, _LL, _VP]),
diff --git a/swapnet_b200/csrc/api.cu b/swapnet_b200/csrc/api.cu
--- a/swapnet_b200/csrc/api.cu
+++ b/swapnet_b200/csrc/api.cu
@@ -91,6 +91,10 @@
 
 int sn_wgrad_ksplit(const sn_wgrad_desc* desc, int sm_count) { return sn_wgrad_plan_ksplit(desc, sm_count); }
 
+long long sn_tap_gemm_mma_macs(const sn_tap_gemm_desc* desc) { return sn_tap_gemm_plan_mma_macs(desc); }
+
+long long sn_wgrad_mma_macs(const sn_wgrad_desc* desc) { return sn_wgrad_plan_mma_macs(desc); }
+
 void sn_plan_destroy(sn_plan* plan) {
   if (plan && plan->kind == 0 && plan->tg.p.tile_counter) cudaFree(plan->tg.p.tile_counter);
   if (plan && plan->kind == 1 && plan->wg.p.det_ws) cudaFree(plan->wg.p.det_ws);
diff --git a/swapnet_b200/csrc/common.cuh b/swapnet_b200/csrc/common.cuh
--- a/swapnet_b200/csrc/common.cuh
+++ b/swapnet_b200/csrc/common.cuh
@@ -134,9 +134,34 @@
 
 template <int N, bool F16>
 struct Wgmma;
+template <> struct Wgmma<8, false> {
+  template <int TA, int TB, int R>
+  static __device__ __forceinline__ void mma(float (&d)[R], uint64_t a, uint64_t b, int scale_d) {
+    static_assert(R >= 4, "accumulator array too small");
+    asm volatile(
+        "{\n.reg .pred p;\nsetp.ne.b32 p, %6, 0;\n"
+        "wgmma.mma_async.sync.aligned.m64n8k16.f32.bf16.bf16 "
+        "{%0, %1, %2, %3}, %4, %5, p, 1, 1, %7, %8;\n}\n"
+        : "+f"(d[0]), "+f"(d[1]), "+f"(d[2]), "+f"(d[3])
+        : "l"(a), "l"(b), "r"(scale_d), "n"(TA), "n"(TB));
+  }
+};
+template <> struct Wgmma<8, true> {
+  template <int TA, int TB, int R>
+  static __device__ __forceinline__ void mma(float (&d)[R], uint64_t a, uint64_t b, int scale_d) {
+    static_assert(R >= 4, "accumulator array too small");
+    asm volatile(
+        "{\n.reg .pred p;\nsetp.ne.b32 p, %6, 0;\n"
+        "wgmma.mma_async.sync.aligned.m64n8k16.f32.f16.f16 "
+        "{%0, %1, %2, %3}, %4, %5, p, 1, 1, %7, %8;\n}\n"
+        : "+f"(d[0]), "+f"(d[1]), "+f"(d[2]), "+f"(d[3])
+        : "l"(a), "l"(b), "r"(scale_d), "n"(TA), "n"(TB));
+  }
+};
 template <> struct Wgmma<16, false> {
-  template <int TA, int TB>
-  static __device__ __forceinline__ void mma(float (&d)[8], uint64_t a, uint64_t b, int scale_d) {
+  template <int TA, int TB, int R>
+  static __device__ __forceinline__ void mma(float (&d)[R], uint64_t a, uint64_t b, int scale_d) {
+    static_assert(R >= 8, "accumulator array too small");
     asm volatile(
         "{\n.reg .pred p;\nsetp.ne.b32 p, %10, 0;\n"
         "wgmma.mma_async.sync.aligned.m64n16k16.f32.bf16.bf16 "
@@ -146,8 +171,9 @@
   }
 };
 template <> struct Wgmma<16, true> {
-  template <int TA, int TB>
-  static __device__ __forceinline__ void mma(float (&d)[8], uint64_t a, uint64_t b, int scale_d) {
+  template <int TA, int TB, int R>
+  static __device__ __forceinline__ void mma(float (&d)[R], uint64_t a, uint64_t b, int scale_d) {
+    static_assert(R >= 8, "accumulator array too small");
     asm volatile(
         "{\n.reg .pred p;\nsetp.ne.b32 p, %10, 0;\n"
         "wgmma.mma_async.sync.aligned.m64n16k16.f32.f16.f16 "
@@ -157,8 +183,9 @@
   }
 };
 template <> struct Wgmma<32, false> {
-  template <int TA, int TB>
-  static __device__ __forceinline__ void mma(float (&d)[16], uint64_t a, uint64_t b, int scale_d) {
+  template <int TA, int TB, int R>
+  static __device__ __forceinline__ void mma(float (&d)[R], uint64_t a, uint64_t b, int scale_d) {
+    static_assert(R >= 16, "accumulator array too small");
     asm volatile(
         "{\n.reg .pred p;\nsetp.ne.b32 p, %18, 0;\n"
         "wgmma.mma_async.sync.aligned.m64n32k16.f32.bf16.bf16 "
@@ -168,8 +195,9 @@
   }
 };
 template <> struct Wgmma<32, true> {
-  template <int TA, int TB>
-  static __device__ __forceinline__ void mma(float (&d)[16], uint64_t a, uint64_t b, int scale_d) {
+  template <int TA, int TB, int R>
+  static __device__ __forceinline__ void mma(float (&d)[R], uint64_t a, uint64_t b, int scale_d) {
+    static_assert(R >= 16, "accumulator array too small");
     asm volatile(
         "{\n.reg .pred p;\nsetp.ne.b32 p, %18, 0;\n"
         "wgmma.mma_async.sync.aligned.m64n32k16.f32.f16.f16 "
@@ -178,9 +206,34 @@
         : "l"(a), "l"(b), "r"(scale_d), "n"(TA), "n"(TB));
   }
 };
+template <> struct Wgmma<48, false> {
+  template <int TA, int TB, int R>
+  static __device__ __forceinline__ void mma(float (&d)[R], uint64_t a, uint64_t b, int scale_d) {
+    static_assert(R >= 24, "accumulator array too small");
+    asm volatile(
+        "{\n.reg .pred p;\nsetp.ne.b32 p, %26, 0;\n"
+        "wgmma.mma_async.sync.aligned.m64n48k16.f32.bf16.bf16 "
+        "{%0, %1, %2, %3, %4, %5, %6, %7, %8, %9, %10, %11, %12, %13, %14, %15, %16, %17, %18, %19, %20, %21, %22, %23}, %24, %25, p, 1, 1, %27, %28;\n}\n"
+        : "+f"(d[0]), "+f"(d[1]), "+f"(d[2]), "+f"(d[3]), "+f"(d[4]), "+f"(d[5]), "+f"(d[6]), "+f"(d[7]), "+f"(d[8]), "+f"(d[9]), "+f"(d[10]), "+f"(d[11]), "+f"(d[12]), "+f"(d[13]), "+f"(d[14]), "+f"(d[15]), "+f"(d[16]), "+f"(d[17]), "+f"(d[18]), "+f"(d[19]), "+f"(d[20]), "+f"(d[21]), "+f"(d[22]), "+f"(d[23])
+        : "l"(a), "l"(b), "r"(scale_d), "n"(TA), "n"(TB));
+  }
+};
+template <> struct Wgmma<48, true> {
+  template <int TA, int TB, int R>
+  static __device__ __forceinline__ void mma(float (&d)[R], uint64_t a, uint64_t b, int scale_d) {
+    static_assert(R >= 24, "accumulator array too small");
+    asm volatile(
+        "{\n.reg .pred p;\nsetp.ne.b32 p, %26, 0;\n"
+        "wgmma.mma_async.sync.aligned.m64n48k16.f32.f16.f16 "
+        "{%0, %1, %2, %3, %4, %5, %6, %7, %8, %9, %10, %11, %12, %13, %14, %15, %16, %17, %18, %19, %20, %21, %22, %23}, %24, %25, p, 1, 1, %27, %28;\n}\n"
+        : "+f"(d[0]), "+f"(d[1]), "+f"(d[2]), "+f"(d[3]), "+f"(d[4]), "+f"(d[5]), "+f"(d[6]), "+f"(d[7]), "+f"(d[8]), "+f"(d[9]), "+f"(d[10]), "+f"(d[11]), "+f"(d[12]), "+f"(d[13]), "+f"(d[14]), "+f"(d[15]), "+f"(d[16]), "+f"(d[17]), "+f"(d[18]), "+f"(d[19]), "+f"(d[20]), "+f"(d[21]), "+f"(d[22]), "+f"(d[23])
+        : "l"(a), "l"(b), "r"(scale_d), "n"(TA), "n"(TB));
+  }
+};
 template <> struct Wgmma<64, false> {
-  template <int TA, int TB>
-  static __device__ __forceinline__ void mma(float (&d)[32], uint64_t a, uint64_t b, int scale_d) {
+  template <int TA, int TB, int R>
+  static __device__ __forceinline__ void mma(float (&d)[R], uint64_t a, uint64_t b, int scale_d) {
+    static_assert(R >= 32, "accumulator array too small");
     asm volatile(
         "{\n.reg .pred p;\nsetp.ne.b32 p, %34, 0;\n"
         "wgmma.mma_async.sync.aligned.m64n64k16.f32.bf16.bf16 "
@@ -190,8 +243,9 @@
   }
 };
 template <> struct Wgmma<64, true> {
-  template <int TA, int TB>
-  static __device__ __forceinline__ void mma(float (&d)[32], uint64_t a, uint64_t b, int scale_d) {
+  template <int TA, int TB, int R>
+  static __device__ __forceinline__ void mma(float (&d)[R], uint64_t a, uint64_t b, int scale_d) {
+    static_assert(R >= 32, "accumulator array too small");
     asm volatile(
         "{\n.reg .pred p;\nsetp.ne.b32 p, %34, 0;\n"
         "wgmma.mma_async.sync.aligned.m64n64k16.f32.f16.f16 "
@@ -201,8 +255,9 @@
   }
 };
 template <> struct Wgmma<96, false> {
-  template <int TA, int TB>
-  static __device__ __forceinline__ void mma(float (&d)[48], uint64_t a, uint64_t b, int scale_d) {
+  template <int TA, int TB, int R>
+  static __device__ __forceinline__ void mma(float (&d)[R], uint64_t a, uint64_t b, int scale_d) {
+    static_assert(R >= 48, "accumulator array too small");
     asm volatile(
         "{\n.reg .pred p;\nsetp.ne.b32 p, %50, 0;\n"
         "wgmma.mma_async.sync.aligned.m64n96k16.f32.bf16.bf16 "
@@ -212,8 +267,9 @@
   }
 };
 template <> struct Wgmma<96, true> {
-  template <int TA, int TB>
-  static __device__ __forceinline__ void mma(float (&d)[48], uint64_t a, uint64_t b, int scale_d) {
+  template <int TA, int TB, int R>
+  static __device__ __forceinline__ void mma(float (&d)[R], uint64_t a, uint64_t b, int scale_d) {
+    static_assert(R >= 48, "accumulator array too small");
     asm volatile(
         "{\n.reg .pred p;\nsetp.ne.b32 p, %50, 0;\n"
         "wgmma.mma_async.sync.aligned.m64n96k16.f32.f16.f16 "
@@ -223,8 +279,9 @@
   }
 };
 template <> struct Wgmma<128, false> {
-  template <int TA, int TB>
-  static __device__ __forceinline__ void mma(float (&d)[64], uint64_t a, uint64_t b, int scale_d) {
+  template <int TA, int TB, int R>
+  static __device__ __forceinline__ void mma(float (&d)[R], uint64_t a, uint64_t b, int scale_d) {
+    static_assert(R >= 64, "accumulator array too small");
     asm volatile(
         "{\n.reg .pred p;\nsetp.ne.b32 p, %66, 0;\n"
         "wgmma.mma_async.sync.aligned.m64n128k16.f32.bf16.bf16 "
@@ -234,8 +291,9 @@
   }
 };
 template <> struct Wgmma<128, true> {
-  template <int TA, int TB>
-  static __device__ __forceinline__ void mma(float (&d)[64], uint64_t a, uint64_t b, int scale_d) {
+  template <int TA, int TB, int R>
+  static __device__ __forceinline__ void mma(float (&d)[R], uint64_t a, uint64_t b, int scale_d) {
+    static_assert(R >= 64, "accumulator array too small");
     asm volatile(
         "{\n.reg .pred p;\nsetp.ne.b32 p, %66, 0;\n"
         "wgmma.mma_async.sync.aligned.m64n128k16.f32.f16.f16 "
@@ -244,7 +302,6 @@
         : "l"(a), "l"(b), "r"(scale_d), "n"(TA), "n"(TB));
   }
 };
-
 
 __device__ __forceinline__ uint64_t gmma_smem_desc(uint32_t smem_addr, uint32_t lbo_bytes, uint32_t sbo_bytes,
                                                    uint32_t layout = 1) {
diff --git a/swapnet_b200/csrc/gemm_tc.cu b/swapnet_b200/csrc/gemm_tc.cu
--- a/swapnet_b200/csrc/gemm_tc.cu
+++ b/swapnet_b200/csrc/gemm_tc.cu
@@ -17,6 +17,10 @@
   static constexpr int kStageBytes = kPlanes * 2 * kTileBytes;
   static constexpr int kSmemBytes = kStages * kStageBytes + 1024;
 };
+
+__host__ __device__ constexpr int mma_n(int block_n) {
+  return block_n <= 16 ? 16 : block_n <= 32 ? 32 : block_n <= 64 ? 64 : block_n <= 96 ? 96 : 128;
+}
 
 __device__ __forceinline__ float apply_act(float v, int act) {
   if (act == SN_ACT_TANH) return tanhf(v);
@@ -290,7 +294,15 @@
   }
 }
 
-template <int NSPLIT, int BN, bool F16, bool DET>
+__host__ __device__ inline bool wgrad_half_rows(int rows_left) { return rows_left <= 64; }
+__host__ __device__ inline int wgrad_cta_cols(int block_n, int gsize, int ycw, bool grouped) {
+  return mma_n(grouped ? gsize * ycw : block_n);
+}
+__host__ __device__ inline unsigned wgrad_shape_bit(bool half, int cta_cols) {
+  return half ? 1u << (16 + cta_cols / 16) : 1u << (cta_cols / 8);
+}
+
+template <int NSPLIT, int WN, bool HALF, bool F16, bool DET>
 __global__ void __launch_bounds__(kThreads, 1)
 wgrad_gemm_kernel(const __grid_constant__ WgradParams p) {
   using C = Cfg<NSPLIT>;
@@ -317,6 +329,11 @@
   const int ycw = p.y_chunk;
   const int y_blocks = ycw == 64 ? p.block_n / 64 : gsize;
   const int y_block_bytes = 64 * ycw * 2;
+  const int cta_cols = p.one_cols ? p.one_cols : wgrad_cta_cols(p.block_n, gsize, ycw, grouped);
+  const bool half = !p.full_rows && wgrad_half_rows(p.rows_valid - m0);
+  if (half != HALF || (HALF ? cta_cols / 2 : cta_cols) != WN)
+    return;
+  constexpr int x_blocks = HALF ? 1 : 2;
 
   if (threadIdx.x == 0) {
     for (int s = 0; s < C::kStages; ++s) {
@@ -337,7 +354,7 @@
     if (warp == kProducerWarp) {
       if (lane == 0) {
         const TapDesc xt = p.xtaps[tap_i];
-        const uint32_t stage_tx = C::kPlanes * (2 * 8192 + y_blocks * y_block_bytes);
+        const uint32_t stage_tx = C::kPlanes * (x_blocks * 8192 + y_blocks * y_block_bytes);
         for (int it = 0; it < k_iters; ++it) {
           const int s = it % C::kStages;
           const uint32_t ph = (it / C::kStages) & 1;
@@ -350,13 +367,13 @@
           const int w0 = tw_i * p.tw, h0 = th_i * p.th, n0 = tn_i * p.nb;
           uint8_t* st = smem + s * C::kStageBytes;
           if (p.x_merged) {
-            for (int b = 0; b < 2; ++b)
+            for (int b = 0; b < x_blocks; ++b)
               tma_load_5d(&p.tmX[0], &full_bar[s], st + b * 16384, xt.c_off + m0 + b * 64, w0 + xt.dw, h0 + xt.dh,
                           n0, 0);
           } else {
 #pragma unroll
             for (int pl = 0; pl < C::kPlanes; ++pl)
-              for (int b = 0; b < 2; ++b)
+              for (int b = 0; b < x_blocks; ++b)
                 tma_load_5d(&p.tmX[pl], &full_bar[s], st + pl * kTileBytes + b * 8192,
                             xt.c_off + m0 + b * 64, w0 + xt.dw, xt.hp, h0 + xt.dh, n0);
           }
@@ -379,33 +396,37 @@
       }
     } else if (warp < kProducerWarp) {
       const int wg = warp >> 2;
-      float acc[BN / 2], part[BN / 2];
-#pragma unroll
-      for (int i = 0; i < BN / 2; ++i) acc[i] = 0.f;
+      const int col0 = HALF ? wg * WN : 0;
+      const int xblk = HALF ? 0 : wg;
+      float acc[WN / 2], part[WN / 2];
+#pragma unroll
+      for (int i = 0; i < WN / 2; ++i) acc[i] = 0.f;
       const uint32_t y_layout = gmma_layout_of_chunk(ycw);
       const uint32_t y_sbo = 8u * ycw * 2u;
       const uint32_t x_lbo = p.x_merged ? 16384u : 8192u;
       const uint32_t x_lo_off = p.x_merged ? 8192u : (uint32_t)kTileBytes;
       const uint32_t y_lbo = p.y_merged ? 16384u : (uint32_t)y_block_bytes;
       const uint32_t y_lo_off = p.y_merged ? 8192u : (uint32_t)kTileBytes;
+      const uint32_t y_col_off = (uint32_t)(col0 / ycw) * y_lbo + (uint32_t)(col0 % ycw) * 2u;
       for (int it = 0; it < k_iters; ++it) {
         const int s = it % C::kStages;
         const uint32_t ph = (it / C::kStages) & 1;
         mbar_wait(&full_bar[s], ph);
         const uint32_t st = smem_base + s * C::kStageBytes;
-        const uint64_t x_hi = gmma_smem_desc(st + wg * x_lbo, x_lbo, 1024);
-        const uint64_t y_hi = gmma_smem_desc(st + C::kPlanes * kTileBytes, y_lbo, y_sbo, y_layout);
-        const uint64_t x_lo = gmma_smem_desc(st + x_lo_off + wg * x_lbo, x_lbo, 1024);
-        const uint64_t y_lo = gmma_smem_desc(st + C::kPlanes * kTileBytes + y_lo_off, y_lbo, y_sbo, y_layout);
+        const uint64_t x_hi = gmma_smem_desc(st + xblk * x_lbo, x_lbo, 1024);
+        const uint64_t y_hi = gmma_smem_desc(st + C::kPlanes * kTileBytes + y_col_off, y_lbo, y_sbo, y_layout);
+        const uint64_t x_lo = gmma_smem_desc(st + x_lo_off + xblk * x_lbo, x_lbo, 1024);
+        const uint64_t y_lo =
+            gmma_smem_desc(st + C::kPlanes * kTileBytes + y_lo_off + y_col_off, y_lbo, y_sbo, y_layout);
         wgmma_fence();
 #pragma unroll
         for (int k = 0; k < 4; ++k) {
           const uint64_t xadv = (uint64_t)(k * 128);
           const uint64_t yadv = (uint64_t)((k * 16 * ycw * 2) >> 4);
-          Wgmma<BN, F16>::template mma<1, 1>(part, x_hi + xadv, y_hi + yadv, k != 0);
+          Wgmma<WN, F16>::template mma<1, 1>(part, x_hi + xadv, y_hi + yadv, k != 0);
           if (NSPLIT == 3) {
-            Wgmma<BN, F16>::template mma<1, 1>(part, x_lo + xadv, y_hi + yadv, 1);
-            Wgmma<BN, F16>::template mma<1, 1>(part, x_hi + xadv, y_lo + yadv, 1);
+            Wgmma<WN, F16>::template mma<1, 1>(part, x_lo + xadv, y_hi + yadv, 1);
+            Wgmma<WN, F16>::template mma<1, 1>(part, x_hi + xadv, y_lo + yadv, 1);
           }
         }
         wgmma_commit();
@@ -413,10 +434,10 @@
         wgmma_fence_acc(part);
         if ((threadIdx.x & 127) == 0) mbar_arrive(&empty_bar[s]);
 #pragma unroll
-        for (int i = 0; i < BN / 2; ++i) acc[i] += part[i];
+        for (int i = 0; i < WN / 2; ++i) acc[i] += part[i];
       }
       const int quad = lane & 3;
-      const int row0 = m0 + wg * 64 + (warp & 3) * 16 + (lane >> 2);
+      const int row0 = m0 + 64 * xblk + (warp & 3) * 16 + (lane >> 2);
 #pragma unroll
       for (int h = 0; h < 2; ++h) {
         const int row = row0 + 8 * h;
@@ -424,10 +445,10 @@
         float* orow = p.out + (long long)row * p.s_row;
         float* wrow = DET ? p.det_ws + (long long)blockIdx.z * p.det_count + (long long)row * p.cols_valid : nullptr;
 #pragma unroll
-        for (int i = 0; i < BN / 8; ++i) {
+        for (int i = 0; i < WN / 8; ++i) {
 #pragma unroll
           for (int e = 0; e < 2; ++e) {
-            const int c = 8 * i + 2 * quad + e;
+            const int c = col0 + 8 * i + 2 * quad + e;
             const float v = acc[4 * i + 2 * h + e];
             if (!grouped) {
               const int col = ncol0 + c;
@@ -693,10 +714,6 @@
   return SN_OK;
 }
 
-static int mma_n(int block_n) {
-  return block_n <= 16 ? 16 : block_n <= 32 ? 32 : block_n <= 64 ? 64 : block_n <= 96 ? 96 : 128;
-}
-
 template <int NSPLIT, int CW, int BN, bool F16>
 static int launch_tap(const TapGemmPlan* plan, cudaStream_t stream) {
   static bool attr_done = false;
@@ -758,6 +775,31 @@
   }
   if (ks > total) ks = total;
   return ks;
+}
+
+static int wgrad_one_cols(const sn_wgrad_desc* d, int y_chunk) {
+  if (y_chunk == 64 || d->ngroups <= 0) return 0;
+  for (int g = 1; g < d->ngroups; ++g)
+    if (wgrad_cta_cols(d->block_n, d->group_size[g], y_chunk, true) !=
+        wgrad_cta_cols(d->block_n, d->group_size[0], y_chunk, true))
+      return mma_n(d->block_n);
+  return 0;
+}
+
+static unsigned wgrad_plan_shapes(const sn_wgrad_desc* d, int y_chunk, int* ctas = nullptr) {
+  const bool grouped = y_chunk != 64 && d->ngroups > 0;
+  const int one_cols = wgrad_one_cols(d, y_chunk);
+  unsigned mask = 0;
+  if (ctas)
+    for (int b = 0; b < 32; ++b) ctas[b] = 0;
+  for (int m0 = 0; m0 < d->rows_valid; m0 += kBlockM)
+    for (int g = 0; g < (grouped ? d->ngroups : 1); ++g) {
+      const int cols = one_cols ? one_cols : wgrad_cta_cols(d->block_n, grouped ? d->group_size[g] : 1, y_chunk, grouped);
+      const unsigned bit = wgrad_shape_bit(wgrad_half_rows(d->rows_valid - m0), cols);
+      mask |= bit;
+      if (ctas) ctas[__builtin_ctz(bit)] += grouped ? 1 : d->ntaps;
+    }
+  return mask;
 }
 
 int sn_wgrad_plan_init(WgradPlan* plan, const sn_wgrad_desc* d, int sm_count) {
@@ -848,10 +890,22 @@
     if (p.y_merged) p.tmY[1] = p.tmY[0];
   }
   plan->nsplit = d->nsplit;
+  int shape_ctas[32];
+  plan->wn_mask = wgrad_plan_shapes(d, y_chunk, shape_ctas);
+  const bool mixed = __builtin_popcount(plan->wn_mask) > 1;
+  p.one_cols = wgrad_one_cols(d, y_chunk);
+  p.full_rows = mixed && d->deterministic;
+  if (p.full_rows)
+    plan->wn_mask = wgrad_shape_bit(false, p.one_cols ? p.one_cols
+                                                      : wgrad_cta_cols(d->block_n, p.ngroups ? p.gsize[0] : 1, y_chunk,
+                                                                       p.ngroups > 0));
   const int base_ctas = p.m_tiles * p.n_tiles * grid_y;
   const int total = p.tiles_w * p.tiles_h * p.tiles_n;
   const int ks = wgrad_ksplit(d, base_ctas, total, sm_count);
   plan->grid = dim3(p.m_tiles * p.n_tiles, grid_y, ks);
+  for (int b = 0; b < 32; ++b)
+    plan->shape_ks[b] = mixed && !d->deterministic && shape_ctas[b] > 0
+                            ? wgrad_ksplit(d, shape_ctas[b] * p.n_tiles, total, sm_count) : ks;
   p.det_ws = nullptr;
   p.det_count = 0;
   plan->ws_bytes = 0;
@@ -878,23 +932,72 @@
   return wgrad_ksplit(d, m_tiles * n_tiles * grid_y, total, sm_count);
 }
 
-template <int NSPLIT, int BN, bool F16, bool DET>
+long long sn_tap_gemm_plan_mma_macs(const sn_tap_gemm_desc* d) {
+  SN_REQUIRE(d && d->ntaps >= 1 && d->ntaps <= SN_MAX_TAPS && d->block_n >= 16 && d->block_n <= 128,
+             "tap_gemm_mma_macs: bad descriptor");
+  int th, tw, nb;
+  pick_patch_conv(d->m_n, d->m_h, d->m_w, &th, &tw, &nb);
+  const long long m_tiles = (long long)((d->m_w + tw - 1) / tw) * ((d->m_h + th - 1) / th) * ((d->m_n + nb - 1) / nb);
+  const long long n_tiles = (d->n_valid + d->block_n - 1) / d->block_n;
+  return m_tiles * n_tiles * kBlockM * mma_n(d->block_n) * (long long)d->ntaps * d->k_per_tap;
+}
+
+long long sn_wgrad_plan_mma_macs(const sn_wgrad_desc* d) {
+  SN_REQUIRE(d && d->ntaps >= 1 && d->ntaps <= SN_MAX_TAPS, "wgrad_mma_macs: bad descriptor");
+  int th, tw, nb;
+  pick_patch(d->m_h, d->m_w, 64, &th, &tw, &nb);
+  const long long pixels = 64LL * ((d->m_w + tw - 1) / tw) * ((d->m_h + th - 1) / th) * ((d->m_n + nb - 1) / nb);
+  const int ycw = d->y_chunk ? d->y_chunk : 64;
+  const bool grouped = ycw != 64 && d->ngroups > 0;
+  const int n_tiles = ycw == 64 ? (d->cols_valid + d->block_n - 1) / d->block_n : 1;
+  const long long m_tiles = (d->rows_valid + kBlockM - 1) / kBlockM;
+  const bool full_rows = d->deterministic && __builtin_popcount(wgrad_plan_shapes(d, ycw)) > 1;
+  const int one_cols = wgrad_one_cols(d, ycw);
+  long long per_pixel = 0;
+  for (int m0 = 0; m0 < d->rows_valid; m0 += kBlockM)
+    for (int g = 0; g < (grouped ? d->ngroups : d->ntaps); ++g)
+      per_pixel += (!full_rows && wgrad_half_rows(d->rows_valid - m0) ? 64 : kBlockM) *
+                   (long long)(one_cols ? one_cols : wgrad_cta_cols(d->block_n, grouped ? d->group_size[g] : 1, ycw,
+                                                                    grouped));
+  return pixels * per_pixel * n_tiles;
+}
+
+template <int NSPLIT, int WN, bool HALF, bool F16, bool DET>
 static int launch_wgrad_k(const WgradPlan* plan, cudaStream_t stream) {
+  if (!(plan->wn_mask & wgrad_shape_bit(HALF, HALF ? 2 * WN : WN))) return SN_OK;
   static bool attr_done = false;
   if (!attr_done) {
-    SN_CHECK_CUDA(cudaFuncSetAttribute(wgrad_gemm_kernel<NSPLIT, BN, F16, DET>,
+    SN_CHECK_CUDA(cudaFuncSetAttribute(wgrad_gemm_kernel<NSPLIT, WN, HALF, F16, DET>,
                                        cudaFuncAttributeMaxDynamicSharedMemorySize, Cfg<NSPLIT>::kSmemBytes));
     attr_done = true;
   }
-  wgrad_gemm_kernel<NSPLIT, BN, F16, DET><<<plan->grid, kThreads, Cfg<NSPLIT>::kSmemBytes, stream>>>(plan->p);
+  const dim3 grid(plan->grid.x, plan->grid.y, plan->shape_ks[__builtin_ctz(wgrad_shape_bit(HALF, HALF ? 2 * WN : WN))]);
+  wgrad_gemm_kernel<NSPLIT, WN, HALF, F16, DET><<<grid, kThreads, Cfg<NSPLIT>::kSmemBytes, stream>>>(plan->p);
   SN_CHECK_CUDA(cudaGetLastError());
   return SN_OK;
 }
 
-template <int NSPLIT, int BN, bool F16>
+template <int NSPLIT, bool F16, bool DET>
+static int launch_wgrad_widths(const WgradPlan* plan, cudaStream_t stream) {
+  int rc = SN_OK;
+  if (!rc) rc = launch_wgrad_k<NSPLIT, 128, false, F16, DET>(plan, stream);
+  if (!rc) rc = launch_wgrad_k<NSPLIT, 96, false, F16, DET>(plan, stream);
+  if (!rc) rc = launch_wgrad_k<NSPLIT, 64, false, F16, DET>(plan, stream);
+  if (!rc) rc = launch_wgrad_k<NSPLIT, 32, false, F16, DET>(plan, stream);
+  if (!rc) rc = launch_wgrad_k<NSPLIT, 16, false, F16, DET>(plan, stream);
+  if (!rc) rc = launch_wgrad_k<NSPLIT, 64, true, F16, DET>(plan, stream);
+  if (!rc) rc = launch_wgrad_k<NSPLIT, 48, true, F16, DET>(plan, stream);
+  if (!rc) rc = launch_wgrad_k<NSPLIT, 32, true, F16, DET>(plan, stream);
+  if (!rc) rc = launch_wgrad_k<NSPLIT, 16, true, F16, DET>(plan, stream);
+  if (!rc) rc = launch_wgrad_k<NSPLIT, 8, true, F16, DET>(plan, stream);
+  sn_count_launch(__builtin_popcount(plan->wn_mask) - 1);
+  return rc;
+}
+
+template <int NSPLIT, bool F16>
 static int launch_wgrad(const WgradPlan* plan, cudaStream_t stream) {
-  if (!plan->p.det_ws) return launch_wgrad_k<NSPLIT, BN, F16, false>(plan, stream);
-  const int rc = launch_wgrad_k<NSPLIT, BN, F16, true>(plan, stream);
+  if (!plan->p.det_ws) return launch_wgrad_widths<NSPLIT, F16, false>(plan, stream);
+  const int rc = launch_wgrad_widths<NSPLIT, F16, true>(plan, stream);
   if (rc) return rc;
   long long g = (plan->p.det_count + 255) / 256;
   if (g > SN_NUM_SMS * 8) g = SN_NUM_SMS * 8;
@@ -904,19 +1007,8 @@
   return SN_OK;
 }
 
-template <int NSPLIT, bool F16>
-static int launch_wgrad_n(const WgradPlan* plan, cudaStream_t stream) {
-  switch (mma_n(plan->p.block_n)) {
-    case 16: return launch_wgrad<NSPLIT, 16, F16>(plan, stream);
-    case 32: return launch_wgrad<NSPLIT, 32, F16>(plan, stream);
-    case 64: return launch_wgrad<NSPLIT, 64, F16>(plan, stream);
-    case 96: return launch_wgrad<NSPLIT, 96, F16>(plan, stream);
-    default: return launch_wgrad<NSPLIT, 128, F16>(plan, stream);
-  }
-}
-
 int sn_wgrad_plan_launch(const WgradPlan* plan, cudaStream_t stream) {
   const bool f16 = plan->p.x_fmt == SN_FMT_F16;
-  if (plan->nsplit == 3) return f16 ? launch_wgrad_n<3, true>(plan, stream) : launch_wgrad_n<3, false>(plan, stream);
-  return f16 ? launch_wgrad_n<1, true>(plan, stream) : launch_wgrad_n<1, false>(plan, stream);
-}
+  if (plan->nsplit == 3) return f16 ? launch_wgrad<3, true>(plan, stream) : launch_wgrad<3, false>(plan, stream);
+  return f16 ? launch_wgrad<1, true>(plan, stream) : launch_wgrad<1, false>(plan, stream);
+}
diff --git a/swapnet_b200/csrc/plan.h b/swapnet_b200/csrc/plan.h
--- a/swapnet_b200/csrc/plan.h
+++ b/swapnet_b200/csrc/plan.h
@@ -54,6 +54,8 @@
   int ngroups;
   int x_merged, y_merged;
   short gstart[SN_MAX_TAPS], gsize[SN_MAX_TAPS];
+  int one_cols;
+  int full_rows;
   float* det_ws;
   long long det_count;
 };
@@ -69,6 +71,8 @@
   dim3 grid;
   int nsplit;
   size_t ws_bytes;
+  unsigned wn_mask;
+  int shape_ks[32];
 };
 
 int sn_tap_gemm_plan_init(TapGemmPlan* plan, const sn_tap_gemm_desc* d);
@@ -76,3 +80,5 @@
 int sn_wgrad_plan_init(WgradPlan* plan, const sn_wgrad_desc* d, int sm_count);
 int sn_wgrad_plan_launch(const WgradPlan* plan, cudaStream_t stream);
 int sn_wgrad_plan_ksplit(const sn_wgrad_desc* d, int sm_count);
+long long sn_tap_gemm_plan_mma_macs(const sn_tap_gemm_desc* d);
+long long sn_wgrad_plan_mma_macs(const sn_wgrad_desc* d);
diff --git a/swapnet_b200/lowering.py b/swapnet_b200/lowering.py
--- a/swapnet_b200/lowering.py
+++ b/swapnet_b200/lowering.py
@@ -245,9 +245,9 @@
 
 
 def pick_block_n(n_valid: int) -> int:
-    if n_valid >= 128:
-        return 128
-    for b in (16, 32, 64, 128):
+    for b in (16, 32, 64):
         if n_valid <= b:
             return b
+    if -(-n_valid // 96) * 96 < -(-n_valid // 128) * 128:
+        return 96
     return 128
diff --git a/swapnet_b200/ops.py b/swapnet_b200/ops.py
--- a/swapnet_b200/ops.py
+++ b/swapnet_b200/ops.py
@@ -283,6 +283,15 @@
     return int(k)
 
 
+def mma_macs(desc) -> int:
+    lib = _lib.load()
+    k = lib.sn_tap_gemm_mma_macs(C.byref(desc)) if isinstance(desc, SnTapGemmDesc) else \
+        lib.sn_wgrad_mma_macs(C.byref(desc))
+    if k < 0:
+        check(int(k))
+    return int(k)
+
+
 def wgrad_plan(desc: SnWgradDesc, keep: Sequence = ()) -> Plan:
     h = C.c_void_p()
     check(_lib.load().sn_wgrad_plan_create(C.byref(desc), C.byref(h)))
```

Result: no change. 138.3 (median of 6 runs) (+0.6%).
